# sangminwoo/SVOL

Hardware: AMD Instinct MI355X
Metric: frames/sec (fwd+matcher+bwd), T=32·P=196·d=256 (higher is better)
Workload: dtype bf16

## Files before the change

### include/svol_hip.h

```cpp
#ifndef SVOL_HIP_H
#define SVOL_HIP_H

#include <stdint.h>

#ifdef __cplusplus
extern "C" {
#endif

#define SVOL_F32 0
#define SVOL_BF16 1
#define SVOL_F16 2

#define SVOL_OK 0
#define SVOL_E_INVALID (-1)
#define SVOL_E_UNSUPPORTED (-2)
#define SVOL_E_LAUNCH (-3)

#define SVOL_ACT_NONE 0
#define SVOL_ACT_RELU 1
#define SVOL_ACT_GELU 2
#define SVOL_ACT_SIGMOID 3
#define SVOL_ACT_GELU_D 5
#define SVOL_ACT_RELU_RES 4

int svol_abi_version(void);
const char* svol_strerror(int code);

int svol_cast(const void* src, int dtype_src, void* dst, int dtype_dst, int64_t n, void* stream);
int svol_cast_transpose(const float* src, void* dst, void* dstT, int dtype, int64_t R, int64_t C, void* stream);
int svol_cast_transpose_multi(const void* descs, int32_t n_desc, int64_t total_tiles, int dtype, void* stream);
int svol_cast_split(const float* src, int64_t ld_src, void* dst_hilo, int64_t R, int64_t C, void* stream);

int svol_adamw_flat(float* p, const float* g, float* m, float* v, int64_t n, float lr, float beta1, float beta2, float eps,
                    float weight_decay, int64_t step, float grad_scale, void* stream);
int svol_adamw_flat_zero(float* p, float* g, float* m, float* v, int64_t n, float lr, float beta1, float beta2, float eps,
                         float weight_decay, int64_t step, float grad_scale, void* stream);
int svol_grad_finite(const float* g, int64_t n, float* scaler_state, void* stream);
int svol_adamw_flat_scaled(float* p, const float* g, float* m, float* v, int64_t n, float lr, float beta1, float beta2, float eps,
                           float weight_decay, float grad_mul, const float* scaler_state, void* stream);
int svol_loss_scaler_update(float* scaler_state, float growth_factor, float backoff_factor, int64_t growth_interval, float min_scale,
                            float max_scale, void* stream);
int svol_sgd_flat(float* p, const float* g, float* buf, int64_t n, float lr, float momentum, float weight_decay, float grad_scale,
                  void* stream);
int svol_sgd_flat_zero(float* p, float* g, float* buf, int64_t n, float lr, float momentum, float weight_decay, float grad_scale,
                       void* stream);
int svol_sgd_flat_scaled(float* p, const float* g, float* buf, int64_t n, float lr, float momentum, float weight_decay, float grad_mul,
                         const float* scaler_state, void* stream);
int svol_adam_flat(float* p, const float* g, float* m, float* v, int64_t n, float lr, float beta1, float beta2, float eps,
                   float weight_decay, int64_t step, float grad_scale, void* stream);
int svol_adam_flat_zero(float* p, float* g, float* m, float* v, int64_t n, float lr, float beta1, float beta2, float eps,
                        float weight_decay, int64_t step, float grad_scale, void* stream);
int svol_adam_flat_scaled(float* p, const float* g, float* m, float* v, int64_t n, float lr, float beta1, float beta2, float eps,
                          float weight_decay, float grad_mul, const float* scaler_state, void* stream);
int64_t svol_grad_sqnorm_ws_bytes(int64_t n);
int svol_grad_sqnorm(const float* g, int64_t n, float* ws, float* out, void* stream);
int svol_grad_clip_state(const float* sq, int32_t nb, float grad_mul, float max_norm, float loss_scale, int64_t steps_taken,
                         float* scaler_state, float* state_out, void* stream);
int svol_sgd_flat_grouped(float* p, float* g, float* buf, int64_t n, const int32_t* seg_end, const int32_t* seg_group, int32_t nseg,
                          const float* hyper, int32_t ngroups, const float* state, float grad_mul, int zero, void* stream);
int svol_adam_flat_grouped(float* p, float* g, float* m, float* v, int64_t n, const int32_t* seg_end, const int32_t* seg_group,
                           int32_t nseg, const float* hyper, int32_t ngroups, const float* state, const float* step_count,
                           float grad_mul, int zero, void* stream);
int svol_adamw_flat_grouped(float* p, float* g, float* m, float* v, int64_t n, const int32_t* seg_end, const int32_t* seg_group,
                            int32_t nseg, const float* hyper, int32_t ngroups, const float* state, const float* step_count,
                            float grad_mul, int zero, void* stream);
int svol_flat_step_advance(float* step_count, const float* state, void* stream);

int svol_gemm_nt(const void* A, int64_t lda, const void* A2, int64_t n_split, const void* B, int64_t ldb,
                 void* C, int64_t ldc, const float* bias, const float* colscale, int act, void* pre_act_out,
                 int64_t ldp, const void* residual, int64_t ldr, int out_f32, int64_t M, int64_t N, int64_t K,
                 int dtype, void* stream);
int svol_gemm_nt_split(const void* A, int64_t lda, const void* W_hilo, int64_t ldw, void* C, int64_t ldc, const float* bias,
                       int64_t M, int64_t N, int64_t K, void* stream);
int svol_gemm_nt_dgelu(const void* A, int64_t lda, const void* B, int64_t ldb, void* C, int64_t ldc,
                       const void* pre, int64_t ldp, float* colsum, int64_t M, int64_t N, int64_t K, int dtype,
                       void* stream);
int svol_gemm_nt_dact(const void* A, int64_t lda, const void* B, int64_t ldb, void* C, int64_t ldc,
                      const void* aux, int64_t ldaux, int act, float* colsum, int64_t M, int64_t N, int64_t K,
                      int dtype, void* stream);

int svol_gemm_tn(const void* A, int64_t lda, const void* B, int64_t ldb, float* C, int64_t ldc, float* colsum,
                 int64_t Mc, int64_t N, int64_t K, int dtype, void* stream);
#define SVOL_TN_GROUP_MAX 6
typedef struct svol_tn_problem {
    const void* A; int64_t lda;
    const void* B; int64_t ldb;
    float* C; int64_t ldc;
    float* colsum;
    int64_t Mc, N, K;
} svol_tn_problem;
int svol_gemm_tn_grouped(const svol_tn_problem* problems, int32_t n, int dtype, void* stream);
int svol_colsum(const void* X, int64_t ldx, float* out, int64_t M, int64_t N, int dtype, void* stream);
int svol_act_bwd(const void* dy, const void* aux, void* dpre, int act, int64_t n, int dtype, void* stream);

int svol_layernorm_fwd(const void* x, int x_f32, const float* gamma, const float* beta, float* y32, void* y,
                       void* ypos, const void* pos, int64_t pos_rows, float* mean, float* rstd, int64_t M, int64_t D,
                       float dropout_p, uint64_t seed, const int64_t* seed_offset_dev, int dtype, void* stream);
int svol_layernorm_bwd(const float* dy32, const void* dy, const void* dy2, const void* x, int x_f32,
                       const float* gamma, const float* mean, const float* rstd, float* dx32, void* dx,
                       float* dgamma, float* dbeta, float* dx_colsum, int64_t M, int64_t D, float dropout_p,
                       uint64_t seed, const int64_t* seed_offset_dev, int dtype, void* stream);

int svol_dropout(const void* x, void* y, int64_t n, int64_t row_len, float p, uint64_t seed, int dtype, void* stream);
int svol_dropout_add(const float* t32, const float* res32, float* out32, int64_t n, int64_t row_len, float p, uint64_t seed, void* stream);
int svol_dropout_sd(const void* x, void* y, int64_t n, int64_t row_len, float p, uint64_t seed, const int64_t* seed_step_dev, int dtype,
                    void* stream);
int svol_dropout_add_sd(const float* t32, const float* res32, float* out32, int64_t n, int64_t row_len, float p, uint64_t seed,
                        const int64_t* seed_step_dev, void* stream);

int svol_posenc_sine(const float* mask, void* pos, int64_t B, int64_t L, int64_t D, int dtype, void* stream);

int64_t svol_attn_ws_bytes(int64_t B, int64_t H, int64_t Lq, int64_t Lk, int64_t dh);
int svol_attn_fwd(const void* q, int64_t ldq, const void* k, int64_t ldk, const void* v, int64_t ldv, void* o,
                  int64_t ldo, float* lse2, const float* kbias, int64_t B, int64_t H, int64_t Lq, int64_t Lk,
                  int64_t dh, float scale, float q_premul, void* ws, int64_t ws_bytes, int dtype, void* stream);
int svol_attn_bwd(const void* q, int64_t ldq, const void* k, int64_t ldk, const void* v, int64_t ldv, const void* o,
                  int64_t ldo, const void* d_o, int64_t lddo, const float* lse2, float* delta, const float* kbias,
                  void* dq, int64_t lddq, void* dk, int64_t lddk, void* dv, int64_t lddv, int64_t B, int64_t H,
                  int64_t Lq, int64_t Lk, int64_t dh, float scale, float q_premul, void* ws, int64_t ws_bytes,
                  int dtype, void* stream);

#define SVOL_ATTN_DQ_PREZEROED 1
int64_t svol_attn_bwd_sp_image_bytes(int64_t B, int64_t H, int64_t Lq, int64_t Lk, int64_t dh, int64_t ws_bytes, int dtype);
int svol_attn_bwd_zero_ws(void* ws, int64_t ws_bytes, int64_t B, int64_t H, int64_t Lq, int64_t Lk, int64_t dh, int dtype, void* stream);
int svol_attn_bwd_ex(const void* q, int64_t ldq, const void* k, int64_t ldk, const void* v, int64_t ldv, const void* o,
                     int64_t ldo, const void* d_o, int64_t lddo, const float* lse2, float* delta, const float* kbias,
                     void* dq, int64_t lddq, void* dk, int64_t lddk, void* dv, int64_t lddv, int64_t B, int64_t H,
                     int64_t Lq, int64_t Lk, int64_t dh, float scale, float q_premul, void* ws, int64_t ws_bytes,
                     int dtype, int flags, void* ev_prep, void* stream);

int svol_attn_fwd_dropout(const void* q, int64_t ldq, const void* k, int64_t ldk, const void* v, int64_t ldv, void* o,
                          int64_t ldo, float* lse2, const float* kbias, int64_t B, int64_t H, int64_t Lq, int64_t Lk,
                          int64_t dh, float scale, float q_premul, void* ws, int64_t ws_bytes, float dropout_p, uint64_t seed,
                          int dtype, void* stream);
int svol_attn_bwd_dropout(const void* q, int64_t ldq, const void* k, int64_t ldk, const void* v, int64_t ldv, const void* o,
                          int64_t ldo, const void* d_o, int64_t lddo, const float* lse2, float* delta, const float* kbias,
                          void* dq, int64_t lddq, void* dk, int64_t lddk, void* dv, int64_t lddv, int64_t B, int64_t H,
                          int64_t Lq, int64_t Lk, int64_t dh, float scale, float q_premul, void* ws, int64_t ws_bytes,
                          float dropout_p, uint64_t seed, int dtype, void* stream);
int svol_attn_fwd_dropout_sd(const void* q, int64_t ldq, const void* k, int64_t ldk, const void* v, int64_t ldv, void* o,
                             int64_t ldo, float* lse2, const float* kbias, int64_t B, int64_t H, int64_t Lq, int64_t Lk,
                             int64_t dh, float scale, float q_premul, void* ws, int64_t ws_bytes, float dropout_p, uint64_t seed,
                             const int64_t* seed_step_dev, int dtype, void* stream);
int svol_attn_bwd_dropout_sd(const void* q, int64_t ldq, const void* k, int64_t ldk, const void* v, int64_t ldv, const void* o,
                             int64_t ldo, const void* d_o, int64_t lddo, const float* lse2, float* delta, const float* kbias,
                             void* dq, int64_t lddq, void* dk, int64_t lddk, void* dv, int64_t lddv, int64_t B, int64_t H,
                             int64_t Lq, int64_t Lk, int64_t dh, float scale, float q_premul, void* ws, int64_t ws_bytes,
                             float dropout_p, uint64_t seed, const int64_t* seed_step_dev, int dtype, void* stream);

int svol_gate_fwd(const float* x32, const void* pos, const float* u, const float* gamma, const float* beta,
                  float* y32, void* y, void* ypos, float* a, float* mean, float* rstd, float* ws, int64_t B,
                  int64_t L, int64_t D, int64_t H, int dtype, void* stream);
int svol_gate_bwd(const float* dy32, const void* dy, const void* dy2, const float* x32, const void* pos,
                  const float* u, const float* gamma, const float* a, const float* mean, const float* rstd,
                  const float* ws, float* ws2, float* dx32, float* du, float* dgamma, float* dbeta, int64_t B,
                  int64_t L, int64_t D, int64_t H, int dtype, void* stream);

int svol_layernorm_gate_scores_fwd(const float* x32, const float* gamma, const float* beta, float* y32, void* y, void* ypos,
                                   const void* pos, float* mean, float* rstd, const float* u_next, float* scores_next,
                                   int64_t B, int64_t L, int64_t D, int64_t H, int dtype, void* stream);
int svol_gate_fwd_scored(const float* x32, const void* pos, const float* u, const float* gamma, const float* beta,
                         float* y32, void* y, void* ypos, float* a, float* mean, float* rstd, float* ws, int64_t B,
                         int64_t L, int64_t D, int64_t H, int dtype, void* stream);

int svol_gate_vectors_fwd(const float* skch, const float* W_in, const float* b_in, float* q_out, float* u_out, int64_t B, int64_t D,
                          int64_t H, void* stream);
int svol_gate_vectors_bwd(const float* du, const float* skch, const float* W_in, const float* q, float* dq_ws, float* dskch,
                          float* dW_in, float* db_in, int64_t B, int64_t D, int64_t H, void* stream);
#define SVOL_GATE_VEC_MAX_LAYERS 8
int svol_gate_vectors_fwd_multi(const float* skch, const float* const* W_in, const float* const* b_in, float* const* q_out,
                                float* const* u_out, int64_t n_layers, int64_t B, int64_t D, int64_t H, void* stream);
int svol_gate_vectors_bwd_multi(const float* const* du, const float* skch, const float* const* W_in, const float* const* q,
                                float* const* dq_ws, float* const* dskch, float* const* dW_in, float* const* db_in, int64_t n_layers,
                                int64_t B, int64_t D, int64_t H, void* stream);

int svol_match_cost(const float* logits, const float* boxes, const float* tgt_boxes, const int32_t* pred_off,
                    const int32_t* pred_cnt, const int32_t* tgt_off, const int32_t* tgt_cnt,
                    const int64_t* cost_off, float* cost, int32_t n_problems, float w_bbox, float w_giou,
                    float w_class, int32_t* box_status, void* stream);
int svol_lsap_batched(const float* cost, const int64_t* cost_off, const int32_t* pred_off, const int32_t* pred_cnt,
                      const int32_t* tgt_off, const int32_t* tgt_cnt, int32_t* match, int32_t* status,
                      int32_t n_problems, int32_t max_dim, void* stream);
int svol_heads_fwd(const float* hs, const float* Wc, const float* bc, const float* W0, const float* b0, const float* W1, const float* b1,
                   const float* W2, const float* b2, float* logits, float* h1, float* h2, float* boxes, int64_t R, int64_t D, void* stream);
int svol_heads_bwd(const float* dlogits, const float* dboxes, const float* hs, const float* h1, const float* h2, const float* boxes,
                   const float* Wc, const float* W0, const float* W1, const float* W2, float* dhs, float* gp0, float* gp1, float* dWc,
                   float* dbc, float* dW2, float* db2, int64_t R, int64_t D, void* stream);
int svol_set_loss_bwd(const float* g_label, const float* g_bbox, const float* g_giou, const float* dl, float* dlogits, float* dboxes,
                      int64_t n_layers, int64_t rows_per_layer, void* stream);
int svol_weighted_total(const float* x, const float* w, int64_t n, float* out, void* stream);
int svol_weighted_total_bwd(const float* w, const float* dout, int64_t n, float* dx, void* stream);
int svol_lsap_solve(const double* cost, int64_t nr, int64_t nc, int64_t* rows, int64_t* cols);
int svol_set_loss(const float* logits, const float* boxes, const float* tgt_boxes, const int32_t* match,
                  float* losses, float* g_label, float* g_bbox, float* g_giou, int32_t n_layers,
                  int32_t rows_per_layer, float eos_coef, const int32_t* rebase_vid_off, int32_t rows_per_video,
                  const int32_t* status, const int32_t* box_status, int32_t problems_per_layer, void* stream);

int svol_postprocess(const float* logits, const float* boxes, float* out, int64_t B, int64_t N, int64_t chunk, void* stream);
int svol_eval_max_iou(const double* pred_box, const int32_t* pred_off, const double* gt_box, const int32_t* gt_off,
                      const int32_t* gt_rec, double* out, int64_t n_gt, int32_t k, void* stream);
int svol_eval_ap(const double* pred_box, const double* pred_score, const int32_t* pred_frame, const int32_t* grp_pred_off,
                 const double* gt_box, const int32_t* gt_frame, const int32_t* grp_gt_off, const double* thresholds,
                 int32_t n_thresholds, int32_t* ws_order, unsigned char* ws_u8, double* ws_f64, double* ap, int64_t n_pred,
                 int64_t n_gt, int64_t n_groups, void* stream);

int svol_ingest_resize(const uint8_t* src, int64_t n, int64_t H, int64_t W, int64_t s_n, int64_t s_h, int64_t s_w,
                       const int32_t* xtab, int64_t kx, const int32_t* ytab, int64_t ky, const float* lut, const uint8_t* flip,
                       void* out, int64_t o_n, int64_t o_c, int64_t o_h, int64_t o_w, int64_t OH, int64_t OW, int out_dtype,
                       void* stream);

int svol_patchify(const float* pixel_values, void* out, int64_t n, int64_t C, int64_t H, int64_t W, int64_t p, int dtype,
                  void* stream);
int svol_vit_embed(const float* patch_proj, const float* cls_token, const float* pos_embed, float* x32, void* x, int64_t n,
                   int64_t P, int64_t D, int dtype, void* stream);
int svol_im2col(const void* x, int64_t sn, int64_t sh, int64_t sw, int64_t sc, int src_dtype, void* cols, int64_t ldcols,
                int64_t N, int64_t H, int64_t W, int64_t C, int64_t kh, int64_t kw, int64_t stride, int64_t pad, int dtype,
                void* stream);
int svol_conv_nhwc(const void* x, const void* w, int64_t ldw, void* y, const float* bias, int act, const void* residual,
                   int64_t N, int64_t H, int64_t W, int64_t C, int64_t Cout, int64_t kh, int64_t kw, int64_t stride,
                   int64_t pad, int dtype, void* stream);
int svol_maxpool_nhwc(const void* x, void* y, int64_t N, int64_t H, int64_t W, int64_t C, int64_t k, int64_t stride,
                      int64_t pad, int dtype, void* stream);
int svol_avgpool_nhwc(const void* x, float* y, int64_t N, int64_t HW, int64_t C, int dtype, void* stream);
int svol_bn_colstats(const void* z, const float* shift, float shift_scale, float* sum, float* sumsq, int64_t M, int64_t C, int dtype,
                     void* stream);
int svol_bn_finalize(const float* sum, const float* sumsq_centered, const float* pivot, const float* gamma, const float* beta,
                     float* running_mean, float* running_var, float momentum, float eps, int64_t M, int64_t C, float* mean, float* rstd,
                     float* scale, float* shift, void* stream);
int svol_conv_weight_pack(const float* w, void* out, int64_t Cout, int64_t Cin, int64_t kh, int64_t kw, int64_t Kp, int flip, int dtype,
                          void* stream);
int svol_conv_weight_unpack_add(const float* dwp, float* grad, int64_t Cout, int64_t Cin, int64_t kh, int64_t kw, int64_t Kp, void* stream);
int svol_conv_wgrad_nhwc(const void* dz, const void* x, float* dwp, int64_t N, int64_t H, int64_t W, int64_t C, int64_t Cout, int64_t kh, int64_t kw,
                         int64_t stride, int64_t pad, int64_t Kp, int dtype, void* stream);
int svol_bn_apply(const void* z, const float* scale, const float* shift, const void* residual, int relu, void* y, int64_t M, int64_t C,
                  int dtype, void* stream);
int svol_bn_bwd_reduce(const void* dy, const void* y, const void* z, const float* mean, const float* rstd, float* sum_g, float* sum_gx,
                       int64_t M, int64_t C, int dtype, void* stream);
int svol_bn_bwd_apply(const void* dy, const void* y, const void* z, const float* mean, const float* rstd, const float* gamma,
                      const float* sum_g, const float* sum_gx, void* dz, void* dres, int64_t M, int64_t C, int dtype, void* stream);
int svol_col2im_nhwc(const void* dcols, int64_t ldcols, void* dx, int64_t N, int64_t H, int64_t W, int64_t C, int64_t kh, int64_t kw,
                     int64_t stride, int64_t pad, int dtype, void* stream);
int svol_maxpool_idx_nhwc(const void* x, void* y, uint8_t* idx, int64_t N, int64_t H, int64_t W, int64_t C, int64_t k, int64_t stride,
                          int64_t pad, int dtype, void* stream);
int svol_maxpool_bwd_nhwc(const void* dy, const uint8_t* idx, void* dx, int64_t N, int64_t H, int64_t W, int64_t C, int64_t k,
                          int64_t stride, int64_t pad, int dtype, void* stream);
int svol_attn_weights_mean(const void* q, int64_t ldq, const void* k, int64_t ldk, const float* lse2, const float* kbias,
                           float* att, int64_t B, int64_t H, int64_t Lq, int64_t Lk, int64_t dh, float scale,
                           float q_premul, int dtype, void* stream);
int svol_attn_small_fwd(const void* q, int64_t ldq, const void* k, int64_t ldk, const void* v, int64_t ldv, void* o, int64_t ldo,
                        int64_t n_seq, int64_t H, int64_t L, int64_t dh, float scale, int dtype, void* stream);
int svol_attn_small_fwd_lse(const void* q, int64_t ldq, const void* k, int64_t ldk, const void* v, int64_t ldv, void* o, int64_t ldo,
                            float* lse2, int64_t n_seq, int64_t H, int64_t L, int64_t dh, float scale, int dtype, void* stream);
int svol_attn_small_bwd(const void* q, int64_t ldq, const void* k, int64_t ldk, const void* v, int64_t ldv, const void* o, int64_t ldo,
                        const void* dout, int64_t lddo, const float* lse2, void* dq, int64_t lddq, void* dk, int64_t lddk, void* dv,
                        int64_t lddv, int64_t n_seq, int64_t H, int64_t L, int64_t dh, float scale, int dtype, void* stream);
int svol_attn_small_fwd_h16(const void* q, int64_t ldq, const void* k, int64_t ldk, const void* v, int64_t ldv, void* o, int64_t ldo,
                            int64_t n_seq, int64_t H, int64_t L, int64_t dh, float scale, int dtype, void* stream);
int svol_attn_small_fwd_lse_h16(const void* q, int64_t ldq, const void* k, int64_t ldk, const void* v, int64_t ldv, void* o, int64_t ldo,
                                float* lse2, int64_t n_seq, int64_t H, int64_t L, int64_t dh, float scale, int dtype, void* stream);
int svol_attn_small_bwd_h16(const void* q, int64_t ldq, const void* k, int64_t ldk, const void* v, int64_t ldv, const void* o, int64_t ldo,
                            const void* dout, int64_t lddo, const float* lse2, void* dq, int64_t lddq, void* dk, int64_t lddk, void* dv,
                            int64_t lddv, int64_t n_seq, int64_t H, int64_t L, int64_t dh, float scale, int dtype, void* stream);

int svol_attn_cls_fwd(const void* q, int64_t ldq, const void* k, int64_t ldk, const void* v, int64_t ldv, void* o, int64_t ldo, float* lse2,
                      int64_t n, int64_t H, int64_t L, int64_t dh, float scale, int dtype, void* stream);
int svol_attn_cls_bwd(const void* q, int64_t ldq, const void* k, int64_t ldk, const void* v, int64_t ldv, const void* o, int64_t ldo,
                      const void* dout, int64_t lddo, const float* lse2, void* dq, int64_t lddq, void* dk, int64_t lddk, void* dv,
                      int64_t lddv, int64_t n, int64_t H, int64_t L, int64_t dh, float scale, int dtype, void* stream);
int svol_attn_cls_fwd_h16(const void* q, int64_t ldq, const void* k, int64_t ldk, const void* v, int64_t ldv, void* o, int64_t ldo, float* lse2,
                          int64_t n, int64_t H, int64_t L, int64_t dh, float scale, int dtype, void* stream);
int svol_attn_cls_bwd_h16(const void* q, int64_t ldq, const void* k, int64_t ldk, const void* v, int64_t ldv, const void* o, int64_t ldo,
                          const void* dout, int64_t lddo, const float* lse2, void* dq, int64_t lddq, void* dk, int64_t lddk, void* dv,
                          int64_t lddv, int64_t n, int64_t H, int64_t L, int64_t dh, float scale, int dtype, void* stream);
int svol_softmax_xent(const float* logits, int64_t ld, const int64_t* targets, float* loss, float* dlogits, int64_t lddl, int32_t* correct,
                      int64_t n, int64_t C, void* stream);


#define SVOL_DIM_B 0
#define SVOL_DIM_L 1
#define SVOL_DIM_N 2
#define SVOL_DIM_D 3
#define SVOL_DIM_H 4
#define SVOL_DIM_F 5
#define SVOL_DIM_DTYPE 6
#define SVOL_DIM_QDTYPE 7
#define SVOL_DIM_ATTN_WS_BYTES 8
#define SVOL_DIM_COUNT 9

#define SVOL_BLK_VIDEO_HALF 0
#define SVOL_BLK_QUERY_SELF 1
#define SVOL_BLK_QUERY_CROSS 2
const char* svol_block_slot_names(int block);
int svol_block_trace_dump(char* buf, int64_t cap);
int svol_clock_probe(uint64_t* samples, int32_t* count, int32_t max_samples, const int32_t* stop, int64_t period_us,
                     int64_t max_ms, int32_t* wall_khz, void* stream);


#define SVOL_VH_SLOTS(X) \
    X(X32) X(POS) X(U) X(G1) X(BT1) X(G2) X(BT2) X(G3) X(BT3) X(B_IN) X(B_O) X(B_FC1) X(B_FC2) X(QSCALE) \
    X(W_IN) X(WV_HILO) X(W_O) X(W_FC1) X(W_FC2) X(W_IN_T) X(W_O_T) X(W_FC1_T) X(W_FC2_T) \
    X(Y1) X(Y1POS) X(A) X(MEAN1) X(RSTD1) X(GATE_WS) X(GATE_PRE) X(U_NEXT) X(GATE_WS_NEXT) \
    X(QKV) X(O) X(LSE) X(S2) X(Y2) X(MEAN2) X(RSTD2) X(PRE) X(HID) X(S3) \
    X(MEAN3) X(RSTD3) X(M32) X(M) X(MPOS) X(Y1_32) X(Y2_32) X(ATTN_WS) \
    X(DM32) X(DM) X(DMPOS) X(DS32_3) X(DS3) X(DPRE) X(DY2) X(DS32_2) X(G2D) X(DO) X(DQKV) X(DELTA) X(DXQP) X(DXQ) X(GATE_WS2) \
    X(DX32) X(DU) \
    X(DG1) X(DBT1) X(DG2) X(DBT2) X(DG3) X(DBT3) X(DW_IN) X(DB_IN) X(DW_O) X(DB_O) X(DW_FC1) X(DB_FC1) X(DW_FC2) X(DB_FC2) \
    X(EV_A0) X(EV_A1) X(EV_CLEAN_IN) X(EV_PREP) X(ATTN_WS_NEXT) X(ZERO_STREAM) X(EV_CLEAN_OUT)
#define SVOL_QS_SLOTS(X) \
    X(O32) X(O) X(OPOS) X(QPOS) X(B_IN) X(B_O) X(G4) X(BT4) X(QSCALE) X(W_IN) X(WV_HILO) X(W_O) X(W_IN_T) X(W_O_T) \
    X(QKV) X(OA) X(LSE) X(S4) X(MEAN4) X(RSTD4) X(Y32) X(Y) X(YPOS) X(ATTN_WS) \
    X(DY32) X(DY) X(DYPOS) X(G) X(DOA) X(DQKV) X(DELTA) X(DO32) X(DXQ) X(DXQP) X(DQPOS) \
    X(DW_IN) X(DB_IN) X(DW_O) X(DB_O) X(DG4) X(DBT4)
#define SVOL_QC_SLOTS(X) \
    X(O32) X(O) X(OPOS) X(MV) X(MPOS) X(KBIAS) X(QPOS) X(B_IN) X(B_O) X(G5) X(BT5) X(B_FC1) X(B_FC2) X(G6) X(BT6) X(QSCALE) \
    X(W_INQ) X(W_INQ_T) X(W_KV) X(W_KV_T) X(WV_HILO) X(W_O) X(W_O_T) X(W_FC1) X(W_FC1_T) X(W_FC2) X(W_FC2_T) \
    X(Q) X(QC) X(KV) X(OA) X(OAQ) X(LSE) X(S5) X(Y5_32) X(Y5) X(MEAN5) X(RSTD5) X(PRE) X(HID) X(S6) X(MEAN6) X(RSTD6) \
    X(Y32) X(Y) X(YPOS) X(ATTN_WS) \
    X(DY32) X(DY) X(DYPOS) X(DS32_6) X(DS6) X(DPRE) X(DY5) X(DS32_5) X(G5D) X(DOAQ) X(DOA) X(DQC) X(DQ) X(DKV) X(DELTA) \
    X(DO32) X(DXQP) X(DMPOS) X(DMV) X(DQPOS) \
    X(DW_IN) X(DB_IN) X(DW_O) X(DB_O) X(DG5) X(DBT5) X(DW_FC1) X(DB_FC1) X(DW_FC2) X(DB_FC2) X(DG6) X(DBT6)
#define SVOL_SLOT_ENUM_VH(n) SVOL_VH_##n,
#define SVOL_SLOT_ENUM_QS(n) SVOL_QS_##n,
#define SVOL_SLOT_ENUM_QC(n) SVOL_QC_##n,
enum { SVOL_VH_SLOTS(SVOL_SLOT_ENUM_VH) SVOL_VH_COUNT };
enum { SVOL_QS_SLOTS(SVOL_SLOT_ENUM_QS) SVOL_QS_COUNT };
enum { SVOL_QC_SLOTS(SVOL_SLOT_ENUM_QC) SVOL_QC_COUNT };

int svol_video_half_fwd(const int64_t* dims, void* const* slots, void* stream);
int svol_video_half_bwd(const int64_t* dims, void* const* slots, int phase, void* stream);
int svol_video_half_wgrad(const int64_t* dims, void* const* slots, void* stream);
int svol_video_half_wgrad_part(const int64_t* dims, void* const* slots, int part, void* stream);
int svol_query_self_fwd(const int64_t* dims, void* const* slots, void* stream);
int svol_query_self_bwd(const int64_t* dims, void* const* slots, void* stream);
int svol_query_self_wgrad(const int64_t* dims, void* const* slots, void* stream);
int svol_query_cross_fwd(const int64_t* dims, void* const* slots, void* stream);
int svol_query_cross_bwd(const int64_t* dims, void* const* slots, void* stream);
int svol_query_cross_wgrad(const int64_t* dims, void* const* slots, void* stream);

#ifdef __cplusplus
}
#endif
#endif
```

### svol_amd/_lib.py

```python
from __future__ import annotations

import ctypes
import os

_HERE = os.path.dirname(os.path.abspath(__file__))
LIB_PATH = os.path.join(_HERE, 'libsvol_hip.so')

_p = ctypes.c_void_p
_i64 = ctypes.c_int64
_i32 = ctypes.c_int32
_int = ctypes.c_int
_f32 = ctypes.c_float
_u64 = ctypes.c_uint64

SIGNATURES = {
    'svol_block_trace_dump': [ctypes.c_char_p, _i64],
    'svol_lsap_solve': [_p, _i64, _i64, _p, _p],
    'svol_heads_fwd': [_p] * 13 + [_i64, _i64, _p],
    'svol_heads_bwd': [_p] * 17 + [_i64, _i64, _p],
    'svol_set_loss_bwd': [_p] * 6 + [_i64, _i64, _p],
    'svol_weighted_total': [_p, _p, _i64, _p, _p],
    'svol_weighted_total_bwd': [_p, _p, _i64, _p, _p],
    'svol_cast': [_p, _int, _p, _int, _i64, _p],
    'svol_cast_transpose': [_p, _p, _p, _int, _i64, _i64, _p],
    'svol_cast_split': [_p, _i64, _p, _i64, _i64, _p],
    'svol_gemm_nt_split': [_p, _i64, _p, _i64, _p, _i64, _p, _i64, _i64, _i64, _p],
    'svol_gemm_nt': [_p, _i64, _p, _i64, _p, _i64, _p, _i64, _p, _p, _int, _p, _i64, _p, _i64, _int, _i64, _i64, _i64,
                     _int, _p],
    'svol_gemm_nt_dgelu': [_p, _i64, _p, _i64, _p, _i64, _p, _i64, _p, _i64, _i64, _i64, _int, _p],
    'svol_gemm_nt_dact': [_p, _i64, _p, _i64, _p, _i64, _p, _i64, _int, _p, _i64, _i64, _i64, _int, _p],
    'svol_gemm_tn': [_p, _i64, _p, _i64, _p, _i64, _p, _i64, _i64, _i64, _int, _p],
    'svol_gemm_tn_grouped': [_p, _i32, _int, _p],
    'svol_colsum': [_p, _i64, _p, _i64, _i64, _int, _p],
    'svol_act_bwd': [_p, _p, _p, _int, _i64, _int, _p],
    'svol_layernorm_fwd': [_p, _int, _p, _p, _p, _p, _p, _p, _i64, _p, _p, _i64, _i64, _f32, _u64, _p, _int, _p],
    'svol_layernorm_bwd': [_p, _p, _p, _p, _int, _p, _p, _p, _p, _p, _p, _p, _p, _i64, _i64, _f32, _u64, _p, _int, _p],
    'svol_cast_transpose_multi': [_p, _int, _i64, _int, _p],
    'svol_postprocess': [_p, _p, _p, _i64, _i64, _i64, _p],
    'svol_eval_max_iou': [_p, _p, _p, _p, _p, _p, _i64, _int, _p],
    'svol_eval_ap': [_p, _p, _p, _p, _p, _p, _p, _p, _int, _p, _p, _p, _p, _i64, _i64, _i64, _p],
    'svol_patchify': [_p, _p, _i64, _i64, _i64, _i64, _i64, _int, _p],
    'svol_vit_embed': [_p, _p, _p, _p, _p, _i64, _i64, _i64, _int, _p],
    'svol_ingest_resize': [_p, _i64, _i64, _i64, _i64, _i64, _i64, _p, _i64, _p, _i64, _p, _p, _p, _i64, _i64, _i64, _i64, _i64, _i64, _int, _p],
    'svol_adamw_flat': [_p, _p, _p, _p, _i64, _f32, _f32, _f32, _f32, _f32, _i64, _f32, _p],
    'svol_adamw_flat_zero': [_p, _p, _p, _p, _i64, _f32, _f32, _f32, _f32, _f32, _i64, _f32, _p],
    'svol_grad_finite': [_p, _i64, _p, _p],
    'svol_adamw_flat_scaled': [_p, _p, _p, _p, _i64, _f32, _f32, _f32, _f32, _f32, _f32, _p, _p],
    'svol_loss_scaler_update': [_p, _f32, _f32, _i64, _f32, _f32, _p],
    'svol_sgd_flat': [_p, _p, _p, _i64, _f32, _f32, _f32, _f32, _p],
    'svol_sgd_flat_zero': [_p, _p, _p, _i64, _f32, _f32, _f32, _f32, _p],
    'svol_sgd_flat_scaled': [_p, _p, _p, _i64, _f32, _f32, _f32, _f32, _p, _p],
    'svol_adam_flat': [_p, _p, _p, _p, _i64, _f32, _f32, _f32, _f32, _f32, _i64, _f32, _p],
    'svol_adam_flat_zero': [_p, _p, _p, _p, _i64, _f32, _f32, _f32, _f32, _f32, _i64, _f32, _p],
    'svol_adam_flat_scaled': [_p, _p, _p, _p, _i64, _f32, _f32, _f32, _f32, _f32, _f32, _p, _p],
    'svol_grad_sqnorm_ws_bytes': [_i64],
    'svol_grad_sqnorm': [_p, _i64, _p, _p, _p],
    'svol_grad_clip_state': [_p, _i32, _f32, _f32, _f32, _i64, _p, _p, _p],
    'svol_sgd_flat_grouped': [_p, _p, _p, _i64, _p, _p, _i32, _p, _i32, _p, _f32, _int, _p],
    'svol_adam_flat_grouped': [_p, _p, _p, _p, _i64, _p, _p, _i32, _p, _i32, _p, _p, _f32, _int, _p],
    'svol_adamw_flat_grouped': [_p, _p, _p, _p, _i64, _p, _p, _i32, _p, _i32, _p, _p, _f32, _int, _p],
    'svol_flat_step_advance': [_p, _p, _p],
    'svol_conv_nhwc': [_p, _p, _i64, _p, _p, _int, _p, _i64, _i64, _i64, _i64, _i64, _i64, _i64, _i64, _i64, _int, _p],
    'svol_im2col': [_p, _i64, _i64, _i64, _i64, _int, _p, _i64, _i64, _i64, _i64, _i64, _i64, _i64, _i64, _i64, _int, _p],
    'svol_maxpool_nhwc': [_p, _p, _i64, _i64, _i64, _i64, _i64, _i64, _i64, _int, _p],
    'svol_avgpool_nhwc': [_p, _p, _i64, _i64, _i64, _int, _p],
    'svol_bn_colstats': [_p, _p, _f32, _p, _p, _i64, _i64, _int, _p],
    'svol_bn_finalize': [_p, _p, _p, _p, _p, _p, _p, _f32, _f32, _i64, _i64, _p, _p, _p, _p, _p],
    'svol_conv_weight_pack': [_p, _p, _i64, _i64, _i64, _i64, _i64, _int, _int, _p],
    'svol_conv_weight_unpack_add': [_p, _p, _i64, _i64, _i64, _i64, _i64, _p],
    'svol_conv_wgrad_nhwc': [_p, _p, _p, _i64, _i64, _i64, _i64, _i64, _i64, _i64, _i64, _i64, _i64, _int, _p],
    'svol_bn_apply': [_p, _p, _p, _p, _int, _p, _i64, _i64, _int, _p],
    'svol_bn_bwd_reduce': [_p, _p, _p, _p, _p, _p, _p, _i64, _i64, _int, _p],
    'svol_bn_bwd_apply': [_p, _p, _p, _p, _p, _p, _p, _p, _p, _p, _i64, _i64, _int, _p],
    'svol_col2im_nhwc': [_p, _i64, _p, _i64, _i64, _i64, _i64, _i64, _i64, _i64, _i64, _int, _p],
    'svol_maxpool_idx_nhwc': [_p, _p, _p, _i64, _i64, _i64, _i64, _i64, _i64, _i64, _int, _p],
    'svol_maxpool_bwd_nhwc': [_p, _p, _p, _i64, _i64, _i64, _i64, _i64, _i64, _i64, _int, _p],
    'svol_attn_weights_mean': [_p, _i64, _p, _i64, _p, _p, _p, _i64, _i64, _i64, _i64, _i64, _f32, _f32, _int, _p],
    'svol_attn_small_fwd': [_p, _i64, _p, _i64, _p, _i64, _p, _i64, _i64, _i64, _i64, _i64, _f32, _int, _p],
    'svol_attn_small_fwd_lse': [_p, _i64, _p, _i64, _p, _i64, _p, _i64, _p, _i64, _i64, _i64, _i64, _f32, _int, _p],
    'svol_attn_small_bwd': [_p, _i64, _p, _i64, _p, _i64, _p, _i64, _p, _i64, _p, _p, _i64, _p, _i64, _p, _i64, _i64, _i64, _i64,
                            _i64, _f32, _int, _p],
    'svol_attn_cls_fwd': [_p, _i64, _p, _i64, _p, _i64, _p, _i64, _p, _i64, _i64, _i64, _i64, _f32, _int, _p],
    'svol_attn_cls_bwd': [_p, _i64, _p, _i64, _p, _i64, _p, _i64, _p, _i64, _p, _p, _i64, _p, _i64, _p, _i64, _i64, _i64, _i64,
                          _i64, _f32, _int, _p],
    'svol_attn_small_fwd_h16': [_p, _i64, _p, _i64, _p, _i64, _p, _i64, _i64, _i64, _i64, _i64, _f32, _int, _p],
    'svol_attn_small_fwd_lse_h16': [_p, _i64, _p, _i64, _p, _i64, _p, _i64, _p, _i64, _i64, _i64, _i64, _f32, _int, _p],
    'svol_attn_small_bwd_h16': [_p, _i64, _p, _i64, _p, _i64, _p, _i64, _p, _i64, _p, _p, _i64, _p, _i64, _p, _i64, _i64, _i64, _i64,
                                _i64, _f32, _int, _p],
    'svol_attn_cls_fwd_h16': [_p, _i64, _p, _i64, _p, _i64, _p, _i64, _p, _i64, _i64, _i64, _i64, _f32, _int, _p],
    'svol_attn_cls_bwd_h16': [_p, _i64, _p, _i64, _p, _i64, _p, _i64, _p, _i64, _p, _p, _i64, _p, _i64, _p, _i64, _i64, _i64, _i64,
                              _i64, _f32, _int, _p],
    'svol_softmax_xent': [_p, _i64, _p, _p, _p, _i64, _p, _i64, _i64, _p],
    'svol_posenc_sine': [_p, _p, _i64, _i64, _i64, _int, _p],
    'svol_attn_ws_bytes': [_i64, _i64, _i64, _i64, _i64],
    'svol_attn_fwd': [_p, _i64, _p, _i64, _p, _i64, _p, _i64, _p, _p, _i64, _i64, _i64, _i64, _i64, _f32, _f32, _p, _i64,
                      _int, _p],
    'svol_attn_bwd': [_p, _i64, _p, _i64, _p, _i64, _p, _i64, _p, _i64, _p, _p, _p, _p, _i64, _p, _i64, _p, _i64,
                      _i64, _i64, _i64, _i64, _i64, _f32, _f32, _p, _i64, _int, _p],
    'svol_attn_bwd_ex': [_p, _i64, _p, _i64, _p, _i64, _p, _i64, _p, _i64, _p, _p, _p, _p, _i64, _p, _i64, _p, _i64,
                         _i64, _i64, _i64, _i64, _i64, _f32, _f32, _p, _i64, _int, _int, _p, _p],
    'svol_attn_bwd_sp_image_bytes': [_i64, _i64, _i64, _i64, _i64, _i64, _int],
    'svol_attn_bwd_zero_ws': [_p, _i64, _i64, _i64, _i64, _i64, _i64, _int, _p],
    'svol_attn_fwd_dropout': [_p, _i64, _p, _i64, _p, _i64, _p, _i64, _p, _p, _i64, _i64, _i64, _i64, _i64, _f32, _f32, _p, _i64,
                              _f32, _u64, _int, _p],
    'svol_attn_bwd_dropout': [_p, _i64, _p, _i64, _p, _i64, _p, _i64, _p, _i64, _p, _p, _p, _p, _i64, _p, _i64, _p, _i64,
                              _i64, _i64, _i64, _i64, _i64, _f32, _f32, _p, _i64, _f32, _u64, _int, _p],
    'svol_dropout': [_p, _p, _i64, _i64, _f32, _u64, _int, _p],
    'svol_dropout_add': [_p, _p, _p, _i64, _i64, _f32, _u64, _p],
    'svol_attn_fwd_dropout_sd': [_p, _i64, _p, _i64, _p, _i64, _p, _i64, _p, _p, _i64, _i64, _i64, _i64, _i64, _f32, _f32, _p, _i64,
                                 _f32, _u64, _p, _int, _p],
    'svol_attn_bwd_dropout_sd': [_p, _i64, _p, _i64, _p, _i64, _p, _i64, _p, _i64, _p, _p, _p, _p, _i64, _p, _i64, _p, _i64,
                                 _i64, _i64, _i64, _i64, _i64, _f32, _f32, _p, _i64, _f32, _u64, _p, _int, _p],
    'svol_dropout_sd': [_p, _p, _i64, _i64, _f32, _u64, _p, _int, _p],
    'svol_dropout_add_sd': [_p, _p, _p, _i64, _i64, _f32, _u64, _p, _p],
    'svol_gate_fwd': [_p, _p, _p, _p, _p, _p, _p, _p, _p, _p, _p, _p, _i64, _i64, _i64, _i64, _int, _p],
    'svol_gate_bwd': [_p, _p, _p, _p, _p, _p, _p, _p, _p, _p, _p, _p, _p, _p, _p, _p, _i64, _i64, _i64, _i64, _int,
                      _p],
    'svol_clock_probe': [_p, _p, _int, _p, _i64, _i64, _p, _p],
    'svol_gate_fwd_scored': [_p, _p, _p, _p, _p, _p, _p, _p, _p, _p, _p, _p, _i64, _i64, _i64, _i64, _int, _p],
    'svol_layernorm_gate_scores_fwd': [_p, _p, _p, _p, _p, _p, _p, _p, _p, _p, _p, _i64, _i64, _i64, _i64, _int, _p],
    'svol_gate_vectors_fwd': [_p, _p, _p, _p, _p, _i64, _i64, _i64, _p],
    'svol_gate_vectors_bwd': [_p, _p, _p, _p, _p, _p, _p, _p, _i64, _i64, _i64, _p],
    'svol_gate_vectors_fwd_multi': [_p, _p, _p, _p, _p, _i64, _i64, _i64, _i64, _p],
    'svol_gate_vectors_bwd_multi': [_p, _p, _p, _p, _p, _p, _p, _p, _i64, _i64, _i64, _i64, _p],
    'svol_match_cost': [_p, _p, _p, _p, _p, _p, _p, _p, _p, _i32, _f32, _f32, _f32, _p, _p],
    'svol_lsap_batched': [_p, _p, _p, _p, _p, _p, _p, _p, _i32, _i32, _p],
    'svol_set_loss': [_p, _p, _p, _p, _p, _p, _p, _p, _i32, _i32, _f32, _p, _i32, _p, _p, _i32, _p],
    'svol_video_half_fwd': [_p, _p, _p],
    'svol_video_half_bwd': [_p, _p, _int, _p],
    'svol_video_half_wgrad': [_p, _p, _p],
    'svol_video_half_wgrad_part': [_p, _p, _int, _p],
    'svol_query_self_fwd': [_p, _p, _p],
    'svol_query_self_bwd': [_p, _p, _p],
    'svol_query_self_wgrad': [_p, _p, _p],
    'svol_query_cross_fwd': [_p, _p, _p],
    'svol_query_cross_bwd': [_p, _p, _p],
    'svol_query_cross_wgrad': [_p, _p, _p],
}



class TnProblem(ctypes.Structure):
    _fields_ = [('A', _p), ('lda', _i64), ('B', _p), ('ldb', _i64), ('C', _p), ('ldc', _i64), ('colsum', _p),
                ('Mc', _i64), ('N', _i64), ('K', _i64)]


_LIB = None


class SvolHipError(RuntimeError):
    pass


def lib():
    global _LIB
    if _LIB is None:
        if not os.path.exists(LIB_PATH):
            raise SvolHipError(
                f'{LIB_PATH} not found: the SVOL hot path has no CPU fallback. '
                'Build it with `python -m svol_amd.build` (hipcc, gfx950).')
        L = ctypes.CDLL(LIB_PATH)
        L.svol_abi_version.restype = _int
        L.svol_abi_version.argtypes = []
        L.svol_strerror.restype = ctypes.c_char_p
        L.svol_strerror.argtypes = [_int]
        for name, at in SIGNATURES.items():
            f = getattr(L, name)
            f.restype = _int
            f.argtypes = at
        L.svol_attn_ws_bytes.restype = _i64
        L.svol_attn_bwd_sp_image_bytes.restype = _i64
        L.svol_grad_sqnorm_ws_bytes.restype = _i64
        L.svol_block_slot_names.restype = ctypes.c_char_p
        L.svol_block_slot_names.argtypes = [_int]
        _LIB = L
    return _LIB


def check(rc: int, name: str):
    if rc != 0:
        msg = lib().svol_strerror(rc).decode()
        raise SvolHipError(f'{name} failed: {msg} (code {rc})')
```

### svol_amd/blocks.py

```python
from __future__ import annotations

import ctypes
import math
import os
import weakref

import torch

from . import _lib, layers, ops, params, wgrad

ENABLED = os.environ.get('SVOL_NO_BLOCKS') is None
GATE_SCORES_FUSE = os.environ.get('SVOL_GATE_SCORES_FUSE') is not None
VH, QS, QC = 0, 1, 2
_F32, _BF16 = 0, 1
_ESZ = {torch.float32: 4, torch.bfloat16: 2, torch.float16: 2}
_SLOTS = {}


def _slots(block):
    m = _SLOTS.get(block)
    if m is None:
        names = _lib.lib().svol_block_slot_names(block).decode().rstrip(',').split(',')
        m = _SLOTS[block] = {n: i for i, n in enumerate(names)}
    return m


class _Table:

    __slots__ = ('arr', 'idx', 'n')

    def __init__(self, block, template=None):
        self.idx = _slots(block)
        self.n = len(self.idx)
        self.arr = (ctypes.c_void_p * self.n)()
        if template is not None:
            ctypes.memmove(self.arr, template.arr, self.n * 8)

    def set(self, name, ptr):
        self.arr[self.idx[name]] = ptr

    def set_t(self, name, t):
        self.arr[self.idx[name]] = t.data_ptr() if t is not None else None


def _align(n, a=256):
    return (n + a - 1) // a * a


class _Layout:

    def __init__(self, items):
        self.off = {}
        n = 0
        for name, nbytes in items:
            self.off[name] = (n, nbytes)
            n += _align(nbytes)
        self.total = max(n, 256)

    def fill(self, tbl, base):
        for name, (o, _) in self.off.items():
            tbl.arr[tbl.idx[name]] = base + o

    def view(self, arena, name, dtype, shape):
        o, nb = self.off[name]
        return arena[o:o + nb].view(dtype).view(shape)


_LAYOUTS = {}


def _layout(key, make):
    lay = _LAYOUTS.get(key)
    if lay is None:
        lay = _LAYOUTS[key] = _Layout(make())
    return lay


_SCRATCH = {}


def _scratch(dev, nbytes):
    key = (dev, ops._stream())
    t = _SCRATCH.get(key)
    if t is None or t.numel() < nbytes:
        t = _SCRATCH[key] = torch.empty((_align(nbytes, 1 << 20),), dtype=torch.uint8, device=dev)
    return t


def _dims(B, L, N, D, H, F, dt, qdt, ws_bytes):
    return (ctypes.c_int64 * 9)(B, L, N, D, H, F, ops._DT[dt], ops._DT[qdt], ws_bytes)


def _c(t):
    return t if t is None or t.is_contiguous() else t.contiguous()


_VH_PARAMS = [
    ('DG1', lambda l: l.norm1.weight), ('DBT1', lambda l: l.norm1.bias),
    ('DW_IN', lambda l: l.content_self_attn.in_proj_weight), ('DB_IN', lambda l: l.content_self_attn.in_proj_bias),
    ('DW_O', lambda l: l.content_self_attn.out_proj.weight), ('DB_O', lambda l: l.content_self_attn.out_proj.bias),
    ('DG2', lambda l: l.norm2.weight), ('DBT2', lambda l: l.norm2.bias),
    ('DW_FC1', lambda l: l.mlp1.fc1.weight), ('DB_FC1', lambda l: l.mlp1.fc1.bias),
    ('DW_FC2', lambda l: l.mlp1.fc2.weight), ('DB_FC2', lambda l: l.mlp1.fc2.bias),
    ('DG3', lambda l: l.norm3.weight), ('DBT3', lambda l: l.norm3.bias)]
_QS_PARAMS = [
    ('DW_IN', lambda l: l.token_self_attn.in_proj_weight), ('DB_IN', lambda l: l.token_self_attn.in_proj_bias),
    ('DW_O', lambda l: l.token_self_attn.out_proj.weight), ('DB_O', lambda l: l.token_self_attn.out_proj.bias),
    ('DG4', lambda l: l.norm4.weight), ('DBT4', lambda l: l.norm4.bias)]
_QC_PARAMS = [
    ('DW_IN', lambda l: l.content_token_cross_attn.in_proj_weight), ('DB_IN', lambda l: l.content_token_cross_attn.in_proj_bias),
    ('DW_O', lambda l: l.content_token_cross_attn.out_proj.weight), ('DB_O', lambda l: l.content_token_cross_attn.out_proj.bias),
    ('DG5', lambda l: l.norm5.weight), ('DBT5', lambda l: l.norm5.bias),
    ('DW_FC1', lambda l: l.mlp2.fc1.weight), ('DB_FC1', lambda l: l.mlp2.fc1.bias),
    ('DW_FC2', lambda l: l.mlp2.fc2.weight), ('DB_FC2', lambda l: l.mlp2.fc2.bias),
    ('DG6', lambda l: l.norm6.weight), ('DBT6', lambda l: l.norm6.bias)]
_PARAMS = {VH: _VH_PARAMS, QS: _QS_PARAMS, QC: _QC_PARAMS}


class BlockPlan:

    def __init__(self, block, layer, dt, qdt):
        self.block, self.dt, self.qdt = block, dt, qdt
        self.layer = weakref.ref(layer)
        self.params = [g(layer) for _, g in _PARAMS[block]]
        self.grad_slots = [n for n, _ in _PARAMS[block]]
        self.tpl = _Table(block)
        self.keep = []
        D = layer.d_model
        self.split_v = params.SPLIT_V and D % 32 == 0
        t = self.tpl
        W = params.weights
        dev = self.params[0].device

        self.casts = []
        self.epoch = W.epoch

        def both(name, w, dtype):
            got = wc, wt = W.get(w, dtype)
            t.set_t(name, wc)
            t.set_t(name + '_T', wt)
            self.keep += [wc, wt]
            self.casts.append((W.get, (w, dtype), got))

        wdt = dt if block == VH else qdt
        adt = qdt if block == QS else dt
        for slot, p in zip(self.grad_slots, self.params):
            if p.dim() == 1:
                t.set_t(slot[1:], p)
            elif block == QC and slot == 'DW_IN':
                both('W_INQ', p, qdt)
                both('W_KV', p, dt)
            else:
                both(slot[1:], p, wdt)
        if adt == torch.bfloat16 and self.split_v:
            w_in = self.params[self.grad_slots.index('DW_IN')]
            hl = W.get_split(w_in, 2 * D, D)
            t.set_t('WV_HILO', hl)
            self.keep.append(hl)
            self.casts.append((W.get_split, (w_in, 2 * D, D), hl))
        if adt != torch.float32:
            q = layers._qscale(D, layers.LOG2E / math.sqrt(D // layer.nhead), dev)
            t.set_t('QSCALE', q)
            self.keep.append(q)
        self.sinks = [params.claim(p, p.requires_grad) for p in self.params]
        self.nosink = [(i, p.numel()) for i, (p, s) in enumerate(zip(self.params, self.sinks)) if s is None]
        for name, s in zip(self.grad_slots, self.sinks):
            if s is not None:
                t.set_t(name, s.view)
        self.graph_params = self.params if (self.nosink or any(s.owner is None for s in self.sinks)) else []
        cnt = {}
        for s in self.sinks:
            if s is not None and s.owner is not None:
                cnt[(id(s.owner), s.bucket)] = (s.owner, s.bucket, cnt.get((id(s.owner), s.bucket), (None, None, 0))[2] + 1)
        self.notify = list(cnt.values())
        self.key = self._key()

    def _key(self):
        k = []
        for p in self.params:
            g = p.grad
            s = getattr(p, '_svol_sink', None)
            k.append((p.data_ptr(), g.data_ptr() if (g is not None and s is not None) else 0, p.requires_grad))
        return (params.SPLIT_V, tuple(k))

    def valid(self):
        return self.layer() is not None and self._key() == self.key

    def fresh_copies(self):
        for again, args, got in self.casts:
            if again(*args) is not got:
                return False
        return True

    def grad_buffers(self, tbl, dev):
        if not self.nosink:
            return None
        offs, n = [], 0
        for _, numel in self.nosink:
            offs.append(n)
            n += (numel + 3) // 4 * 4
        flat = torch.zeros((n,), dtype=torch.float32, device=dev)
        out = {}
        base = flat.data_ptr()
        for (i, numel), o in zip(self.nosink, offs):
            tbl.set(self.grad_slots[i], base + o * 4)
            out[i] = flat[o:o + numel].view_as(self.params[i])
        return out

    def inputs(self, *tensors):
        if self.graph_params or not any(t_.requires_grad for t_ in tensors):
            return self.params
        return ()

    def done(self, in_graph):
        if not in_graph:
            for owner, bi, n in self.notify:
                owner.params_done(bi, n)

    def grads_out(self, bufs, needs, in_graph):
        res = []
        if not in_graph:
            return res
        for i, p in enumerate(self.params):
            if bufs is not None and i in bufs and needs[i]:
                res.append(bufs[i])
            else:
                res.append(None)
        return res


_PLANS = weakref.WeakKeyDictionary()


def plan(layer, block, dt, qdt):
    per = _PLANS.get(layer)
    if per is None:
        per = _PLANS[layer] = {}
    k = (block, dt, qdt)
    pl = per.get(k)
    if pl is None or not pl.valid() or not pl.fresh_copies():
        pl = per[k] = BlockPlan(block, layer, dt, qdt)
    return pl


def _call(name, ctx, *extra, stream=None):
    rc = getattr(_lib.lib(), name)(ctx.dims, ctx.tbl.arr, *extra, ops._stream() if stream is None else stream)
    _lib.check(rc, name)


def _open(ctx, pl, block, key, dims, n_par, dev, fwd_items, scr_items, **inputs):
    ctx.set_materialize_grads(False)
    lay = _layout(('f', block) + key, fwd_items)
    slay = _layout(('s', block) + key, scr_items)
    arena = torch.empty((lay.total,), dtype=torch.uint8, device=dev)
    tbl = _Table(block, pl.tpl)
    lay.fill(tbl, arena.data_ptr())
    slay.fill(tbl, _scratch(dev, slay.total).data_ptr())
    for name, t in inputs.items():
        tbl.set(name, t.data_ptr())
    ctx.pl, ctx.tbl, ctx.dims, ctx.arena, ctx.key, ctx.n_par = pl, tbl, dims, arena, (block,) + key, n_par
    return lay


def _no_grads(ctx, n_in):
    ctx.pl.done(ctx.n_par > 0)
    return (None,) * (n_in + ctx.n_par)


def _open_bwd(ctx, dev, bwd_items, **grads):
    tbl = ctx.tbl
    lay = _layout(('b',) + ctx.key, bwd_items)
    tmp = torch.empty((lay.total,), dtype=torch.uint8, device=dev)
    lay.fill(tbl, tmp.data_ptr())
    gs = []
    for name, g in grads.items():
        g = _c(g)
        tbl.set_t(name, g)
        if g is not None:
            gs.append(g)
    slay = _layout(('s',) + ctx.key, None)
    slay.fill(tbl, _scratch(dev, slay.total).data_ptr())
    return lay, tmp, ctx.pl.grad_buffers(tbl, dev), gs


def _close_bwd(ctx, name, bufs, keep, n_in):
    if bufs is not None or not wgrad.issue(lambda ws: _call(name, ctx, stream=ws.cuda_stream), keep, ops._current_stream_obj()):
        _call(name, ctx)
    in_graph = ctx.n_par > 0
    ctx.pl.done(in_graph)
    return tuple(ctx.pl.grads_out(bufs, ctx.needs_input_grad[n_in:], in_graph))


def _maybe_events(name, meta):
    tm = ops.timer
    if not tm.enabled or name not in tm.names:
        return None
    e0, e1 = torch.cuda.Event(enable_timing=True), torch.cuda.Event(enable_timing=True)
    e0.record()
    e1.record()
    tm.records.setdefault((name, meta), []).append((e0, e1))
    return e0, e1


DQ_PREZERO = os.environ.get('SVOL_DQ_PREZERO') is not None and os.environ.get('SVOL_NO_DQ_PREZERO') is None
_DQ_PREZERO = {}


class _DqPrezero:
    __slots__ = ('bufs', 'side', 'ev_prep', 'clean_ev', 'clean', 'nxt')

    def __init__(self, dev, wsb):
        self.bufs = [torch.empty((_align(wsb, 1 << 20),), dtype=torch.uint8, device=dev) for _ in range(2)]
        self.side = torch.cuda.Stream(device=dev)
        self.ev_prep = torch.cuda.Event()
        self.clean_ev = [torch.cuda.Event(), torch.cuda.Event()]
        for e_ in [self.ev_prep] + self.clean_ev:
            e_.record()
        self.clean = [False, False]
        self.nxt = 0

    def bind(self, tbl):
        i = self.nxt
        tbl.set('ATTN_WS', self.bufs[i].data_ptr())
        tbl.set('EV_CLEAN_IN', self.clean_ev[i].cuda_event if self.clean[i] else None)
        tbl.set('EV_PREP', self.ev_prep.cuda_event)
        tbl.set('ATTN_WS_NEXT', self.bufs[1 - i].data_ptr())
        tbl.set('ZERO_STREAM', self.side.cuda_stream)
        tbl.set('EV_CLEAN_OUT', self.clean_ev[1 - i].cuda_event)
        self.clean[i] = False

    def advance(self, tbl):
        i = self.nxt
        self.clean[1 - i] = True
        self.nxt = 1 - i
        for n_ in ('EV_CLEAN_IN', 'EV_PREP', 'ATTN_WS_NEXT', 'ZERO_STREAM', 'EV_CLEAN_OUT'):
            tbl.set(n_, None)


def _dq_prezero(dev, B, H, L, dh, dt, wsb):
    if not DQ_PREZERO or dt == torch.float32 or torch.cuda.is_current_stream_capturing():
        return None
    key = (dev, ops._stream(), B, H, L, dh, dt, wsb)
    st = _DQ_PREZERO.get(key)
    if st is None:
        img = _lib.lib().svol_attn_bwd_sp_image_bytes(B, H, L, L, dh, wsb, ops._DT[dt])
        st = _DQ_PREZERO[key] = _DqPrezero(dev, wsb) if img > 0 else False
    return st or None


def _vh_fwd_layout(B, L, D, H, F, e):
    M = B * L
    return [('Y1', M * D * e), ('Y1POS', M * D * e), ('A', M * 4), ('MEAN1', M * 4), ('RSTD1', M * 4), ('GATE_WS', B * H * (L + 2) * 4),
            ('QKV', M * 3 * D * e), ('O', M * D * e), ('LSE', B * H * L * 4), ('S2', M * D * 4), ('Y2', M * D * e), ('MEAN2', M * 4),
            ('RSTD2', M * 4), ('PRE', M * F * e), ('HID', M * F * e), ('S3', M * D * 4), ('MEAN3', M * 4), ('RSTD3', M * 4),
            ('M32', M * D * 4), ('M', M * D * e), ('MPOS', M * D * e)]


def _vh_bwd_layout(B, L, D, H, F, e):
    M = B * L
    return [('DS32_3', M * D * 4), ('DS3', M * D * e), ('DPRE', M * F * e), ('DY2', M * D * e), ('DS32_2', M * D * 4), ('G2D', M * D * e),
            ('DO', M * D * e), ('DQKV', M * 3 * D * e), ('DELTA', 3 * B * H * L * 4), ('DXQ', M * D * e),
            ('GATE_WS2', (B * L + B * H) * 4), ('DX32', M * D * 4)]


def _attn_events(tbl, ev):
    tbl.set('EV_A0', ev[0].cuda_event if ev else None)
    tbl.set('EV_A1', ev[1].cuda_event if ev else None)


class VideoHalfFn(torch.autograd.Function):

    @staticmethod
    def forward(ctx, pl, x32, pos, u, u_next, sc_in, *params):
        B, L, D = x32.shape
        layer = pl.layer()
        H, F = layer.nhead, layer.mlp1.fc1.weight.shape[0]
        dt = pl.dt
        e = _ESZ[dt]
        dev = x32.device
        M = B * L
        x2, pos2, u = _c(x32.reshape(M, D)), _c(pos.reshape(M, D)), _c(u)
        assert x2.dtype == torch.float32 and pos2.dtype == dt and u.dtype == torch.float32
        wsb = ops.attn_ws_bytes(dt, B, H, L, L, D // H)
        lay = _open(ctx, pl, VH, (B, L, D, H, F, dt), _dims(B, L, 0, D, H, F, dt, dt, wsb), len(params), dev,
                    lambda: _vh_fwd_layout(B, L, D, H, F, e),
                    lambda: [('Y1_32', M * D * 4), ('Y2_32', M * D * 4), ('ATTN_WS', max(wsb, 16))], X32=x2, POS=pos2, U=u)
        tbl = ctx.tbl
        if sc_in is not None:
            assert sc_in.dtype == torch.float32 and sc_in.numel() == B * H * (L + 2) and sc_in.is_contiguous()
            tbl.set('GATE_WS', sc_in.data_ptr())
            tbl.set('GATE_PRE', sc_in.data_ptr())
        if u_next is not None:
            u_next = u_next.contiguous()
            assert u_next.dtype == torch.float32 and u_next.shape == u.shape and L % 4 == 0
            sc_next = torch.empty((B * H * (L + 2),), dtype=torch.float32, device=dev)
            tbl.set('U_NEXT', u_next.data_ptr())
            tbl.set('GATE_WS_NEXT', sc_next.data_ptr())
        else:
            sc_next = torch.empty((0,), dtype=torch.float32, device=dev)
        ctx.big = wgrad.attn_forward(B * H * L * L)
        _attn_events(tbl, _maybe_events('attn_fwd', (B, H, L, L, D // H)))
        _call('svol_video_half_fwd', ctx)
        _attn_events(tbl, None)
        tbl.set('U_NEXT', None)
        tbl.set('GATE_WS_NEXT', None)
        ctx.shape = (B, L, D, H, F)
        ctx.sc_in = sc_in
        ctx.save_for_backward(x2, pos2, u)
        ctx.mark_non_differentiable(sc_next)
        return (lay.view(ctx.arena, 'M32', torch.float32, (B, L, D)), lay.view(ctx.arena, 'M', dt, (B, L, D)),
                lay.view(ctx.arena, 'MPOS', dt, (B, L, D)), sc_next)

    @staticmethod
    def backward(ctx, dm32, dm, dmpos, _dsc=None):
        if dm32 is None and dm is None and dmpos is None:
            return _no_grads(ctx, 6)
        tbl = ctx.tbl
        B, L, D, H, F = ctx.shape
        dt = ctx.pl.dt
        dev = ctx.saved_tensors[0].device
        du = torch.zeros((B, H, D), dtype=torch.float32, device=dev)
        tbl.set('DU', du.data_ptr())
        lay, tmp, bufs, gs = _open_bwd(ctx, dev, lambda: _vh_bwd_layout(B, L, D, H, F, _ESZ[dt]), DM32=dm32, DM=dm, DMPOS=dmpos)
        _call('svol_video_half_bwd', ctx, 1)
        wgrad.attn_backward(B * H * L * L)
        _attn_events(tbl, _maybe_events('attn_bwd', (B, H, L, L, D // H)))
        pz = _dq_prezero(dev, B, H, L, D // H, dt, ctx.dims[8]) if ctx.big else None
        if pz is not None:
            pz.bind(tbl)
        _call('svol_video_half_bwd', ctx, 2)
        if pz is not None:
            pz.advance(tbl)
        _attn_events(tbl, None)
        pg = _close_bwd(ctx, 'svol_video_half_wgrad', bufs, [ctx.arena, tmp] + gs, 6)
        dx32 = lay.view(tmp, 'DX32', torch.float32, (B, L, D))
        return (None, dx32, None, du if ctx.needs_input_grad[3] else None, None, None) + pg


def gate_scores_fusable(L, D, H):
    return GATE_SCORES_FUSE and L % 4 == 0 and D % 4 == 0 and D <= 256 and H <= 8


def video_half(layer, x32, pos, u, dt, u_next=None, sc_in=None):
    pl = plan(layer, VH, dt, dt)
    if u_next is not None and not gate_scores_fusable(x32.shape[1], x32.shape[2], layer.nhead):
        u_next = None
    m32, m, mpos, sc = VideoHalfFn.apply(pl, x32, pos, u, u_next, sc_in, *pl.inputs(x32, u))
    return m32, m, mpos, (sc if u_next is not None else None)


def _qpos_target(ctx, qpos, need, N, D):
    g = s = None
    if need and qpos.requires_grad:
        s = params.claim(qpos, True) if (qpos.is_leaf and qpos.dtype == torch.float32) else None
        if s is None:
            g = torch.zeros((N, D), dtype=torch.float32, device=qpos.device)
    ctx.tbl.set_t('DQPOS', s.view if s is not None else g)
    return g


def _qpos_grad(g, qdt):
    return ops.cast(g, qdt) if (g is not None and qdt != torch.float32) else g


class QuerySelfFn(torch.autograd.Function):

    @staticmethod
    def forward(ctx, pl, o32, o, opos, qpos, *params):
        B, N, D = o.shape
        H, qdt = pl.layer().nhead, pl.qdt
        e, R = _ESZ[qdt], B * N
        o32_, o_, opos_, qpos_ = _c(o32), _c(o), _c(opos), _c(qpos)
        assert o32_.dtype == torch.float32 and o_.dtype == qdt and opos_.dtype == qdt and qpos_.dtype == qdt
        wsb = ops.attn_ws_bytes(qdt, B, H, N, N, D // H)
        lay = _open(ctx, pl, QS, (B, N, D, H, qdt), _dims(B, 0, N, D, H, 0, qdt, qdt, wsb), len(params), o.device,
                    lambda: [('QKV', R * 3 * D * e), ('OA', R * D * e), ('LSE', B * H * N * 4), ('S4', R * D * 4), ('MEAN4', R * 4),
                             ('RSTD4', R * 4), ('Y32', R * D * 4), ('Y', R * D * e), ('YPOS', R * D * e)],
                    lambda: [('ATTN_WS', max(wsb, 16))], O32=o32_, O=o_, OPOS=opos_, QPOS=qpos_)
        _call('svol_query_self_fwd', ctx)
        ctx.shape = (B, N, D, H)
        ctx.save_for_backward(o32_, o_, opos_, qpos)
        return (lay.view(ctx.arena, 'Y32', torch.float32, (B, N, D)), lay.view(ctx.arena, 'Y', qdt, (B, N, D)),
                lay.view(ctx.arena, 'YPOS', qdt, (B, N, D)))

    @staticmethod
    def backward(ctx, dy32, dy, dypos):
        if dy32 is None and dy is None and dypos is None:
            return _no_grads(ctx, 5)
        B, N, D, H = ctx.shape
        o32_, o_, opos_, qpos = ctx.saved_tensors
        qdt = ctx.pl.qdt
        e, R = _ESZ[qdt], B * N
        gq = _qpos_target(ctx, qpos, ctx.needs_input_grad[4], N, D)
        lay, tmp, bufs, gs = _open_bwd(ctx, o_.device, lambda: [('G', R * D * e), ('DOA', R * D * e), ('DQKV', R * 3 * D * e),
                                                               ('DELTA', 3 * B * H * N * 4), ('DO32', R * D * 4), ('DXQ', R * D * e),
                                                               ('DXQP', R * D * e)], DY32=dy32, DY=dy, DYPOS=dypos)
        _call('svol_query_self_bwd', ctx)
        pg = _close_bwd(ctx, 'svol_query_self_wgrad', bufs, [ctx.arena, tmp, o_, opos_], 5)
        v = lambda n_, dt_: lay.view(tmp, n_, dt_, (B, N, D))
        return (None, v('DO32', torch.float32), v('DXQ', qdt), v('DXQP', qdt), _qpos_grad(gq, qdt)) + pg


def query_self(layer, out, qpos, dt, qdt):
    pl = plan(layer, QS, dt, qdt)
    o32, o, opos = out
    return QuerySelfFn.apply(pl, o32, o, opos, qpos, *pl.inputs(o32, o, opos))


def _qc_fwd_layout(B, N, L, D, H, F, e, qe):
    R, M = B * N, B * L
    return [('Q', R * D * qe), ('QC', R * D * e), ('KV', M * 2 * D * e), ('OA', R * D * e), ('OAQ', R * D * qe), ('LSE', B * H * N * 4),
            ('S5', R * D * 4), ('Y5_32', R * D * 4), ('Y5', R * D * qe), ('MEAN5', R * 4), ('RSTD5', R * 4), ('PRE', R * F * qe),
            ('HID', R * F * qe), ('S6', R * D * 4), ('MEAN6', R * 4), ('RSTD6', R * 4), ('Y32', R * D * 4), ('Y', R * D * qe),
            ('YPOS', R * D * qe)]


def _qc_bwd_layout(B, N, L, D, H, F, e, qe, merged):
    R, M = B * N, B * L
    return [('DS32_6', R * D * 4), ('DS6', R * D * qe), ('DPRE', R * F * qe), ('DY5', R * D * qe), ('G5D', R * D * qe), ('DOAQ', R * D * qe),
            ('DOA', R * D * e), ('DQC', R * D * e), ('DQ', R * D * qe), ('DKV', M * 2 * D * e), ('DELTA', 3 * B * H * N * 4),
            ('DO32', R * D * 4), ('DXQP', R * D * qe)] + ([] if merged else [('DMPOS', M * D * e)]) + [('DMV', M * D * e)]


class QueryCrossFn(torch.autograd.Function):

    @staticmethod
    def forward(ctx, pl, o32, o, opos, mv, mpos, kbias, qpos, merged, *params):
        B, N, D = o.shape
        L = mv.shape[1]
        layer = pl.layer()
        H, F = layer.nhead, layer.mlp2.fc1.weight.shape[0]
        dt, qdt = pl.dt, pl.qdt
        e, qe = _ESZ[dt], _ESZ[qdt]
        o32_, o_, opos_, mv_, mpos_, kb_, qpos_ = _c(o32), _c(o), _c(opos), _c(mv), _c(mpos), _c(kbias), _c(qpos)
        assert o32_.dtype == torch.float32 and o_.dtype == qdt and opos_.dtype == qdt and qpos_.dtype == qdt
        assert mv_.dtype == dt and mpos_.dtype == dt and kb_.dtype == torch.float32
        wsb = ops.attn_ws_bytes(dt, B, H, N, L, D // H)
        lay = _open(ctx, pl, QC, (B, N, L, D, H, F, dt, qdt, merged), _dims(B, L, N, D, H, F, dt, qdt, wsb), len(params), o.device,
                    lambda: _qc_fwd_layout(B, N, L, D, H, F, e, qe), lambda: [('ATTN_WS', max(wsb, 16))],
                    O32=o32_, O=o_, OPOS=opos_, MV=mv_, MPOS=mpos_, KBIAS=kb_, QPOS=qpos_)
        _call('svol_query_cross_fwd', ctx)
        ctx.shape = (B, N, L, D, H, F)
        ctx.merged = merged
        ctx.save_for_backward(o32_, o_, opos_, mv_, mpos_, kb_, qpos)
        return (lay.view(ctx.arena, 'Y32', torch.float32, (B, N, D)), lay.view(ctx.arena, 'Y', qdt, (B, N, D)),
                lay.view(ctx.arena, 'YPOS', qdt, (B, N, D)))

    @staticmethod
    def backward(ctx, dy32, dy, dypos):
        if dy32 is None and dy is None and dypos is None:
            return _no_grads(ctx, 9)
        B, N, L, D, H, F = ctx.shape
        o32_, o_, opos_, mv_, mpos_, kb_, qpos = ctx.saved_tensors
        dt, qdt = ctx.pl.dt, ctx.pl.qdt
        gq = _qpos_target(ctx, qpos, ctx.needs_input_grad[7], N, D)
        lay, tmp, bufs, gs = _open_bwd(ctx, o_.device, lambda: _qc_bwd_layout(B, N, L, D, H, F, _ESZ[dt], _ESZ[qdt], ctx.merged),
                                       DY32=dy32, DY=dy, DYPOS=dypos)
        _call('svol_query_cross_bwd', ctx)
        pg = _close_bwd(ctx, 'svol_query_cross_wgrad', bufs, [ctx.arena, tmp, opos_, mv_, mpos_], 9)
        vq = lambda n_, dt_: lay.view(tmp, n_, dt_, (B, N, D))
        vm = lambda n_: lay.view(tmp, n_, dt, (B, L, D))
        return (None, vq('DO32', torch.float32), None, vq('DXQP', qdt), vm('DMV'), None if ctx.merged else vm('DMPOS'), None,
                _qpos_grad(gq, qdt), None) + pg


def query_cross(layer, out, mv, mpos, kbias, qpos, dt, qdt):
    pl = plan(layer, QC, dt, qdt)
    o32, o, opos = out
    fn = mv.grad_fn
    merged = fn is not None and fn is mpos.grad_fn and isinstance(fn, VideoHalfFn._backward_cls)
    return QueryCrossFn.apply(pl, o32, o, opos, mv, mpos, kbias, qpos, merged, *pl.inputs(o32, opos, mv, mpos))


def trace_dump() -> str:
    buf = ctypes.create_string_buffer(1 << 20)
    _lib.check(_lib.lib().svol_block_trace_dump(buf, len(buf)), 'svol_block_trace_dump')
    return buf.value.decode()
```

### svol_amd/csrc/blocks.hip

```cpp
#include <math.h>
#include <stdio.h>
#include <stdlib.h>
#include <string.h>

#include <map>
#include <mutex>
#include <string>
#include <vector>

#include "common.h"

namespace {

const bool kTrace = getenv("SVOL_BLOCK_TRACE") != nullptr;
struct TraceRec { const char* prog; const char* site; hipEvent_t e0, e1; };
std::mutex g_trace_mu;
std::vector<TraceRec> g_trace_log;
struct Trace {
    const char* prog;
    hipStream_t s;
    hipEvent_t last = nullptr;
    Trace* prev;
    static thread_local Trace* cur;
    Trace(const char* prog_, void* s_) : prog(prog_), s(static_cast<hipStream_t>(s_)), prev(cur) {
        cur = this;
        if (kTrace && hipEventCreate(&last) == hipSuccess) (void)hipEventRecord(last, s);
    }
    ~Trace() { cur = prev; }
    void mark(const char* site) {
        if (!kTrace || !last) return;
        hipEvent_t e;
        if (hipEventCreate(&e) != hipSuccess) return;
        (void)hipEventRecord(e, s);
        std::lock_guard<std::mutex> lk(g_trace_mu);
        g_trace_log.push_back({prog, site, last, e});
        last = e;
    }
};
thread_local Trace* Trace::cur = nullptr;

struct Dims {
    int64_t B, L, N, D, H, F, ws_bytes;
    int dt, qdt;
    explicit Dims(const int64_t* d)
        : B(d[SVOL_DIM_B]), L(d[SVOL_DIM_L]), N(d[SVOL_DIM_N]), D(d[SVOL_DIM_D]), H(d[SVOL_DIM_H]), F(d[SVOL_DIM_F]),
          ws_bytes(d[SVOL_DIM_ATTN_WS_BYTES]), dt((int)d[SVOL_DIM_DTYPE]), qdt((int)d[SVOL_DIM_QDTYPE]) {}
    bool ok() const {
        return B > 0 && D > 0 && H > 0 && D % H == 0 && (dt == SVOL_F32 || svol_is16(dt)) && (qdt == SVOL_F32 || svol_is16(qdt));
    }
};

inline int esz(int dtype) { return svol_is16(dtype) ? 2 : 4; }
inline void* at(void* p, int64_t elems, int dtype) { return p ? static_cast<char*>(p) + elems * esz(dtype) : nullptr; }
inline const void* at(const void* p, int64_t elems, int dtype) { return p ? static_cast<const char*>(p) + elems * esz(dtype) : nullptr; }
inline float* f32(void* p) { return static_cast<float*>(p); }

inline float attn_scale(int64_t dh) { return (float)(1.0 / sqrt((double)dh)); }
inline float attn_premul(int64_t dh, int dtype) { return svol_is16(dtype) ? (float)(1.4426950408889634 / sqrt((double)dh)) : 0.f; }

inline int nt(const void* A, int64_t lda, const void* W, int64_t ldw, void* C, int64_t ldc, const void* bias, const void* colscale,
              int64_t M, int64_t N, int64_t K, int dtype, void* s) {
    return svol_gemm_nt(A, lda, nullptr, 0, W, ldw, C, ldc, static_cast<const float*>(bias), static_cast<const float*>(colscale),
                        SVOL_ACT_NONE, nullptr, 0, nullptr, 0, 0, M, N, K, dtype, s);
}
inline int nt_res(const void* A, int64_t lda, const void* W, int64_t ldw, void* C32, const void* bias, const void* res32, int64_t M,
                  int64_t N, int64_t K, int dtype, void* s) {
    return svol_gemm_nt(A, lda, nullptr, 0, W, ldw, C32, N, static_cast<const float*>(bias), nullptr, SVOL_ACT_NONE, nullptr, 0, res32, N,
                        1, M, N, K, dtype, s);
}

#define RUN(expr)                                 \
    do {                                          \
        const int rc_ = (expr);                   \
        if (rc_) return rc_;                      \
        if (kTrace && Trace::cur) Trace::cur->mark(#expr); \
    } while (0)

#define SLOT_NAME(n) #n ","
const char* const kVhNames = SVOL_VH_SLOTS(SLOT_NAME);
const char* const kQsNames = SVOL_QS_SLOTS(SLOT_NAME);
const char* const kQcNames = SVOL_QC_SLOTS(SLOT_NAME);

inline void record(void* ev, void* stream) {
    if (ev) (void)hipEventRecord(static_cast<hipEvent_t>(ev), static_cast<hipStream_t>(stream));
}

}


extern "C" {

int svol_block_trace_dump(char* buf, int64_t cap) {
    if (!buf || cap <= 0) return SVOL_E_INVALID;
    buf[0] = 0;
    if (!kTrace) return SVOL_OK;
    if (hipDeviceSynchronize() != hipSuccess) return SVOL_E_LAUNCH;
    std::lock_guard<std::mutex> lk(g_trace_mu);
    static const bool timeline = getenv("SVOL_BLOCK_TRACE") && atoi(getenv("SVOL_BLOCK_TRACE")) == 2;
    if (timeline && !g_trace_log.empty()) {
        std::string out;
        char line[256];
        const hipEvent_t ref = g_trace_log.front().e0;
        for (const TraceRec& r : g_trace_log) {
            float t0 = 0.f, t1 = 0.f;
            if (hipEventElapsedTime(&t0, ref, r.e0) != hipSuccess || hipEventElapsedTime(&t1, ref, r.e1) != hipSuccess) continue;
            std::string site(r.site);
            const size_t c = site.find(',');
            if (c != std::string::npos) site.resize(c);
            snprintf(line, sizeof line, "%9.3f %9.3f  %-20s %s\n", t0, t1, r.prog, site.c_str());
            out += line;
        }
        std::map<hipEvent_t, int> seen_;
        for (const TraceRec& r : g_trace_log) { seen_[r.e0] = 1; seen_[r.e1] = 1; }
        for (auto& kv : seen_) (void)hipEventDestroy(kv.first);
        g_trace_log.clear();
        strncpy(buf, out.c_str(), (size_t)cap - 1);
        buf[cap - 1] = 0;
        return SVOL_OK;
    }
    std::map<std::string, std::pair<double, int>> acc;
    std::vector<std::string> order;
    std::map<hipEvent_t, int> seen;
    for (const TraceRec& r : g_trace_log) {
        float ms = 0.f;
        if (hipEventElapsedTime(&ms, r.e0, r.e1) != hipSuccess) continue;
        std::string site(r.site);
        const size_t c = site.find(',');
        if (c != std::string::npos) site.resize(c);
        const std::string key = std::string(r.prog) + " | " + site;
        if (!acc.count(key)) order.push_back(key);
        acc[key].first += ms;
        acc[key].second += 1;
    }
    for (const TraceRec& r : g_trace_log) { seen[r.e0] = 1; seen[r.e1] = 1; }
    for (auto& kv : seen) (void)hipEventDestroy(kv.first);
    g_trace_log.clear();
    std::string out;
    char line[256];
    for (const std::string& k : order) {
        snprintf(line, sizeof line, "%-110s calls %6d  avg_us %9.1f  total_ms %9.3f\n", k.c_str(), acc[k].second,
                 acc[k].first / acc[k].second * 1e3, acc[k].first);
        out += line;
    }
    strncpy(buf, out.c_str(), (size_t)cap - 1);
    buf[cap - 1] = 0;
    return SVOL_OK;
}

const char* svol_block_slot_names(int block) {
    switch (block) {
        case SVOL_BLK_VIDEO_HALF: return kVhNames;
        case SVOL_BLK_QUERY_SELF: return kQsNames;
        case SVOL_BLK_QUERY_CROSS: return kQcNames;
        default: return "";
    }
}

int svol_video_half_fwd(const int64_t* dims, void* const* p, void* s) {
    if (!dims || !p) return SVOL_E_INVALID;
    Trace tr_("video_half_fwd", s);
    const Dims d(dims);
    if (!d.ok() || d.L <= 0 || d.F <= 0) return SVOL_E_INVALID;
    const int64_t M = d.B * d.L, D = d.D, F = d.F, dh = D / d.H;
    const int dt = d.dt, xf = dt != SVOL_F32;
#define P(n) p[SVOL_VH_##n]
    if (P(GATE_PRE))
        RUN(svol_gate_fwd_scored(f32(P(X32)), P(POS), f32(P(U)), f32(P(G1)), f32(P(BT1)), f32(P(Y1_32)), P(Y1), P(Y1POS), f32(P(A)),
                                 f32(P(MEAN1)), f32(P(RSTD1)), f32(P(GATE_WS)), d.B, d.L, D, d.H, dt, s));
    else
        RUN(svol_gate_fwd(f32(P(X32)), P(POS), f32(P(U)), f32(P(G1)), f32(P(BT1)), f32(P(Y1_32)), P(Y1), P(Y1POS), f32(P(A)), f32(P(MEAN1)),
                          f32(P(RSTD1)), f32(P(GATE_WS)), d.B, d.L, D, d.H, dt, s));
    RUN(nt(P(Y1POS), D, P(W_IN), D, P(QKV), 3 * D, P(B_IN), P(QSCALE), M, 2 * D, D, dt, s));
    if (P(WV_HILO))
        RUN(svol_gemm_nt_split(P(Y1), D, P(WV_HILO), 2 * D, at(P(QKV), 2 * D, dt), 3 * D, f32(P(B_IN)) + 2 * D, M, D, D, s));
    else
        RUN(nt(P(Y1), D, at(P(W_IN), 2 * D * D, dt), D, at(P(QKV), 2 * D, dt), 3 * D, f32(P(B_IN)) + 2 * D, nullptr, M, D, D, dt, s));
    record(P(EV_A0), s);
    RUN(svol_attn_fwd(P(QKV), 3 * D, at(P(QKV), D, dt), 3 * D, at(P(QKV), 2 * D, dt), 3 * D, P(O), D, f32(P(LSE)), nullptr, d.B, d.H, d.L,
                      d.L, dh, attn_scale(dh), attn_premul(dh, dt), P(ATTN_WS), d.ws_bytes, dt, s));
    record(P(EV_A1), s);
    RUN(nt_res(P(O), D, P(W_O), D, P(S2), P(B_O), P(Y1_32), M, D, D, dt, s));
    RUN(svol_layernorm_fwd(P(S2), xf, f32(P(G2)), f32(P(BT2)), f32(P(Y2_32)), P(Y2), nullptr, nullptr, 0, f32(P(MEAN2)), f32(P(RSTD2)), M,
                           D, 0.f, 0, nullptr, dt, s));
    RUN(svol_gemm_nt(P(Y2), D, nullptr, 0, P(W_FC1), D, P(HID), F, f32(P(B_FC1)), nullptr, SVOL_ACT_GELU_D, P(PRE), F, nullptr, 0, 0, M, F, D, dt, s));
    RUN(nt_res(P(HID), F, P(W_FC2), F, P(S3), P(B_FC2), P(Y2_32), M, D, F, dt, s));
    if (P(U_NEXT) && P(GATE_WS_NEXT))
        RUN(svol_layernorm_gate_scores_fwd(f32(P(S3)), f32(P(G3)), f32(P(BT3)), f32(P(M32)), P(M), P(MPOS), P(POS), f32(P(MEAN3)),
                                           f32(P(RSTD3)), f32(P(U_NEXT)), f32(P(GATE_WS_NEXT)), d.B, d.L, D, d.H, dt, s));
    else
        RUN(svol_layernorm_fwd(P(S3), xf, f32(P(G3)), f32(P(BT3)), f32(P(M32)), P(M), P(MPOS), P(POS), M, f32(P(MEAN3)), f32(P(RSTD3)), M, D,
                               0.f, 0, nullptr, dt, s));
    return SVOL_OK;
}

int svol_video_half_bwd(const int64_t* dims, void* const* p, int phase, void* s) {
    if (!dims || !p || phase < 0 || phase > 2) return SVOL_E_INVALID;
    Trace tr_(phase == 2 ? "video_half_bwd.2" : "video_half_bwd.1", s);
    const Dims d(dims);
    if (!d.ok() || d.L <= 0 || d.F <= 0) return SVOL_E_INVALID;
    const int64_t M = d.B * d.L, D = d.D, F = d.F, dh = D / d.H;
    const int dt = d.dt, xf = dt != SVOL_F32;
    if (phase != 2) {
        RUN(svol_layernorm_bwd(f32(P(DM32)), P(DM), P(DMPOS), P(S3), xf, f32(P(G3)), f32(P(MEAN3)), f32(P(RSTD3)), f32(P(DS32_3)), P(DS3),
                               f32(P(DG3)), f32(P(DBT3)), f32(P(DB_FC2)), M, D, 0.f, 0, nullptr, dt, s));
        RUN(svol_gemm_nt_dact(P(DS3), D, P(W_FC2_T), D, P(DPRE), F, P(PRE), F, SVOL_ACT_GELU_D, f32(P(DB_FC1)), M, F, D, dt, s));
        RUN(nt(P(DPRE), F, P(W_FC1_T), F, P(DY2), D, nullptr, nullptr, M, D, F, dt, s));
        RUN(svol_layernorm_bwd(f32(P(DS32_3)), P(DY2), nullptr, P(S2), xf, f32(P(G2)), f32(P(MEAN2)), f32(P(RSTD2)), f32(P(DS32_2)), P(G2D),
                               f32(P(DG2)), f32(P(DBT2)), f32(P(DB_O)), M, D, 0.f, 0, nullptr, dt, s));
        RUN(nt(P(G2D), D, P(W_O_T), D, P(DO), D, nullptr, nullptr, M, D, D, dt, s));
    }
    if (phase != 1) {
        int aflags = 0;
        if (P(EV_CLEAN_IN)) {
            if (hipStreamWaitEvent(static_cast<hipStream_t>(s), static_cast<hipEvent_t>(P(EV_CLEAN_IN)), 0) != hipSuccess) return SVOL_E_LAUNCH;
            aflags = SVOL_ATTN_DQ_PREZEROED;
        }
        record(P(EV_A0), s);
        RUN(svol_attn_bwd_ex(P(QKV), 3 * D, at(P(QKV), D, dt), 3 * D, at(P(QKV), 2 * D, dt), 3 * D, P(O), D, P(DO), D, f32(P(LSE)),
                             f32(P(DELTA)), nullptr, P(DQKV), 3 * D, at(P(DQKV), D, dt), 3 * D, at(P(DQKV), 2 * D, dt), 3 * D, d.B, d.H, d.L,
                             d.L, dh, attn_scale(dh), attn_premul(dh, dt), P(ATTN_WS), d.ws_bytes, dt, aflags, P(EV_PREP), s));
        record(P(EV_A1), s);
        if (P(ATTN_WS_NEXT) && P(ZERO_STREAM) && P(EV_PREP) && P(EV_CLEAN_OUT)) {
            hipStream_t zs = static_cast<hipStream_t>(P(ZERO_STREAM));
            if (hipStreamWaitEvent(zs, static_cast<hipEvent_t>(P(EV_PREP)), 0) != hipSuccess) return SVOL_E_LAUNCH;
            const int zrc = svol_attn_bwd_zero_ws(P(ATTN_WS_NEXT), d.ws_bytes, d.B, d.H, d.L, d.L, dh, dt, zs);
            if (zrc) return zrc;
            record(P(EV_CLEAN_OUT), zs);
        }
        RUN(nt(P(DQKV), 3 * D, P(W_IN_T), 3 * D, P(DXQ), D, nullptr, nullptr, M, D, 3 * D, dt, s));
        RUN(svol_gate_bwd(f32(P(DS32_2)), P(DXQ), nullptr, f32(P(X32)), P(POS), f32(P(U)), f32(P(G1)), f32(P(A)), f32(P(MEAN1)),
                          f32(P(RSTD1)), f32(P(GATE_WS)), f32(P(GATE_WS2)), f32(P(DX32)), f32(P(DU)), f32(P(DG1)), f32(P(DBT1)), d.B, d.L,
                          D, d.H, dt, s));
    }
    return SVOL_OK;
}

int svol_video_half_wgrad_part(const int64_t* dims, void* const* p, int part, void* s) {
    if (!dims || !p || part < 0 || part > 2) return SVOL_E_INVALID;
    Trace tr_(part == 1 ? "video_half_wgrad.1" : part == 2 ? "video_half_wgrad.2" : "video_half_wgrad", s);
    const Dims d(dims);
    if (!d.ok()) return SVOL_E_INVALID;
    const int64_t M = d.B * d.L, D = d.D, F = d.F;
    const int dt = d.dt;
    const svol_tn_problem pr[5] = {
        {P(DS3), D, P(HID), F, f32(P(DW_FC2)), F, nullptr, M, D, F},
        {P(DPRE), F, P(Y2), D, f32(P(DW_FC1)), D, nullptr, M, F, D},
        {P(G2D), D, P(O), D, f32(P(DW_O)), D, nullptr, M, D, D},
        {P(DQKV), 3 * D, P(Y1POS), D, f32(P(DW_IN)), D, f32(P(DB_IN)), M, 2 * D, D},
        {at(P(DQKV), 2 * D, dt), 3 * D, P(Y1), D, f32(P(DW_IN)) + 2 * D * D, D, f32(P(DB_IN)) + 2 * D, M, D, D}};
    if (part == 1) RUN(svol_gemm_tn_grouped(pr, 3, dt, s));
    else if (part == 2) RUN(svol_gemm_tn_grouped(pr + 3, 2, dt, s));
    else RUN(svol_gemm_tn_grouped(pr, 5, dt, s));
    return SVOL_OK;
}

int svol_video_half_wgrad(const int64_t* dims, void* const* p, void* s) { return svol_video_half_wgrad_part(dims, p, 0, s); }
#undef P

int svol_query_self_fwd(const int64_t* dims, void* const* p, void* s) {
    if (!dims || !p) return SVOL_E_INVALID;
    Trace tr_("query_self_fwd", s);
    const Dims d(dims);
    if (!d.ok() || d.N <= 0) return SVOL_E_INVALID;
    const int64_t R = d.B * d.N, D = d.D, dh = D / d.H;
    const int qdt = d.qdt, xf = qdt != SVOL_F32;
#define P(n) p[SVOL_QS_##n]
    RUN(nt(P(OPOS), D, P(W_IN), D, P(QKV), 3 * D, P(B_IN), P(QSCALE), R, 2 * D, D, qdt, s));
    if (P(WV_HILO))
        RUN(svol_gemm_nt_split(P(O), D, P(WV_HILO), 2 * D, at(P(QKV), 2 * D, qdt), 3 * D, f32(P(B_IN)) + 2 * D, R, D, D, s));
    else
        RUN(nt(P(O), D, at(P(W_IN), 2 * D * D, qdt), D, at(P(QKV), 2 * D, qdt), 3 * D, f32(P(B_IN)) + 2 * D, nullptr, R, D, D, qdt, s));
    RUN(svol_attn_fwd(P(QKV), 3 * D, at(P(QKV), D, qdt), 3 * D, at(P(QKV), 2 * D, qdt), 3 * D, P(OA), D, f32(P(LSE)), nullptr, d.B, d.H,
                      d.N, d.N, dh, attn_scale(dh), attn_premul(dh, qdt), P(ATTN_WS), d.ws_bytes, qdt, s));
    RUN(nt_res(P(OA), D, P(W_O), D, P(S4), P(B_O), P(O32), R, D, D, qdt, s));
    RUN(svol_layernorm_fwd(P(S4), xf, f32(P(G4)), f32(P(BT4)), f32(P(Y32)), P(Y), P(YPOS), P(QPOS), d.N, f32(P(MEAN4)), f32(P(RSTD4)), R, D,
                           0.f, 0, nullptr, qdt, s));
    return SVOL_OK;
}

int svol_query_self_bwd(const int64_t* dims, void* const* p, void* s) {
    if (!dims || !p) return SVOL_E_INVALID;
    Trace tr_("query_self_bwd", s);
    const Dims d(dims);
    if (!d.ok() || d.N <= 0) return SVOL_E_INVALID;
    const int64_t R = d.B * d.N, D = d.D, dh = D / d.H;
    const int qdt = d.qdt, xf = qdt != SVOL_F32;
    RUN(svol_layernorm_bwd(f32(P(DY32)), P(DY), P(DYPOS), P(S4), xf, f32(P(G4)), f32(P(MEAN4)), f32(P(RSTD4)), f32(P(DO32)), P(G),
                           f32(P(DG4)), f32(P(DBT4)), f32(P(DB_O)), R, D, 0.f, 0, nullptr, qdt, s));
    if (P(DQPOS) && P(DYPOS))
        RUN(svol_colsum(P(DYPOS), d.N * D, f32(P(DQPOS)), d.B, d.N * D, qdt, s));
    RUN(nt(P(G), D, P(W_O_T), D, P(DOA), D, nullptr, nullptr, R, D, D, qdt, s));
    RUN(svol_attn_bwd(P(QKV), 3 * D, at(P(QKV), D, qdt), 3 * D, at(P(QKV), 2 * D, qdt), 3 * D, P(OA), D, P(DOA), D, f32(P(LSE)),
                      f32(P(DELTA)), nullptr, P(DQKV), 3 * D, at(P(DQKV), D, qdt), 3 * D, at(P(DQKV), 2 * D, qdt), 3 * D, d.B, d.H, d.N,
                      d.N, dh, attn_scale(dh), attn_premul(dh, qdt), P(ATTN_WS), d.ws_bytes, qdt, s));
    RUN(nt(P(DQKV), 3 * D, P(W_IN_T), 3 * D, P(DXQP), D, nullptr, nullptr, R, D, 2 * D, qdt, s));
    RUN(nt(at(P(DQKV), 2 * D, qdt), 3 * D, at(P(W_IN_T), 2 * D, qdt), 3 * D, P(DXQ), D, nullptr, nullptr, R, D, D, qdt, s));
    return SVOL_OK;
}

int svol_query_self_wgrad(const int64_t* dims, void* const* p, void* s) {
    if (!dims || !p) return SVOL_E_INVALID;
    Trace tr_("query_self_wgrad", s);
    const Dims d(dims);
    if (!d.ok()) return SVOL_E_INVALID;
    const int64_t R = d.B * d.N, D = d.D;
    const int qdt = d.qdt;
    const svol_tn_problem pr[3] = {
        {P(G), D, P(OA), D, f32(P(DW_O)), D, nullptr, R, D, D},
        {P(DQKV), 3 * D, P(OPOS), D, f32(P(DW_IN)), D, f32(P(DB_IN)), R, 2 * D, D},
        {at(P(DQKV), 2 * D, qdt), 3 * D, P(O), D, f32(P(DW_IN)) + 2 * D * D, D, f32(P(DB_IN)) + 2 * D, R, D, D}};
    RUN(svol_gemm_tn_grouped(pr, 3, qdt, s));
    return SVOL_OK;
#undef P
}

int svol_query_cross_fwd(const int64_t* dims, void* const* p, void* s) {
    if (!dims || !p) return SVOL_E_INVALID;
    Trace tr_("query_cross_fwd", s);
    const Dims d(dims);
    if (!d.ok() || d.N <= 0 || d.L <= 0 || d.F <= 0) return SVOL_E_INVALID;
    const int64_t R = d.B * d.N, M = d.B * d.L, D = d.D, F = d.F, dh = D / d.H;
    const int dt = d.dt, qdt = d.qdt, xf = qdt != SVOL_F32;
    const bool mixed = qdt != dt;
#define P(n) p[SVOL_QC_##n]
    if (mixed) {
        RUN(nt(P(OPOS), D, P(W_INQ), D, P(Q), D, P(B_IN), P(QSCALE), R, D, D, qdt, s));
        RUN(svol_cast(P(Q), qdt, P(QC), dt, R * D, s));
    } else {
        RUN(nt(P(OPOS), D, P(W_KV), D, P(QC), D, P(B_IN), P(QSCALE), R, D, D, dt, s));
    }
    RUN(nt(P(MPOS), D, at(P(W_KV), D * D, dt), D, P(KV), 2 * D, f32(P(B_IN)) + D, nullptr, M, D, D, dt, s));
    if (P(WV_HILO))
        RUN(svol_gemm_nt_split(P(MV), D, P(WV_HILO), 2 * D, at(P(KV), D, dt), 2 * D, f32(P(B_IN)) + 2 * D, M, D, D, s));
    else
        RUN(nt(P(MV), D, at(P(W_KV), 2 * D * D, dt), D, at(P(KV), D, dt), 2 * D, f32(P(B_IN)) + 2 * D, nullptr, M, D, D, dt, s));
    RUN(svol_attn_fwd(P(QC), D, P(KV), 2 * D, at(P(KV), D, dt), 2 * D, P(OA), D, f32(P(LSE)), f32(P(KBIAS)), d.B, d.H, d.N, d.L, dh,
                      attn_scale(dh), attn_premul(dh, dt), P(ATTN_WS), d.ws_bytes, dt, s));
    const void* oq = P(OA);
    if (mixed) {
        RUN(svol_cast(P(OA), dt, P(OAQ), qdt, R * D, s));
        oq = P(OAQ);
    }
    RUN(nt_res(oq, D, P(W_O), D, P(S5), P(B_O), P(O32), R, D, D, qdt, s));
    RUN(svol_layernorm_fwd(P(S5), xf, f32(P(G5)), f32(P(BT5)), f32(P(Y5_32)), P(Y5), nullptr, nullptr, 0, f32(P(MEAN5)), f32(P(RSTD5)), R,
                           D, 0.f, 0, nullptr, qdt, s));
    RUN(svol_gemm_nt(P(Y5), D, nullptr, 0, P(W_FC1), D, P(HID), F, f32(P(B_FC1)), nullptr, SVOL_ACT_GELU, P(PRE), F, nullptr, 0, 0, R, F, D,
                     qdt, s));
    RUN(nt_res(P(HID), F, P(W_FC2), F, P(S6), P(B_FC2), P(Y5_32), R, D, F, qdt, s));
    RUN(svol_layernorm_fwd(P(S6), xf, f32(P(G6)), f32(P(BT6)), f32(P(Y32)), P(Y), P(YPOS), P(QPOS), d.N, f32(P(MEAN6)), f32(P(RSTD6)), R, D,
                           0.f, 0, nullptr, qdt, s));
    return SVOL_OK;
}

int svol_query_cross_bwd(const int64_t* dims, void* const* p, void* s) {
    if (!dims || !p) return SVOL_E_INVALID;
    Trace tr_("query_cross_bwd", s);
    const Dims d(dims);
    if (!d.ok() || d.N <= 0 || d.L <= 0 || d.F <= 0) return SVOL_E_INVALID;
    const int64_t R = d.B * d.N, M = d.B * d.L, D = d.D, F = d.F, dh = D / d.H;
    const int dt = d.dt, qdt = d.qdt, xf = qdt != SVOL_F32;
    const bool mixed = qdt != dt;
    RUN(svol_layernorm_bwd(f32(P(DY32)), P(DY), P(DYPOS), P(S6), xf, f32(P(G6)), f32(P(MEAN6)), f32(P(RSTD6)), f32(P(DS32_6)), P(DS6),
                           f32(P(DG6)), f32(P(DBT6)), f32(P(DB_FC2)), R, D, 0.f, 0, nullptr, qdt, s));
    if (P(DQPOS) && P(DYPOS)) RUN(svol_colsum(P(DYPOS), d.N * D, f32(P(DQPOS)), d.B, d.N * D, qdt, s));
    RUN(svol_gemm_nt_dact(P(DS6), D, P(W_FC2_T), D, P(DPRE), F, P(PRE), F, SVOL_ACT_GELU, f32(P(DB_FC1)), R, F, D, qdt, s));
    RUN(nt(P(DPRE), F, P(W_FC1_T), F, P(DY5), D, nullptr, nullptr, R, D, F, qdt, s));
    RUN(svol_layernorm_bwd(f32(P(DS32_6)), P(DY5), nullptr, P(S5), xf, f32(P(G5)), f32(P(MEAN5)), f32(P(RSTD5)), f32(P(DO32)), P(G5D),
                           f32(P(DG5)), f32(P(DBT5)), f32(P(DB_O)), R, D, 0.f, 0, nullptr, qdt, s));
    RUN(nt(P(G5D), D, P(W_O_T), D, P(DOAQ), D, nullptr, nullptr, R, D, D, qdt, s));
    const void* d_o = P(DOAQ);
    if (mixed) {
        RUN(svol_cast(P(DOAQ), qdt, P(DOA), dt, R * D, s));
        d_o = P(DOA);
    }
    RUN(svol_attn_bwd(P(QC), D, P(KV), 2 * D, at(P(KV), D, dt), 2 * D, P(OA), D, d_o, D, f32(P(LSE)), f32(P(DELTA)), f32(P(KBIAS)), P(DQC), D,
                      P(DKV), 2 * D, at(P(DKV), D, dt), 2 * D, d.B, d.H, d.N, d.L, dh, attn_scale(dh), attn_premul(dh, dt), P(ATTN_WS),
                      d.ws_bytes, dt, s));
    if (P(DMPOS)) {
        RUN(nt(P(DKV), 2 * D, at(P(W_KV_T), D, dt), 3 * D, P(DMPOS), D, nullptr, nullptr, M, D, D, dt, s));
        RUN(nt(at(P(DKV), D, dt), 2 * D, at(P(W_KV_T), 2 * D, dt), 3 * D, P(DMV), D, nullptr, nullptr, M, D, D, dt, s));
    } else {
        RUN(nt(P(DKV), 2 * D, at(P(W_KV_T), D, dt), 3 * D, P(DMV), D, nullptr, nullptr, M, D, 2 * D, dt, s));
    }
    const void* dq = P(DQC);
    if (mixed) {
        RUN(svol_cast(P(DQC), dt, P(DQ), qdt, R * D, s));
        dq = P(DQ);
    }
    RUN(nt(dq, D, mixed ? P(W_INQ_T) : P(W_KV_T), 3 * D, P(DXQP), D, nullptr, nullptr, R, D, D, qdt, s));
    return SVOL_OK;
}

int svol_query_cross_wgrad(const int64_t* dims, void* const* p, void* s) {
    if (!dims || !p) return SVOL_E_INVALID;
    Trace tr_("query_cross_wgrad", s);
    const Dims d(dims);
    if (!d.ok()) return SVOL_E_INVALID;
    const int64_t R = d.B * d.N, M = d.B * d.L, D = d.D, F = d.F;
    const int dt = d.dt, qdt = d.qdt;
    const bool mixed = qdt != dt;
    const svol_tn_problem pv[2] = {
        {P(DKV), 2 * D, P(MPOS), D, f32(P(DW_IN)) + D * D, D, f32(P(DB_IN)) + D, M, D, D},
        {at(P(DKV), D, dt), 2 * D, P(MV), D, f32(P(DW_IN)) + 2 * D * D, D, f32(P(DB_IN)) + 2 * D, M, D, D}};
    RUN(svol_gemm_tn_grouped(pv, 2, dt, s));
    const svol_tn_problem pq[4] = {
        {P(DS6), D, P(HID), F, f32(P(DW_FC2)), F, nullptr, R, D, F},
        {P(DPRE), F, P(Y5), D, f32(P(DW_FC1)), D, nullptr, R, F, D},
        {P(G5D), D, mixed ? P(OAQ) : P(OA), D, f32(P(DW_O)), D, nullptr, R, D, D},
        {mixed ? P(DQ) : P(DQC), D, P(OPOS), D, f32(P(DW_IN)), D, f32(P(DB_IN)), R, D, D}};
    RUN(svol_gemm_tn_grouped(pq, 4, qdt, s));
    return SVOL_OK;
#undef P
}

}
```

### svol_amd/csrc/gate.hip

```cpp
#include <cstdlib>

#include "common.h"

namespace {

constexpr int GP = 4;
constexpr int GH = 8;

__device__ __forceinline__ void store_head_sums(const float (&part)[GH], float* __restrict__ scores, int b, int l, int L, int H, int lane) {
    const bool b0 = lane & 1, b1 = lane & 2;
    float h4[4], h2[2];
#pragma unroll
    for (int i = 0; i < 4; ++i) {
        const float send = b0 ? part[i] : part[4 + i], keep = b0 ? part[4 + i] : part[i];
        h4[i] = keep + dpp_f32<0xB1>(send);
    }
#pragma unroll
    for (int i = 0; i < 2; ++i) {
        const float send = b1 ? h4[i] : h4[2 + i], keep = b1 ? h4[2 + i] : h4[i];
        h2[i] = keep + dpp_f32<0x4E>(send);
    }
#pragma unroll
    for (int i = 0; i < 2; ++i) {
        float v = h2[i];
// ... 442 lines not shown
        }
#pragma unroll
        for (int hh = 0; hh < GH; ++hh)
            if (hh < H) sr[hh] = scores[((int64_t)b * H + hh) * L + l];
        dr1 = da[row];
    };
    if (l0 < lend) fetch(l0, xv, pv, dv, sc, dar);
    for (int l = l0; l < lend; ++l) {
        const int64_t row = (int64_t)b * L + l;
        if (l + 1 < lend) fetch(l + 1, nxv, npv, ndv, nsc, ndar);
        float ds[GH];
        const float dal = dar / (float)H;
#pragma unroll
        for (int hh = 0; hh < GH; ++hh) {
            if (hh < H) {
                const float pp = __expf(sc[hh] - mxr[hh]) * isr[hh];
                ds[hh] = pp * (dal - ccr[hh]);
            } else ds[hh] = 0.f;
        }
#pragma unroll
        for (int j = 0; j < NP; ++j) {
            const int c = (lane + 64 * j) * 4;
            if (c < D) {
#pragma unroll
                for (int e = 0; e < 4; ++e) {
                    const float t = xv[j].get(e) + pv[j].get(e);
                    float add = 0.f;
#pragma unroll
                    for (int hh = 0; hh < GH; ++hh) {
                        add += ds[hh] * ur[hh][j][e];
                        dur[hh][j][e] += ds[hh] * t;
                    }
                    dv[j].set(e, dv[j].get(e) + add);
                }
                dv[j].store(dx + row * D + c);
            }
        }
#pragma unroll
        for (int j = 0; j < NP; ++j) { xv[j] = nxv[j]; pv[j] = npv[j]; dv[j] = ndv[j]; }
#pragma unroll
        for (int hh = 0; hh < GH; ++hh) sc[hh] = nsc[hh];
        dar = ndar;
    }
    __shared__ float red[GH * NP * 256];
    for (int w = 0; w < 4; ++w) {
        if (wave == w) {
#pragma unroll
            for (int hh = 0; hh < GH; ++hh)
#pragma unroll
                for (int j = 0; j < NP; ++j) {
                    const int c = (lane + 64 * j) * 4;
#pragma unroll
                    for (int e = 0; e < 4; ++e) {
                        float* r = red + hh * NP * 256 + c + e;
                        if (w == 0) *r = dur[hh][j][e];
                        else *r += dur[hh][j][e];
                    }
                }
        }
        __syncthreads();
    }
    for (int i = threadIdx.x; i < GH * NP * 256; i += 256) {
        const int hh = i / (NP * 256), c = i % (NP * 256);
        if (hh < H && c < D) {
            if (det_du) det_du[(((int64_t)b * gridDim.x + blockIdx.x) * H + hh) * D + c] = red[i];
            else atomicAdd(du + ((int64_t)b * H + hh) * D + c, red[i]);
        }
    }
}

__device__ __forceinline__ void gate_vec_fwd_body(const float* __restrict__ skch, const float* __restrict__ W,
                                                  const float* __restrict__ bias, float* __restrict__ q_out,
                                                  float* __restrict__ u_out, int D, int H) {
    __shared__ float s_q[GP * 256];
    const int hh = blockIdx.x, b = blockIdx.y, tid = threadIdx.x, lane = tid & 63, wave = tid >> 6, dh = D / H;
    float sv[GP][4];
#pragma unroll
    for (int j = 0; j < GP; ++j) {
        const int c = (lane + 64 * j) * 4;
#pragma unroll
        for (int e = 0; e < 4; ++e) sv[j][e] = c < D ? skch[(int64_t)b * D + c + e] : 0.f;
    }
    for (int e = wave; e < dh; e += 4) {
        const int row = hh * dh + e;
        const float* w = W + (int64_t)row * D;
        float acc = 0.f;
#pragma unroll
        for (int j = 0; j < GP; ++j) {
            const int c = (lane + 64 * j) * 4;
            if (c < D) {
                const f32x4 wv = *reinterpret_cast<const f32x4*>(w + c);
                acc += wv[0] * sv[j][0] + wv[1] * sv[j][1] + wv[2] * sv[j][2] + wv[3] * sv[j][3];
            }
        }
        acc = wave_sum(acc) + bias[row];
        if (lane == 0) { s_q[e] = acc; q_out[(int64_t)b * D + row] = acc; }
    }
    __syncthreads();
    const float sc = rsqrtf((float)dh);
    const float* Wk = W + (int64_t)D * D + (int64_t)hh * dh * D;
    for (int c = tid; c < D; c += 256) {
        float acc = 0.f;
        for (int e = 0; e < dh; ++e) acc += s_q[e] * Wk[(int64_t)e * D + c];
        u_out[((int64_t)b * H + hh) * D + c] = acc * sc;
    }
}
__global__ __launch_bounds__(256) void gate_vec_fwd_kernel(const float* skch, const float* W, const float* bias, float* q_out,
                                                           float* u_out, int D, int H) {
    gate_vec_fwd_body(skch, W, bias, q_out, u_out, D, H);
}
__device__ __forceinline__ void gate_vec_bwd_a_body(const float* __restrict__ du, const float* __restrict__ W,
                                                    float* __restrict__ dq_out, int D, int H) {
    const int hh = blockIdx.x, b = blockIdx.y, tid = threadIdx.x, lane = tid & 63, wave = tid >> 6, dh = D / H;
    const float sc = rsqrtf((float)dh);
    float gv[GP][4];
#pragma unroll
    for (int j = 0; j < GP; ++j) {
        const int c = (lane + 64 * j) * 4;
#pragma unroll
        for (int e = 0; e < 4; ++e) gv[j][e] = c < D ? du[((int64_t)b * H + hh) * D + c + e] : 0.f;
    }
    const float* Wk = W + (int64_t)D * D;
    for (int e = wave; e < dh; e += 4) {
        const int row = hh * dh + e;
        const float* w = Wk + (int64_t)row * D;
        float acc = 0.f;
#pragma unroll
        for (int j = 0; j < GP; ++j) {
            const int c = (lane + 64 * j) * 4;
            if (c < D) {
                const f32x4 wv = *reinterpret_cast<const f32x4*>(w + c);
                acc += wv[0] * gv[j][0] + wv[1] * gv[j][1] + wv[2] * gv[j][2] + wv[3] * gv[j][3];
            }
        }
        acc = wave_sum(acc) * sc;
        if (lane == 0) dq_out[(int64_t)b * D + row] = acc;
    }
}
__global__ __launch_bounds__(256) void gate_vec_bwd_a_kernel(const float* du, const float* W, float* dq_out, int D, int H) {
    gate_vec_bwd_a_body(du, W, dq_out, D, H);
}
__device__ __forceinline__ void gate_vec_bwd_b_body(const float* __restrict__ du, const float* __restrict__ skch,
                                                    const float* __restrict__ q, const float* __restrict__ dq,
                                                    const float* __restrict__ W, float* __restrict__ dW,
                                                    float* __restrict__ db, float* __restrict__ dskch, int B, int D, int H) {
    const int tid = threadIdx.x, dh = D / H;
    if ((int)blockIdx.x >= D) {
        const int b = blockIdx.x - D;
        if (!dskch) return;
        __shared__ float s_dq[GP * 256];
        __shared__ float4 s_red[4][GP * 64];
        for (int e = tid; e < D; e += 256) s_dq[e] = dq[(int64_t)b * D + e];
        __syncthreads();
        const int w = tid >> 6, l = tid & 63;
        for (int c = 4 * l, k = l; c < D; c += 256, k += 64) {
            float4 acc = make_float4(0.f, 0.f, 0.f, 0.f);
#pragma unroll 8
            for (int e = w; e < D; e += 4) {
                const float4 wv = *reinterpret_cast<const float4*>(W + (int64_t)e * D + c);
                const float g = s_dq[e];
                acc.x += g * wv.x; acc.y += g * wv.y; acc.z += g * wv.z; acc.w += g * wv.w;
            }
            s_red[w][k] = acc;
        }
        __syncthreads();
        for (int c = tid; c < D; c += 256) {
            const float* r = reinterpret_cast<const float*>(&s_red[0][0]);
            const int stride = GP * 64 * 4;
            dskch[(int64_t)b * D + c] = (r[c] + r[stride + c]) + (r[2 * stride + c] + r[3 * stride + c]);
        }
        return;
    }
    const int e = blockIdx.x, hh = e / dh;
    const float sc = rsqrtf((float)dh);
    for (int c = tid; c < D; c += 256) {
        float aq = 0.f, ak = 0.f;
        for (int b = 0; b < B; ++b) {
            aq += dq[(int64_t)b * D + e] * skch[(int64_t)b * D + c];
            ak += q[(int64_t)b * D + e] * du[((int64_t)b * H + hh) * D + c];
        }
        dW[(int64_t)e * D + c] += aq;
        dW[(int64_t)(D + e) * D + c] += ak * sc;
    }
    if (tid == 0) {
        float bsum = 0.f;
        for (int b = 0; b < B; ++b) bsum += dq[(int64_t)b * D + e];
        db[e] += bsum;
    }
}
__global__ __launch_bounds__(256) void gate_vec_bwd_b_kernel(const float* du, const float* skch, const float* q, const float* dq,
                                                             const float* W, float* dW, float* db, float* dskch, int B, int D, int H) {
    gate_vec_bwd_b_body(du, skch, q, dq, W, dW, db, dskch, B, D, H);
}

struct GateVecMulti {
    const float* du[SVOL_GATE_VEC_MAX_LAYERS];
    const float* W[SVOL_GATE_VEC_MAX_LAYERS];
    const float* bias[SVOL_GATE_VEC_MAX_LAYERS];
    float* q[SVOL_GATE_VEC_MAX_LAYERS];
    float* u[SVOL_GATE_VEC_MAX_LAYERS];
    float* dq[SVOL_GATE_VEC_MAX_LAYERS];
    float* dW[SVOL_GATE_VEC_MAX_LAYERS];
    float* db[SVOL_GATE_VEC_MAX_LAYERS];
    float* dskch[SVOL_GATE_VEC_MAX_LAYERS];
};
__global__ __launch_bounds__(256) void gate_vec_fwd_multi_kernel(const float* skch, GateVecMulti g, int D, int H) {
    const int l = blockIdx.z;
    gate_vec_fwd_body(skch, g.W[l], g.bias[l], g.q[l], g.u[l], D, H);
}
__global__ __launch_bounds__(256) void gate_vec_bwd_a_multi_kernel(GateVecMulti g, int D, int H) {
    const int l = blockIdx.z;
    gate_vec_bwd_a_body(g.du[l], g.W[l], g.dq[l], D, H);
}
__global__ __launch_bounds__(256) void gate_vec_bwd_b_multi_kernel(const float* skch, GateVecMulti g, int B, int D, int H) {
    const int l = blockIdx.z;
    gate_vec_bwd_b_body(g.du[l], skch, g.q[l], g.dq[l], g.W[l], g.dW[l], g.db[l], g.dskch[l], B, D, H);
}

int rows_per_wave(int64_t rows, int64_t target_waves) {
    int64_t r = (rows + target_waves - 1) / target_waves;
    return (int)(r < 1 ? 1 : r);
}
int64_t gate_waves(int which) {
    static const char* names[3] = {"SVOL_GATE_WAVES_SC", "SVOL_GATE_WAVES_LN", "SVOL_GATE_WAVES_AP"};
    static int64_t w[3] = {0, 0, 0};
    if (!w[which]) w[which] = getenv(names[which]) ? atoll(getenv(names[which])) : 4096;
    return w[which] < 64 ? 64 : w[which];
}

}

extern "C" {

static int gate_fwd_impl(const float* x32, const void* pos, const float* u, const float* gamma, const float* beta, float* y32,
                         void* y, void* ypos, float* a, float* mean, float* rstd, float* ws, int64_t B, int64_t L, int64_t D, int64_t H,
                         int dtype, void* stream, bool scored) {
    if (!x32 || !pos || !u || !gamma || !beta || (!y && !y32) || !a || !mean || !rstd || !ws) return SVOL_E_INVALID;
    if (!aligned16(gamma) || !aligned16(beta)) return SVOL_E_INVALID;
    if (B <= 0 || L <= 0 || D <= 0 || H <= 0) return SVOL_E_INVALID;
    if (D % 4 || D > GP * 256 || H > GH || B > 65535 || L > (1 << 24)) return SVOL_E_UNSUPPORTED;
    if (!svol_is16(dtype) && dtype != SVOL_F32) return SVOL_E_INVALID;
    hipStream_t s = reinterpret_cast<hipStream_t>(stream);
    const int np_ = D <= 256 ? 1 : (D <= 512 ? 2 : 4);
    float* scores = ws;
    float* mx = ws + B * H * L;
    float* sm = mx + B * H;
    const int rpw = rows_per_wave(L, gate_waves(0) / B + 1);
    dim3 g1((unsigned)((L + 4 * rpw - 1) / (4 * rpw)), (unsigned)B);
    const int64_t M = B * L;
    const unsigned g3 = (unsigned)((M + 3) / 4);
#define SVOL_GATE_FWD(TT)                                                                                                   \
    do {                                                                                                                    \
        if (scored) { }                                                                                                      \
        else if (np_ == 1) hipLaunchKernelGGL((gate_scores_kernel<TT, 1>), g1, dim3(256), 0, s, x32, (const TT*)pos, u, scores, (int)L, (int)D, (int)H, rpw); \
        else if (np_ == 2) hipLaunchKernelGGL((gate_scores_kernel<TT, 2>), g1, dim3(256), 0, s, x32, (const TT*)pos, u, scores, (int)L, (int)D, (int)H, rpw); \
        else hipLaunchKernelGGL((gate_scores_kernel<TT, 4>), g1, dim3(256), 0, s, x32, (const TT*)pos, u, scores, (int)L, (int)D, (int)H, rpw); \
        hipLaunchKernelGGL(gate_stats_kernel, dim3((unsigned)(B * H)), dim3(256), 0, s, scores, mx, sm, (int)L);            \
        if (np_ == 1) hipLaunchKernelGGL((gate_apply_kernel<TT, 1>), dim3(g3), dim3(256), 0, s, x32, (const TT*)pos, scores, mx, sm, gamma, beta, y32, (TT*)y, (TT*)ypos, a, mean, rstd, (int)L, (int)D, (int)H, M); \
        else if (np_ == 2) hipLaunchKernelGGL((gate_apply_kernel<TT, 2>), dim3(g3), dim3(256), 0, s, x32, (const TT*)pos, scores, mx, sm, gamma, beta, y32, (TT*)y, (TT*)ypos, a, mean, rstd, (int)L, (int)D, (int)H, M); \
        else hipLaunchKernelGGL((gate_apply_kernel<TT, 4>), dim3(g3), dim3(256), 0, s, x32, (const TT*)pos, scores, mx, sm, gamma, beta, y32, (TT*)y, (TT*)ypos, a, mean, rstd, (int)L, (int)D, (int)H, M); \
    } while (0)
    if (dtype == SVOL_BF16) SVOL_GATE_FWD(bf16_t);
    else if (dtype == SVOL_F16) SVOL_GATE_FWD(f16_t);
    else SVOL_GATE_FWD(float);
#undef SVOL_GATE_FWD
    SVOL_CHECK_LAUNCH();
    return SVOL_OK;
}

int svol_gate_fwd(const float* x32, const void* pos, const float* u, const float* gamma, const float* beta, float* y32,
                  void* y, void* ypos, float* a, float* mean, float* rstd, float* ws, int64_t B, int64_t L, int64_t D, int64_t H,
                  int dtype, void* stream) {
    return gate_fwd_impl(x32, pos, u, gamma, beta, y32, y, ypos, a, mean, rstd, ws, B, L, D, H, dtype, stream, false);
}

int svol_gate_fwd_scored(const float* x32, const void* pos, const float* u, const float* gamma, const float* beta, float* y32,
                         void* y, void* ypos, float* a, float* mean, float* rstd, float* ws, int64_t B, int64_t L, int64_t D,
                         int64_t H, int dtype, void* stream) {
    return gate_fwd_impl(x32, pos, u, gamma, beta, y32, y, ypos, a, mean, rstd, ws, B, L, D, H, dtype, stream, true);
}

int svol_layernorm_gate_scores_fwd(const float* x32, const float* gamma, const float* beta, float* y32, void* y, void* ypos,
                                   const void* pos, float* mean, float* rstd, const float* u_next, float* scores_next, int64_t B,
                                   int64_t L, int64_t D, int64_t H, int dtype, void* stream) {
    if (!x32 || !gamma || !beta || (!y && !y32 && !ypos) || !pos || !mean || !rstd || !u_next || !scores_next) return SVOL_E_INVALID;
    if (!aligned16(gamma) || !aligned16(beta) || !aligned16(u_next)) return SVOL_E_INVALID;
    if (B <= 0 || L <= 0 || D <= 0 || H <= 0) return SVOL_E_INVALID;
    if (D % 4 || D > 256 || H > GH || L % 4 || L > (1 << 24) || B > 65535) return SVOL_E_UNSUPPORTED;
    if (!svol_is16(dtype) && dtype != SVOL_F32) return SVOL_E_INVALID;
    hipStream_t s = reinterpret_cast<hipStream_t>(stream);
    const dim3 grid((unsigned)(L / 4), (unsigned)B);
    const size_t lds = (size_t)GH * D * sizeof(float);
#define SVOL_LNS(TT)                                                                                                          \
    hipLaunchKernelGGL((ln_scores_kernel<TT, 1>), grid, dim3(256), lds, s, x32, gamma, beta, y32, (TT*)y, (TT*)ypos,               \
                       (const TT*)pos, mean, rstd, u_next, scores_next, (int)L, (int)D, (int)H)
    if (dtype == SVOL_BF16) SVOL_LNS(bf16_t);
    else if (dtype == SVOL_F16) SVOL_LNS(f16_t);
    else SVOL_LNS(float);
#undef SVOL_LNS
    SVOL_CHECK_LAUNCH();
    return SVOL_OK;
}

int svol_gate_bwd(const float* dy32, const void* dy, const void* dy2, const float* x32, const void* pos, const float* u,
                  const float* gamma, const float* a, const float* mean, const float* rstd, const float* ws, float* ws2,
                  float* dx32, float* du, float* dgamma, float* dbeta, int64_t B, int64_t L, int64_t D, int64_t H, int dtype,
                  void* stream) {
    if ((!dy32 && !dy && !dy2) || !x32 || !pos || !u || !gamma || !a || !mean || !rstd || !ws || !ws2 || !dx32 || !du ||
        !dgamma || !dbeta)
        return SVOL_E_INVALID;
    if (B <= 0 || L <= 0 || D <= 0 || H <= 0) return SVOL_E_INVALID;
    if (D % 4 || D > GP * 256 || H > GH || B > 65535 || L > (1 << 24)) return SVOL_E_UNSUPPORTED;
    if (!svol_is16(dtype) && dtype != SVOL_F32) return SVOL_E_INVALID;
    hipStream_t s = reinterpret_cast<hipStream_t>(stream);
    const int np_ = D <= 256 ? 1 : (D <= 512 ? 2 : 4);
    const float* scores = ws;
    const float* mx = ws + B * H * L;
    const float* sm = mx + B * H;
    float* da = ws2;
    float* cc = ws2 + B * L;
    const int64_t M = B * L;
    const int rpw1 = rows_per_wave(M, gate_waves(1));
    const unsigned g1 = (unsigned)(((M + rpw1 - 1) / rpw1 + 3) / 4);
    const int rpw3 = rows_per_wave(L, gate_waves(2) / B + 1);
    dim3 g3((unsigned)((L + 4 * rpw3 - 1) / (4 * rpw3)), (unsigned)B);
    if (hipMemsetAsync(cc, 0, sizeof(float) * (size_t)(B * H), s) != hipSuccess) return SVOL_E_LAUNCH;
    const bool det_mode = svol_deterministic();
    const size_t n_cc = (size_t)g1 * 4 * (size_t)(B * H), n_gb = (size_t)g1 * 2 * (size_t)D, n_du = (size_t)B * g3.x * (size_t)(H * D);
    DetScratch det(det_mode ? n_cc + n_gb + n_du : 0, s, true);
    if (det_mode && !det.p) return SVOL_E_LAUNCH;
    float* det_cc = det_mode ? det.p : nullptr;
    float* det_gb = det_mode ? det.p + n_cc : nullptr;
    float* det_du = det_mode ? det.p + n_cc + n_gb : nullptr;
#define SVOL_GATE_BWD(TT)                                                                                                   \
    do {                                                                                                                    \
        if (np_ == 1) hipLaunchKernelGGL((gate_bwd_ln_kernel<TT, 1>), dim3(g1), dim3(256), 0, s, dy32, (const TT*)dy, (const TT*)dy2, x32, a, gamma, mean, rstd, dx32, da, dgamma, dbeta, scores, mx, sm, cc, (int)L, (int)H, M, (int)D, rpw1, det_cc, det_gb); \
        else if (np_ == 2) hipLaunchKernelGGL((gate_bwd_ln_kernel<TT, 2>), dim3(g1), dim3(256), 0, s, dy32, (const TT*)dy, (const TT*)dy2, x32, a, gamma, mean, rstd, dx32, da, dgamma, dbeta, scores, mx, sm, cc, (int)L, (int)H, M, (int)D, rpw1, det_cc, det_gb); \
        else hipLaunchKernelGGL((gate_bwd_ln_kernel<TT, 4>), dim3(g1), dim3(256), 0, s, dy32, (const TT*)dy, (const TT*)dy2, x32, a, gamma, mean, rstd, dx32, da, dgamma, dbeta, scores, mx, sm, cc, (int)L, (int)H, M, (int)D, rpw1, det_cc, det_gb); \
        if (det_mode) {                                                                                                     \
            det_fold(det_cc, (int)(g1 * 4), B * H, cc, B * H, s);                                                           \
            det_fold(det_gb, (int)g1, 2 * D, dgamma, D, s);                                                                 \
            det_fold(det_gb + D, (int)g1, 2 * D, dbeta, D, s);                                                              \
        }                                                                                                                   \
        if (np_ == 1) hipLaunchKernelGGL((gate_bwd_apply_kernel<TT, 1>), g3, dim3(256), 0, s, x32, (const TT*)pos, u, scores, mx, sm, da, cc, dx32, du, (int)L, (int)D, (int)H, rpw3, det_du); \
        else if (np_ == 2) hipLaunchKernelGGL((gate_bwd_apply_kernel<TT, 2>), g3, dim3(256), 0, s, x32, (const TT*)pos, u, scores, mx, sm, da, cc, dx32, du, (int)L, (int)D, (int)H, rpw3, det_du); \
        else hipLaunchKernelGGL((gate_bwd_apply_kernel<TT, 4>), g3, dim3(256), 0, s, x32, (const TT*)pos, u, scores, mx, sm, da, cc, dx32, du, (int)L, (int)D, (int)H, rpw3, det_du); \
    } while (0)
    if (dtype == SVOL_BF16) SVOL_GATE_BWD(bf16_t);
    else if (dtype == SVOL_F16) SVOL_GATE_BWD(f16_t);
    else SVOL_GATE_BWD(float);
#undef SVOL_GATE_BWD
    if (det_mode) det_fold(det_du, (int)g3.x, H * D, du, H * D, s, (int)B, (int64_t)g3.x * H * D, H * D);
    SVOL_CHECK_LAUNCH();
    return SVOL_OK;
}

int svol_gate_vectors_fwd(const float* skch, const float* W_in, const float* b_in, float* q_out, float* u_out, int64_t B, int64_t D,
                          int64_t H, void* stream) {
    if (!skch || !W_in || !b_in || !q_out || !u_out || B <= 0 || D <= 0 || H <= 0) return SVOL_E_INVALID;
    if (D % 4 || D > GP * 256 || H > GH || D % H || B > 65535) return SVOL_E_UNSUPPORTED;
    if (!aligned16(W_in)) return SVOL_E_INVALID;
    hipLaunchKernelGGL(gate_vec_fwd_kernel, dim3((unsigned)H, (unsigned)B), dim3(256), 0, reinterpret_cast<hipStream_t>(stream), skch,
                       W_in, b_in, q_out, u_out, (int)D, (int)H);
    SVOL_CHECK_LAUNCH();
    return SVOL_OK;
}

int svol_gate_vectors_bwd(const float* du, const float* skch, const float* W_in, const float* q, float* dq_ws, float* dskch,
                          float* dW_in, float* db_in, int64_t B, int64_t D, int64_t H, void* stream) {
    if (!du || !skch || !W_in || !q || !dq_ws || !dW_in || !db_in || B <= 0 || D <= 0 || H <= 0) return SVOL_E_INVALID;
    if (D % 4 || D > GP * 256 || H > GH || D % H || B > 65535) return SVOL_E_UNSUPPORTED;
    if (!aligned16(W_in)) return SVOL_E_INVALID;
    hipStream_t s = reinterpret_cast<hipStream_t>(stream);
    hipLaunchKernelGGL(gate_vec_bwd_a_kernel, dim3((unsigned)H, (unsigned)B), dim3(256), 0, s, du, W_in, dq_ws, (int)D, (int)H);
    hipLaunchKernelGGL(gate_vec_bwd_b_kernel, dim3((unsigned)(D + B)), dim3(256), 0, s, du, skch, q, dq_ws, W_in, dW_in, db_in, dskch,
                       (int)B, (int)D, (int)H);
    SVOL_CHECK_LAUNCH();
    return SVOL_OK;
}

int svol_gate_vectors_fwd_multi(const float* skch, const float* const* W_in, const float* const* b_in, float* const* q_out,
                                float* const* u_out, int64_t n_layers, int64_t B, int64_t D, int64_t H, void* stream) {
    if (!skch || !W_in || !b_in || !q_out || !u_out || B <= 0 || D <= 0 || H <= 0 || n_layers <= 0) return SVOL_E_INVALID;
    if (D % 4 || D > GP * 256 || H > GH || D % H || B > 65535 || n_layers > SVOL_GATE_VEC_MAX_LAYERS) return SVOL_E_UNSUPPORTED;
    GateVecMulti g{};
    for (int l = 0; l < n_layers; ++l) {
        if (!W_in[l] || !b_in[l] || !q_out[l] || !u_out[l] || !aligned16(W_in[l])) return SVOL_E_INVALID;
        g.W[l] = W_in[l]; g.bias[l] = b_in[l]; g.q[l] = q_out[l]; g.u[l] = u_out[l];
    }
    hipLaunchKernelGGL(gate_vec_fwd_multi_kernel, dim3((unsigned)H, (unsigned)B, (unsigned)n_layers), dim3(256), 0,
                       reinterpret_cast<hipStream_t>(stream), skch, g, (int)D, (int)H);
    SVOL_CHECK_LAUNCH();
    return SVOL_OK;
}

int svol_gate_vectors_bwd_multi(const float* const* du, const float* skch, const float* const* W_in, const float* const* q,
                                float* const* dq_ws, float* const* dskch, float* const* dW_in, float* const* db_in, int64_t n_layers,
                                int64_t B, int64_t D, int64_t H, void* stream) {
    if (!du || !skch || !W_in || !q || !dq_ws || !dW_in || !db_in || B <= 0 || D <= 0 || H <= 0 || n_layers <= 0) return SVOL_E_INVALID;
    if (D % 4 || D > GP * 256 || H > GH || D % H || B > 65535 || n_layers > SVOL_GATE_VEC_MAX_LAYERS) return SVOL_E_UNSUPPORTED;
    GateVecMulti g{};
    for (int l = 0; l < n_layers; ++l) {
        if (!du[l] || !W_in[l] || !q[l] || !dq_ws[l] || !dW_in[l] || !db_in[l] || !aligned16(W_in[l])) return SVOL_E_INVALID;
        g.du[l] = du[l]; g.W[l] = W_in[l]; g.q[l] = const_cast<float*>(q[l]); g.dq[l] = dq_ws[l]; g.dW[l] = dW_in[l]; g.db[l] = db_in[l];
        g.dskch[l] = dskch ? dskch[l] : nullptr;
    }
    hipStream_t s = reinterpret_cast<hipStream_t>(stream);
    hipLaunchKernelGGL(gate_vec_bwd_a_multi_kernel, dim3((unsigned)H, (unsigned)B, (unsigned)n_layers), dim3(256), 0, s, g, (int)D, (int)H);
    hipLaunchKernelGGL(gate_vec_bwd_b_multi_kernel, dim3((unsigned)(D + B), 1, (unsigned)n_layers), dim3(256), 0, s, skch, g, (int)B,
                       (int)D, (int)H);
    SVOL_CHECK_LAUNCH();
    return SVOL_OK;
}

}
```

### svol_amd/csrc/norm.hip

```cpp
#include "common.h"

namespace {

constexpr int LN_MAX_PASSES = 4;

template <typename T, typename TX, int NP>
__global__ __launch_bounds__(256) void ln_fwd_kernel(const TX* __restrict__ x, const float* __restrict__ gamma,
                                                     const float* __restrict__ beta, float* __restrict__ y32,
                                                     T* __restrict__ y, T* __restrict__ ypos, const T* __restrict__ pos,
                                                     int64_t pos_rows, float* __restrict__ mean, float* __restrict__ rstd,
                                                     int64_t M, int D, float p, float inv_keep, uint64_t seed0,
                                                     const int64_t* __restrict__ soff) {
    const uint64_t seed = seed0 + (soff ? ((uint64_t)soff[0] << 8) : 0ull);
    const int lane = threadIdx.x & 63;
    const int64_t row = (int64_t)blockIdx.x * 4 + (threadIdx.x >> 6);
    if (row >= M) return;
    const TX* xr = x + row * D;
    float v[NP][4];
    float s = 0.f;
    const T* pr = pos ? pos + (row % pos_rows) * D : nullptr;
    Vec4<TX> t[NP];
    Vec4<T> pv[NP];
    Vec4<float> gv[NP], bv[NP];
#pragma unroll
    for (int j = 0; j < NP; ++j) {
        const int c = (lane + 64 * j) * 4;
        if (c < D) {
            t[j].load(xr + c);
            if (pr) pv[j].load(pr + c);
            gv[j].load(gamma + c);
            bv[j].load(beta + c);
        }
    }
#pragma unroll
    for (int j = 0; j < NP; ++j) {
        const int c = (lane + 64 * j) * 4;
#pragma unroll
        for (int e = 0; e < 4; ++e) {
            v[j][e] = c < D ? t[j].get(e) : 0.f;
            s += v[j][e];
        }
    }
    const float mu = wave_sum(s) / (float)D;
    float q = 0.f;
#pragma unroll
    for (int j = 0; j < NP; ++j) {
        const int c = (lane + 64 * j) * 4;
        if (c < D) {
#pragma unroll
            for (int e = 0; e < 4; ++e) { const float d = v[j][e] - mu; q += d * d; }
        }
    }
    const float rs = rsqrtf(wave_sum(q) / (float)D + 1e-5f);
    if (lane == 0) { mean[row] = mu; rstd[row] = rs; }
#pragma unroll
    for (int j = 0; j < NP; ++j) {
        const int c = (lane + 64 * j) * 4;
        if (c < D) {
            Vec4<T> o, op;
            Vec4<float> o32;
#pragma unroll
            for (int e = 0; e < 4; ++e) {
                float r = (v[j][e] - mu) * rs * gv[j].get(e) + bv[j].get(e);
                if (p > 0.f) r *= dropout_scale(seed, (uint64_t)row, (uint32_t)(c + e), p, inv_keep);
                o.set(e, r);
                o32.set(e, r);
                if (pr) op.set(e, r + pv[j].get(e));
            }
            if (y32) o32.store(y32 + row * D + c);
            if (y) o.store(y + row * D + c);
            if (ypos) op.store(ypos + row * D + c);
        }
    }
}

template <typename T, typename TX, int NP>
__global__ __launch_bounds__(256) void ln_bwd_kernel(const float* __restrict__ dy32, const T* __restrict__ dy,
                                                     const T* __restrict__ dy2, const TX* __restrict__ x,
                                                     const float* __restrict__ gamma, const float* __restrict__ mean,
                                                     const float* __restrict__ rstd, float* __restrict__ dx32,
                                                     T* __restrict__ dx, float* __restrict__ dgamma,
                                                     float* __restrict__ dbeta, float* __restrict__ dxsum, int64_t M, int D,
                                                     float p, float inv_keep, uint64_t seed0, const int64_t* __restrict__ soff, int rows_per_wave,
                                                     float* __restrict__ det_part) {
    const uint64_t seed = seed0 + (soff ? ((uint64_t)soff[0] << 8) : 0ull);
    const int lane = threadIdx.x & 63;
    const int64_t wave_id = (int64_t)blockIdx.x * 4 + (threadIdx.x >> 6);
    const int64_t r0 = wave_id * rows_per_wave;
    float dg[NP][4], db[NP][4], dxs[NP][4], gm[NP][4];
#pragma unroll
    for (int j = 0; j < NP; ++j) {
        const int c = (lane + 64 * j) * 4;
#pragma unroll
        for (int e = 0; e < 4; ++e) { dg[j][e] = 0.f; db[j][e] = 0.f; dxs[j][e] = 0.f; gm[j][e] = c < D ? gamma[c + e] : 0.f; }
    }
    struct Row { Vec4<float> a32[NP]; Vec4<T> a[NP], b[NP]; Vec4<TX> xv[NP]; float mu, rs; };
    auto fetch = [&](int64_t row, Row& r) {
#pragma unroll
        for (int j = 0; j < NP; ++j) {
            const int c = (lane + 64 * j) * 4;
            if (c < D) {
                if (dy32) r.a32[j].load(dy32 + row * D + c);
                if (dy) r.a[j].load(dy + row * D + c);
                if (dy2) r.b[j].load(dy2 + row * D + c);
                r.xv[j].load(x + row * D + c);
            }
        }
        r.mu = mean[row];
        r.rs = rstd[row];
    };
    const int64_t rend = (r0 + rows_per_wave < M) ? r0 + rows_per_wave : M;
    Row cur, nxt;
    if (r0 < rend) fetch(r0, cur);
    for (int64_t row = r0; row < rend; ++row) {
        if (row + 1 < rend) fetch(row + 1, nxt);
        const float mu = cur.mu, rs = cur.rs;
        float g[NP][4], xh[NP][4];
        float s1 = 0.f, s2 = 0.f;
#pragma unroll
        for (int j = 0; j < NP; ++j) {
            const int c = (lane + 64 * j) * 4;
            if (c < D) {
#pragma unroll
                for (int e = 0; e < 4; ++e) {
                    float d = (dy32 ? cur.a32[j].get(e) : 0.f) + (dy ? cur.a[j].get(e) : 0.f) + (dy2 ? cur.b[j].get(e) : 0.f);
                    if (p > 0.f) d *= dropout_scale(seed, (uint64_t)row, (uint32_t)(c + e), p, inv_keep);
                    const float h = (cur.xv[j].get(e) - mu) * rs;
                    xh[j][e] = h;
                    dg[j][e] += d * h;
                    db[j][e] += d;
                    const float gg = d * gm[j][e];
                    g[j][e] = gg;
                    s1 += gg;
                    s2 += gg * h;
                }
            }
        }
        s1 = wave_sum(s1) / (float)D;
        s2 = wave_sum(s2) / (float)D;
#pragma unroll
        for (int j = 0; j < NP; ++j) {
            const int c = (lane + 64 * j) * 4;
            if (c < D) {
                Vec4<T> o;
                Vec4<float> o32;
#pragma unroll
                for (int e = 0; e < 4; ++e) {
                    const float r = rs * (g[j][e] - s1 - xh[j][e] * s2);
                    dxs[j][e] += r;
                    o.set(e, r);
                    o32.set(e, r);
                }
                if (dx32) o32.store(dx32 + row * D + c);
                if (dx) o.store(dx + row * D + c);
            }
        }
        cur = nxt;
    }
    __shared__ float red[3][NP * 256];
    const int wave = threadIdx.x >> 6;
    for (int w = 0; w < 4; ++w) {
        if (wave == w) {
#pragma unroll
            for (int j = 0; j < NP; ++j) {
                const int c = (lane + 64 * j) * 4;
                if (c < D) {
#pragma unroll
                    for (int e = 0; e < 4; ++e) {
                        if (w == 0) { red[0][c + e] = dg[j][e]; red[1][c + e] = db[j][e]; red[2][c + e] = dxs[j][e]; }
                        else { red[0][c + e] += dg[j][e]; red[1][c + e] += db[j][e]; red[2][c + e] += dxs[j][e]; }
                    }
                }
            }
        }
        __syncthreads();
    }
    if (det_part) {
        float* row = det_part + (int64_t)blockIdx.x * 3 * D;
        for (int c = threadIdx.x; c < D; c += 256) { row[c] = red[0][c]; row[D + c] = red[1][c]; row[2 * D + c] = red[2][c]; }
        return;
    }
    for (int c = threadIdx.x; c < D; c += 256) {
        atomicAdd(dgamma + c, red[0][c]);
        atomicAdd(dbeta + c, red[1][c]);
        if (dxsum) atomicAdd(dxsum + c, red[2][c]);
    }
}

template <typename T>
__global__ __launch_bounds__(256) void posenc_kernel(const float* __restrict__ mask, T* __restrict__ pos, int L, int D) {
    __shared__ float red[2][4];
    __shared__ float xe[64];
    const int b = blockIdx.y, tid = threadIdx.x, lane = tid & 63, wave = tid >> 6;
    const float* mr = mask + (int64_t)b * L;
    const int l0 = blockIdx.x * 64;
    float before = 0.f, all = 0.f;
    for (int l = tid; l < L; l += 256) {
        const float v = (mr[l] != 0.f) ? 1.f : 0.f;
        all += v;
        if (l < l0) before += v;
    }
    before = wave_sum(before);
    all = wave_sum(all);
    if (lane == 0) { red[0][wave] = before; red[1][wave] = all; }
    __syncthreads();
    if (tid == 0) {
        float run = red[0][0] + red[0][1] + red[0][2] + red[0][3];
        const float denom = (red[1][0] + red[1][1] + red[1][2] + red[1][3]) + 1e-6f;
        for (int i = 0; i < 64 && l0 + i < L; ++i) {
            run += (mr[l0 + i] != 0.f) ? 1.f : 0.f;
            xe[i] = run / denom * 6.283185307179586f;
        }
    }
    __syncthreads();
    const int ntok = min(64, L - l0);
    for (int i = tid; i < D; i += 256) {
        const float dim_t = powf(10000.f, (float)(2 * (i / 2)) / (float)D);
        const bool odd = i & 1;
        T* out = pos + ((int64_t)b * L + l0) * D + i;
        if constexpr (sizeof(T) == 4) {
            for (int t = 0; t < ntok; ++t) {
                const float a = xe[t] / dim_t;
                out[(int64_t)t * D] = from_f32<T>(odd ? cosf(a) : sinf(a));
            }
        } else {
            const float inv = 0.15915494309189535f / dim_t;
            for (int t = 0; t < ntok; ++t) {
                const float rev = xe[t] * inv;
                out[(int64_t)t * D] = from_f32<T>(odd ? __builtin_amdgcn_cosf(rev) : __builtin_amdgcn_sinf(rev));
            }
        }
    }
}


template <typename T>
__global__ __launch_bounds__(256) void dropout_kernel(const T* __restrict__ x, T* __restrict__ y, int64_t n, int64_t row_len, float p,
                                                      float inv_keep, uint64_t seed, const int64_t* __restrict__ step) {
    const uint32_t s0 = drop_seed32(drop_seed_at(seed, step));
    int64_t i = ((int64_t)blockIdx.x * blockDim.x + threadIdx.x) * 4;
    const int64_t stride = (int64_t)gridDim.x * blockDim.x * 4;
    for (; i < n; i += stride) {
        int64_t r = i / row_len;
        int64_t k = i - r * row_len;
        uint32_t rm = drop_row(s0, (uint64_t)r);
#pragma unroll
        for (int e = 0; e < 4; ++e) {
            if (i + e >= n) break;
            y[i + e] = from_f32<T>(to_f32(x[i + e]) * drop_scale_rk(rm, (uint32_t)k, p, inv_keep));
            if (++k == row_len) { k = 0; ++r; rm = drop_row(s0, (uint64_t)r); }
        }
    }
}
__global__ __launch_bounds__(256) void dropout_add_kernel(const float* t, const float* res, float* out, int64_t n, int64_t row_len, float p,
                                                          float inv_keep, uint64_t seed, const int64_t* __restrict__ step) {
    const uint32_t s0 = drop_seed32(drop_seed_at(seed, step));
    int64_t i = ((int64_t)blockIdx.x * blockDim.x + threadIdx.x) * 4;
    const int64_t stride = (int64_t)gridDim.x * blockDim.x * 4;
    for (; i < n; i += stride) {
        int64_t r = i / row_len;
        int64_t k = i - r * row_len;
        uint32_t rm = drop_row(s0, (uint64_t)r);
#pragma unroll
        for (int e = 0; e < 4; ++e) {
            if (i + e >= n) break;
            out[i + e] = res[i + e] + t[i + e] * drop_scale_rk(rm, (uint32_t)k, p, inv_keep);
            if (++k == row_len) { k = 0; ++r; rm = drop_row(s0, (uint64_t)r); }
        }
    }
}
}

extern "C" {

int svol_layernorm_fwd(const void* x, int x_f32, const float* gamma, const float* beta, float* y32, void* y,
                       void* ypos, const void* pos, int64_t pos_rows, float* mean, float* rstd, int64_t M, int64_t D,
                       float dropout_p, uint64_t seed, const int64_t* seed_offset_dev, int dtype, void* stream) {
    if (!x || !gamma || !beta || (!y && !y32) || !mean || !rstd || M < 0 || D <= 0) return SVOL_E_INVALID;
    if (!aligned16(gamma) || !aligned16(beta)) return SVOL_E_INVALID;
    if ((ypos != nullptr) != (pos != nullptr)) return SVOL_E_INVALID;
    if (pos && pos_rows <= 0) return SVOL_E_INVALID;
    if (D % 4 || D > LN_MAX_PASSES * 256) return SVOL_E_UNSUPPORTED;
    if (dropout_p < 0.f || dropout_p >= 1.f) return SVOL_E_INVALID;
    if (!svol_is16(dtype) && dtype != SVOL_F32) return SVOL_E_INVALID;
    if (M == 0) return SVOL_OK;
    const float inv_keep = 1.f / (1.f - dropout_p);
    const unsigned grid = (unsigned)((M + 3) / 4);
    hipStream_t s = reinterpret_cast<hipStream_t>(stream);
#define SVOL_LNF(TT, TXX, NPP)                                                                                              \
    hipLaunchKernelGGL((ln_fwd_kernel<TT, TXX, NPP>), dim3(grid), dim3(256), 0, s, (const TXX*)x, gamma, beta, y32, (TT*)y,      \
                       (TT*)ypos, (const TT*)pos, pos_rows, mean, rstd, M, (int)D, dropout_p, inv_keep, seed, seed_offset_dev)
#define SVOL_LNF_NP(TT, TXX)                     \
    do {                                         \
        if (D <= 256) SVOL_LNF(TT, TXX, 1);      \
        else if (D <= 512) SVOL_LNF(TT, TXX, 2); \
        else SVOL_LNF(TT, TXX, 4);               \
    } while (0)
    if (dtype == SVOL_BF16 && x_f32) SVOL_LNF_NP(bf16_t, float);
    else if (dtype == SVOL_BF16) SVOL_LNF_NP(bf16_t, bf16_t);
    else if (dtype == SVOL_F16 && x_f32) SVOL_LNF_NP(f16_t, float);
    else if (dtype == SVOL_F16) SVOL_LNF_NP(f16_t, f16_t);
    else SVOL_LNF_NP(float, float);
#undef SVOL_LNF_NP
#undef SVOL_LNF
    SVOL_CHECK_LAUNCH();
    return SVOL_OK;
}

int svol_layernorm_bwd(const float* dy32, const void* dy, const void* dy2, const void* x, int x_f32, const float* gamma,
                       const float* mean, const float* rstd, float* dx32, void* dx, float* dgamma, float* dbeta,
                       float* dx_colsum, int64_t M, int64_t D, float dropout_p, uint64_t seed, const int64_t* seed_offset_dev,
                       int dtype, void* stream) {
    if ((!dy32 && !dy && !dy2) || !x || !gamma || !mean || !rstd || (!dx && !dx32) || !dgamma || !dbeta || M < 0 || D <= 0)
        return SVOL_E_INVALID;
    if (D % 4 || D > LN_MAX_PASSES * 256) return SVOL_E_UNSUPPORTED;
    if (dropout_p < 0.f || dropout_p >= 1.f) return SVOL_E_INVALID;
    if (!svol_is16(dtype) && dtype != SVOL_F32) return SVOL_E_INVALID;
    if (M == 0) return SVOL_OK;
    const float inv_keep = 1.f / (1.f - dropout_p);
    int64_t rpw = (M + 2047) / 2048;
    if (rpw < 1) rpw = 1;
    const int64_t waves = (M + rpw - 1) / rpw;
    const unsigned grid = (unsigned)((waves + 3) / 4);
    hipStream_t s = reinterpret_cast<hipStream_t>(stream);
    const bool det_mode = svol_deterministic();
    DetScratch det(det_mode ? (size_t)grid * 3 * (size_t)D : 0, s);
    if (det_mode && !det.p) return SVOL_E_LAUNCH;
#define SVOL_LNB(TT, TXX, NPP)                                                                                                      \
    hipLaunchKernelGGL((ln_bwd_kernel<TT, TXX, NPP>), dim3(grid), dim3(256), 0, s, dy32, (const TT*)dy, (const TT*)dy2, (const TXX*)x, \
                       gamma, mean, rstd, dx32, (TT*)dx, dgamma, dbeta, dx_colsum, M, (int)D, dropout_p, inv_keep, seed,              \
                       seed_offset_dev, (int)rpw, det.p)
#define SVOL_LNB_NP(TT, TXX)                  \
    do {                                      \
        if (D <= 256) SVOL_LNB(TT, TXX, 1);   \
        else if (D <= 512) SVOL_LNB(TT, TXX, 2); \
        else SVOL_LNB(TT, TXX, 4);            \
    } while (0)
    if (dtype == SVOL_BF16 && x_f32) SVOL_LNB_NP(bf16_t, float);
    else if (dtype == SVOL_BF16) SVOL_LNB_NP(bf16_t, bf16_t);
    else if (dtype == SVOL_F16 && x_f32) SVOL_LNB_NP(f16_t, float);
    else if (dtype == SVOL_F16) SVOL_LNB_NP(f16_t, f16_t);
    else SVOL_LNB_NP(float, float);
#undef SVOL_LNB_NP
#undef SVOL_LNB
    if (det_mode) {
        det_fold(det.p, (int)grid, 3 * D, dgamma, D, s);
        det_fold(det.p + D, (int)grid, 3 * D, dbeta, D, s);
        det_fold(det.p + 2 * D, (int)grid, 3 * D, dx_colsum, D, s);
    }
    SVOL_CHECK_LAUNCH();
    return SVOL_OK;
}

int svol_dropout_sd(const void* x, void* y, int64_t n, int64_t row_len, float p, uint64_t seed, const int64_t* seed_step_dev, int dtype,
                    void* stream) {
    if (!x || !y || n < 0 || row_len <= 0 || row_len > 0xffffffffll || !(p >= 0.f && p < 1.f)) return SVOL_E_INVALID;
    if (n == 0) return SVOL_OK;
    const float inv = 1.f / (1.f - p);
    int64_t g = (n + 1023) / 1024;
    if (g > 8192) g = 8192;
    hipStream_t s = reinterpret_cast<hipStream_t>(stream);
    if (dtype == SVOL_F32) hipLaunchKernelGGL(dropout_kernel<float>, dim3((unsigned)g), dim3(256), 0, s, (const float*)x, (float*)y, n, row_len, p, inv, seed, seed_step_dev);
    else if (dtype == SVOL_BF16) hipLaunchKernelGGL(dropout_kernel<bf16_t>, dim3((unsigned)g), dim3(256), 0, s, (const bf16_t*)x, (bf16_t*)y, n, row_len, p, inv, seed, seed_step_dev);
    else if (dtype == SVOL_F16) hipLaunchKernelGGL(dropout_kernel<f16_t>, dim3((unsigned)g), dim3(256), 0, s, (const f16_t*)x, (f16_t*)y, n, row_len, p, inv, seed, seed_step_dev);
    else return SVOL_E_INVALID;
    SVOL_CHECK_LAUNCH();
    return SVOL_OK;
}

int svol_dropout(const void* x, void* y, int64_t n, int64_t row_len, float p, uint64_t seed, int dtype, void* stream) {
    return svol_dropout_sd(x, y, n, row_len, p, seed, nullptr, dtype, stream);
}

int svol_dropout_add_sd(const float* t32, const float* res32, float* out32, int64_t n, int64_t row_len, float p, uint64_t seed,
                        const int64_t* seed_step_dev, void* stream) {
    if (!t32 || !res32 || !out32 || n < 0 || row_len <= 0 || row_len > 0xffffffffll || !(p >= 0.f && p < 1.f)) return SVOL_E_INVALID;
    if (n == 0) return SVOL_OK;
    int64_t g = (n + 1023) / 1024;
    if (g > 8192) g = 8192;
    hipLaunchKernelGGL(dropout_add_kernel, dim3((unsigned)g), dim3(256), 0, reinterpret_cast<hipStream_t>(stream), t32, res32, out32, n,
                       row_len, p, 1.f / (1.f - p), seed, seed_step_dev);
    SVOL_CHECK_LAUNCH();
    return SVOL_OK;
}
int svol_dropout_add(const float* t32, const float* res32, float* out32, int64_t n, int64_t row_len, float p, uint64_t seed, void* stream) {
    return svol_dropout_add_sd(t32, res32, out32, n, row_len, p, seed, nullptr, stream);
}

int svol_posenc_sine(const float* mask, void* pos, int64_t B, int64_t L, int64_t D, int dtype, void* stream) {
    if (!mask || !pos || B <= 0 || L <= 0 || D <= 0) return SVOL_E_INVALID;
    if (L > (1 << 24) || D > 4096) return SVOL_E_UNSUPPORTED;
    hipStream_t s = reinterpret_cast<hipStream_t>(stream);
    if (B > 65535) return SVOL_E_UNSUPPORTED;
    dim3 grid((unsigned)((L + 63) / 64), (unsigned)B);
    if (dtype == SVOL_BF16)
        hipLaunchKernelGGL(posenc_kernel<bf16_t>, grid, dim3(256), 0, s, mask, (bf16_t*)pos, (int)L, (int)D);
    else if (dtype == SVOL_F16)
        hipLaunchKernelGGL(posenc_kernel<f16_t>, grid, dim3(256), 0, s, mask, (f16_t*)pos, (int)L, (int)D);
    else if (dtype == SVOL_F32)
        hipLaunchKernelGGL(posenc_kernel<float>, grid, dim3(256), 0, s, mask, (float*)pos, (int)L, (int)D);
    else return SVOL_E_INVALID;
    SVOL_CHECK_LAUNCH();
    return SVOL_OK;
}

}
```

### svol_amd/modeling/cross_modal_transformer.py

```python
from __future__ import annotations

import copy
import os

import torch
from torch import nn

from .. import _lib, blocks, layers, ops
from ..params import GradGroup, claim, weights

D_FF = 2048


class MLP(nn.Module):

    def __init__(self, in_features, hidden_features):
        super().__init__()
        self.fc1 = nn.Linear(in_features, hidden_features)
        self.fc2 = nn.Linear(hidden_features, in_features)


OVERLAP_QUERY_STREAM = os.environ.get('SVOL_NO_STREAM_OVERLAP') is None
QUERY_FP32 = os.environ.get('SVOL_QUERY_BF16') is None
_SIDE = {}


def _side_stream(dev):
    s = _SIDE.get(dev)
    if s is None:
        s = _SIDE[dev] = torch.cuda.Stream(device=dev)
        try:
            torch.autograd.graph.set_warn_on_accumulate_grad_stream_mismatch(False)
        except AttributeError:
            pass
    return s


def side_streams(dev):
    return [s for d, s in _SIDE.items() if d == dev]


class _GateVectorsFn(torch.autograd.Function):

    @staticmethod
    def forward(ctx, skch, W_in, b_in, h):
        B, d = skch.shape
        skch = skch.contiguous().float()
        q = torch.empty((B, d), dtype=torch.float32, device=skch.device)
        u = torch.empty((B, h, d), dtype=torch.float32, device=skch.device)
        Wd, bd = W_in.detach(), b_in.detach()
        rc = _lib.lib().svol_gate_vectors_fwd(ops._ptr(skch), ops._ptr(Wd), ops._ptr(bd), ops._ptr(q), ops._ptr(u), B, d, h, ops._stream())
        _lib.check(rc, 'svol_gate_vectors_fwd')
        ctx.save_for_backward(skch, W_in, q)
        ctx.h = h
        ctx.sinks = (claim(W_in, ctx.needs_input_grad[1]), claim(b_in, ctx.needs_input_grad[2]))
        return u

    @staticmethod
    def backward(ctx, du):
        skch, W_in, q = ctx.saved_tensors
        h = ctx.h
        B, d = skch.shape
        sW, sb = ctx.sinks
        du = du.contiguous().float()
        dev = du.device
        gW, gb = GradGroup(((sW, (3 * d, d)),), dev), GradGroup(((sb, (3 * d,)),), dev)
        dskch = torch.empty((B, d), dtype=torch.float32, device=dev) if ctx.needs_input_grad[0] else None
        ws = torch.empty((B, d), dtype=torch.float32, device=dev)
        rc = _lib.lib().svol_gate_vectors_bwd(ops._ptr(du), ops._ptr(skch), ops._ptr(W_in.detach()), ops._ptr(q), ops._ptr(ws),
                                              ops._ptr(dskch), ops._ptr(gW.out[0]), ops._ptr(gb.out[0]), B, d, h, ops._stream())
        _lib.check(rc, 'svol_gate_vectors_bwd')
        return (dskch,) + gW.finish() + gb.finish() + (None,)


def _ptr_array(tensors):
    import ctypes
    return (ctypes.c_void_p * len(tensors))(*[None if t is None else t.data_ptr() for t in tensors])


class _GateVectorsAllFn(torch.autograd.Function):

    @staticmethod
    def forward(ctx, skch, h, *params):
        B, d = skch.shape
        n = len(params) // 2
        skch = skch.contiguous().float()
        dev = skch.device
        Ws, bs = params[0::2], params[1::2]
        q = torch.empty((n, B, d), dtype=torch.float32, device=dev)
        us = [torch.empty((B, h, d), dtype=torch.float32, device=dev) for _ in range(n)]
        rc = _lib.lib().svol_gate_vectors_fwd_multi(ops._ptr(skch), _ptr_array([w.detach() for w in Ws]), _ptr_array([b.detach() for b in bs]),
                                                    _ptr_array(list(q.unbind(0))), _ptr_array(us), n, B, d, h, ops._stream())
        _lib.check(rc, 'svol_gate_vectors_fwd_multi')
        ctx.save_for_backward(skch, q, *Ws)
        ctx.h, ctx.n = h, n
        ctx.sinks = [(claim(Ws[l], ctx.needs_input_grad[2 + 2 * l]), claim(bs[l], ctx.needs_input_grad[3 + 2 * l])) for l in range(n)]
        return tuple(us)

    @staticmethod
    def backward(ctx, *dus):
        skch, q = ctx.saved_tensors[:2]
        Ws = ctx.saved_tensors[2:]
        h, n = ctx.h, ctx.n
        B, d = skch.shape
        dev = skch.device
        dus = [torch.zeros((B, h, d), dtype=torch.float32, device=dev) if g is None else g.contiguous().float() for g in dus]
        gWs = [GradGroup(((sW, (3 * d, d)),), dev) for sW, _ in ctx.sinks]
        gbs = [GradGroup(((sb, (3 * d,)),), dev) for _, sb in ctx.sinks]
        ws = torch.empty((n, B, d), dtype=torch.float32, device=dev)
        dsk = torch.empty((n, B, d), dtype=torch.float32, device=dev) if ctx.needs_input_grad[0] else None
        rc = _lib.lib().svol_gate_vectors_bwd_multi(_ptr_array(dus), ops._ptr(skch), _ptr_array([w.detach() for w in Ws]),
                                                    _ptr_array(list(q.unbind(0))), _ptr_array(list(ws.unbind(0))),
                                                    None if dsk is None else _ptr_array(list(dsk.unbind(0))), _ptr_array([g.out[0] for g in gWs]),
                                                    _ptr_array([g.out[0] for g in gbs]), n, B, d, h, ops._stream())
        _lib.check(rc, 'svol_gate_vectors_bwd_multi')
        grads = [None if dsk is None else dsk.sum(0), None]
        for gW, gb in zip(gWs, gbs):
            grads += gW.finish() + gb.finish()
        return tuple(grads)


GATE_VECTORS_MULTI_MAX = 8


def all_gate_vectors(layers, skch):
    import os
    if len(layers) > GATE_VECTORS_MULTI_MAX or len(layers) < 2 or os.environ.get('SVOL_GATE_VEC_PER_LAYER') is not None:
        return [layer.gate_vectors(skch) for layer in layers]
    params = []
    for layer in layers:
        a = layer.sketch_video_cross_attn
        params += [a.in_proj_weight, a.in_proj_bias]
    return list(_GateVectorsAllFn.apply(skch, layers[0].nhead, *params))


class CrossModalTransformerLayer(nn.Module):
    def __init__(self, d_model=512, nhead=8, dim_feedforward=D_FF):
        super().__init__()
        self.sketch_video_cross_attn = nn.MultiheadAttention(d_model, nhead)
        self.norm1 = nn.LayerNorm(d_model)
        self.content_self_attn = nn.MultiheadAttention(d_model, nhead)
        self.norm2 = nn.LayerNorm(d_model)
        self.mlp1 = MLP(d_model, dim_feedforward)
        self.norm3 = nn.LayerNorm(d_model)
        self.token_self_attn = nn.MultiheadAttention(d_model, nhead)
        self.norm4 = nn.LayerNorm(d_model)
        self.content_token_cross_attn = nn.MultiheadAttention(d_model, nhead)
        self.norm5 = nn.LayerNorm(d_model)
        self.mlp2 = MLP(d_model, dim_feedforward)
        self.norm6 = nn.LayerNorm(d_model)
        self.d_model, self.nhead = d_model, nhead

    def gate_vectors(self, skch):
        m = self.sketch_video_cross_attn
        return _GateVectorsFn.apply(skch, m.in_proj_weight, m.in_proj_bias, self.nhead)

    def forward(self, mem32, skch32, out, pos, qpos, kbias, u=None):
        m32, m, mpos = self.video_half(mem32, skch32, pos, u)
        return m32, self.query_half(out, m, mpos, qpos, kbias)

    def video_half(self, mem32, skch32, pos, u=None, u_next=None, sc_in=None):
        if blocks.ENABLED:
            uu = self.gate_vectors(skch32) if u is None else u
            m32, m, mpos, sc = blocks.video_half(self, mem32, pos, uu, pos.dtype, u_next, sc_in)
            return (m32, m, mpos) if u_next is None else (m32, m, mpos, sc)
        assert sc_in is None
        h = self.nhead
        n = lambda m: (m.weight, m.bias)
        mha = lambda m: (m.in_proj_weight, m.in_proj_bias, m.out_proj.weight, m.out_proj.bias)
        mlp = lambda m: (m.fc1.weight, m.fc1.bias, m.fc2.weight, m.fc2.bias)
        m32, m, mpos = layers.gate(mem32, pos, self.gate_vectors(skch32) if u is None else u, *n(self.norm1), h)
        m32, m = layers.self_attn_ln(m32, m, mpos, *mha(self.content_self_attn), *n(self.norm2), None, h)
        return layers.mlp_ln(m32, m, *mlp(self.mlp1), *n(self.norm3), pos)

    def query_half(self, out, m, mpos, qpos, kbias):
        return self.query_cross(self.query_self(out, qpos, m.dtype), m, mpos, qpos, kbias)

    def query_self(self, out, qpos, dt=None):
        if blocks.ENABLED:
            return blocks.query_self(self, out, qpos, dt if dt is not None else qpos.dtype, qpos.dtype)
        n = lambda m_: (m_.weight, m_.bias)
        mha = lambda m_: (m_.in_proj_weight, m_.in_proj_bias, m_.out_proj.weight, m_.out_proj.bias)
        o32, o, opos = out
        return layers.self_attn_ln(o32, o, opos, *mha(self.token_self_attn), *n(self.norm4), qpos, self.nhead)

    def query_cross(self, out, m, mpos, qpos, kbias):
        n = lambda m_: (m_.weight, m_.bias)
        mha = lambda m_: (m_.in_proj_weight, m_.in_proj_bias, m_.out_proj.weight, m_.out_proj.bias)
        mlp = lambda m_: (m_.fc1.weight, m_.fc1.bias, m_.fc2.weight, m_.fc2.bias)
        if blocks.ENABLED:
            return blocks.query_cross(self, out, m, mpos, kbias, qpos, m.dtype, qpos.dtype)
        o32, o, opos = out
        o32, o = layers.cross_attn_ln(o32, o, opos, mpos, m, *mha(self.content_token_cross_attn), *n(self.norm5), None, self.nhead,
                                   kbias)
        return layers.mlp_ln(o32, o, *mlp(self.mlp2), *n(self.norm6), qpos)


class CrossModalTransformer(nn.Module):
    def __init__(self, d_model=512, nhead=8, num_layers=6, dim_feedforward=D_FF):
        super().__init__()
        layer = CrossModalTransformerLayer(d_model, nhead, dim_feedforward)
        self.layers = nn.ModuleList([copy.deepcopy(layer) for _ in range(num_layers)])
        for p in self.parameters():
            if p.dim() > 1:
                nn.init.xavier_uniform_(p)
        self.d_model, self.nhead, self.num_layers = d_model, nhead, num_layers
        self._epoch_seen = -1

    def forward(self, src_vid32, src_skch32, kbias, vid_pos, query_embed, us=None):
        if weights.epoch == self._epoch_seen:
            weights.new_epoch()
        self._epoch_seen = weights.epoch
        B = src_vid32.shape[0]
        dt = torch.float32 if QUERY_FP32 else vid_pos.dtype
        qpos = layers.cast_ag(query_embed, dt)
        N, d = qpos.shape
        def initial_queries():
            return (torch.zeros((B, N, d), dtype=torch.float32, device=vid_pos.device),
                    torch.zeros((B, N, d), dtype=dt, device=vid_pos.device),
                    qpos.unsqueeze(0).expand(B, -1, -1).contiguous())
        mem32 = src_vid32
        outputs = []
        if us is None:
            us = all_gate_vectors(list(self.layers), src_skch32)
        if not OVERLAP_QUERY_STREAM:
            out = initial_queries()
            for layer, u in zip(self.layers, us):
                mem32, out = layer(mem32, src_skch32, out, vid_pos, qpos, kbias, u)
                outputs.append(out[0])
            return torch.stack(outputs)
        main = torch.cuda.current_stream()
        side = _side_stream(main.device)
        side.wait_stream(main)
        qpos.record_stream(side)
        kbias.record_stream(side)
        with torch.cuda.stream(side):
            out = initial_queries()
        sc = None
        for li, (layer, u) in enumerate(zip(self.layers, us)):
            with torch.cuda.stream(side):
                out_sa = layer.query_self(out, qpos, vid_pos.dtype)
            if blocks.ENABLED and blocks.GATE_SCORES_FUSE and li + 1 < len(us):
                m32, m, mpos, sc = layer.video_half(mem32, src_skch32, vid_pos, u, us[li + 1], sc)
            elif sc is not None:
                m32, m, mpos = layer.video_half(mem32, src_skch32, vid_pos, u, None, sc)
            else:
                m32, m, mpos = layer.video_half(mem32, src_skch32, vid_pos, u)
            side.wait_stream(main)
            m.record_stream(side)
            mpos.record_stream(side)
            with torch.cuda.stream(side):
                out = layer.query_cross(out_sa, m, mpos, qpos, kbias)
                outputs.append(out[0])
            mem32 = m32
        main.wait_stream(side)
        for t in outputs:
            t.record_stream(main)
        return torch.stack(outputs)


def build_cross_modal_transformer(args):
    return CrossModalTransformer(d_model=args.hidden_dim, nhead=args.nheads, num_layers=args.num_layers,
                                 dim_feedforward=D_FF)
```

Measured before the change: 15290.

## Defer gate backward apply pass into next layer's LayerNorm backward kernel

Splits the gate backward into a partial pass (LN grads, dgamma/dbeta) and an apply pass that adds the gate-score contribution to dx and du. The apply pass is deferred across layers and fused into the following (earlier) layer's first LayerNorm backward kernel through a link object. That kernel reads the deferred gate workspaces and accumulates du. The goal is to drop one full read/write pass over the activation gradient per layer boundary. In exchange it adds deferral bookkeeping, pointer/key matching with a flush fallback, and a non-deterministic-only path with atomics.

```diff
diff --git a/include/svol_hip.h b/include/svol_hip.h
--- a/include/svol_hip.h
+++ b/include/svol_hip.h
@@ -155,6 +155,16 @@
                   const float* u, const float* gamma, const float* a, const float* mean, const float* rstd,
                   const float* ws, float* ws2, float* dx32, float* du, float* dgamma, float* dbeta, int64_t B,
                   int64_t L, int64_t D, int64_t H, int dtype, void* stream);
+int svol_gate_bwd_partial(const float* dy32, const void* dy, const void* dy2, const float* x32, const float* gamma,
+                          const float* a, const float* mean, const float* rstd, const float* ws, float* ws2, float* dx32,
+                          float* dgamma, float* dbeta, int64_t B, int64_t L, int64_t D, int64_t H, int dtype, void* stream);
+int svol_gate_bwd_apply(const float* x32, const void* pos, const float* u, const float* ws, const float* ws2, float* dx32,
+                        float* du, int64_t B, int64_t L, int64_t D, int64_t H, int dtype, void* stream);
+int svol_layernorm_bwd_gate(const float* dy32, const void* dy, const void* dy2, const float* x32, const float* gamma,
+                            const float* beta, const float* mean, const float* rstd, float* dx32, void* dx, float* dgamma,
+                            float* dbeta, float* dx_colsum, const void* pos, const float* u, const float* gate_ws,
+                            const float* gate_ws2, float* du, int64_t B, int64_t L, int64_t D, int64_t H, int dtype,
+                            void* stream);
 
 int svol_layernorm_gate_scores_fwd(const float* x32, const float* gamma, const float* beta, float* y32, void* y, void* ypos,
                                    const void* pos, float* mean, float* rstd, const float* u_next, float* scores_next,
@@ -305,7 +315,8 @@
     X(DM32) X(DM) X(DMPOS) X(DS32_3) X(DS3) X(DPRE) X(DY2) X(DS32_2) X(G2D) X(DO) X(DQKV) X(DELTA) X(DXQP) X(DXQ) X(GATE_WS2) \
     X(DX32) X(DU) \
     X(DG1) X(DBT1) X(DG2) X(DBT2) X(DG3) X(DBT3) X(DW_IN) X(DB_IN) X(DW_O) X(DB_O) X(DW_FC1) X(DB_FC1) X(DW_FC2) X(DB_FC2) \
-    X(EV_A0) X(EV_A1) X(EV_CLEAN_IN) X(EV_PREP) X(ATTN_WS_NEXT) X(ZERO_STREAM) X(EV_CLEAN_OUT)
+    X(EV_A0) X(EV_A1) X(EV_CLEAN_IN) X(EV_PREP) X(ATTN_WS_NEXT) X(ZERO_STREAM) X(EV_CLEAN_OUT) \
+    X(GATE_BWD_DEFER) X(DEFER_WS) X(DEFER_WS2) X(DEFER_U) X(DEFER_DU) X(DEFER_POS)
 #define SVOL_QS_SLOTS(X) \
     X(O32) X(O) X(OPOS) X(QPOS) X(B_IN) X(B_O) X(G4) X(BT4) X(QSCALE) X(W_IN) X(WV_HILO) X(W_O) X(W_IN_T) X(W_O_T) \
     X(QKV) X(OA) X(LSE) X(S4) X(MEAN4) X(RSTD4) X(Y32) X(Y) X(YPOS) X(ATTN_WS) \
diff --git a/svol_amd/_lib.py b/svol_amd/_lib.py
--- a/svol_amd/_lib.py
+++ b/svol_amd/_lib.py
@@ -116,6 +116,9 @@
     'svol_gate_fwd': [_p, _p, _p, _p, _p, _p, _p, _p, _p, _p, _p, _p, _i64, _i64, _i64, _i64, _int, _p],
     'svol_gate_bwd': [_p, _p, _p, _p, _p, _p, _p, _p, _p, _p, _p, _p, _p, _p, _p, _p, _i64, _i64, _i64, _i64, _int,
                       _p],
+    'svol_gate_bwd_partial': [_p, _p, _p, _p, _p, _p, _p, _p, _p, _p, _p, _p, _p, _i64, _i64, _i64, _i64, _int, _p],
+    'svol_gate_bwd_apply': [_p, _p, _p, _p, _p, _p, _p, _i64, _i64, _i64, _i64, _int, _p],
+    'svol_layernorm_bwd_gate': [_p] * 18 + [_i64, _i64, _i64, _i64, _int, _p],
     'svol_clock_probe': [_p, _p, _int, _p, _i64, _i64, _p, _p],
     'svol_gate_fwd_scored': [_p, _p, _p, _p, _p, _p, _p, _p, _p, _p, _p, _p, _i64, _i64, _i64, _i64, _int, _p],
     'svol_layernorm_gate_scores_fwd': [_p, _p, _p, _p, _p, _p, _p, _p, _p, _p, _p, _i64, _i64, _i64, _i64, _int, _p],
diff --git a/svol_amd/blocks.py b/svol_amd/blocks.py
--- a/svol_amd/blocks.py
+++ b/svol_amd/blocks.py
@@ -11,6 +11,7 @@
 
 ENABLED = os.environ.get('SVOL_NO_BLOCKS') is None
 GATE_SCORES_FUSE = os.environ.get('SVOL_GATE_SCORES_FUSE') is not None
+GATE_BWD_DEFER = True
 VH, QS, QC = 0, 1, 2
 _F32, _BF16 = 0, 1
 _ESZ = {torch.float32: 4, torch.bfloat16: 2, torch.float16: 2}
@@ -348,6 +349,52 @@
     return st or None
 
 
+def gate_bwd_deferrable(D, H, deterministic=None, enabled=None, defer=None):
+    deterministic = (os.environ.get('SVOL_DETERMINISTIC') is not None) if deterministic is None else deterministic
+    enabled = ENABLED if enabled is None else enabled
+    defer = GATE_BWD_DEFER if defer is None else defer
+    return bool(defer and enabled and not deterministic and D % 4 == 0 and D <= 256 and H <= 8)
+
+
+def gate_defer_pairs(n_layers, D, H, us_from_all, **state):
+    if n_layers < 2 or not us_from_all or not gate_bwd_deferrable(D, H, **state):
+        return None
+    return [GateDeferLink() for _ in range(n_layers - 1)]
+
+
+class GateDeferLink:
+
+    __slots__ = ('pending',)
+
+    def __init__(self):
+        self.pending = None
+
+    def pend(self, dx32_ptr, key, slots, apply_fn, keep):
+        if self.pending is not None:
+            self.flush()
+        self.pending = (dx32_ptr, key, slots, apply_fn, keep)
+
+    def take(self, dm32_ptr, key):
+        p = self.pending
+        if p is None:
+            return None
+        if dm32_ptr is not None and dm32_ptr == p[0] and key == p[1]:
+            self.pending = None
+            return p[2], p[4]
+        self.flush()
+        return None
+
+    def flush(self):
+        p, self.pending = self.pending, None
+        if p is not None:
+            p[3]()
+
+
+def flush_gate_defer(links):
+    for ln in links or ():
+        ln.flush()
+
+
 def _vh_fwd_layout(B, L, D, H, F, e):
     M = B * L
     return [('Y1', M * D * e), ('Y1POS', M * D * e), ('A', M * 4), ('MEAN1', M * 4), ('RSTD1', M * 4), ('GATE_WS', B * H * (L + 2) * 4),
@@ -371,7 +418,7 @@
 class VideoHalfFn(torch.autograd.Function):
 
     @staticmethod
-    def forward(ctx, pl, x32, pos, u, u_next, sc_in, *params):
+    def forward(ctx, pl, x32, pos, u, u_next, sc_in, defer, *params):
         B, L, D = x32.shape
         layer = pl.layer()
         H, F = layer.nhead, layer.mlp1.fc1.weight.shape[0]
@@ -406,6 +453,7 @@
         tbl.set('GATE_WS_NEXT', None)
         ctx.shape = (B, L, D, H, F)
         ctx.sc_in = sc_in
+        ctx.defer_out, ctx.defer_in = defer if defer is not None else (None, None)
         ctx.save_for_backward(x2, pos2, u)
         ctx.mark_non_differentiable(sc_next)
         return (lay.view(ctx.arena, 'M32', torch.float32, (B, L, D)), lay.view(ctx.arena, 'M', dt, (B, L, D)),
@@ -414,38 +462,62 @@
     @staticmethod
     def backward(ctx, dm32, dm, dmpos, _dsc=None):
         if dm32 is None and dm is None and dmpos is None:
-            return _no_grads(ctx, 6)
+            if ctx.defer_in is not None:
+                ctx.defer_in.flush()
+            return _no_grads(ctx, 7)
         tbl = ctx.tbl
         B, L, D, H, F = ctx.shape
         dt = ctx.pl.dt
-        dev = ctx.saved_tensors[0].device
+        x2, pos2, u = ctx.saved_tensors
+        dev = x2.device
         du = torch.zeros((B, H, D), dtype=torch.float32, device=dev)
         tbl.set('DU', du.data_ptr())
         lay, tmp, bufs, gs = _open_bwd(ctx, dev, lambda: _vh_bwd_layout(B, L, D, H, F, _ESZ[dt]), DM32=dm32, DM=dm, DMPOS=dmpos)
+        dkey = (B, L, D, H, dt, ops._stream())
+        taken = ctx.defer_in.take(gs[0].data_ptr() if dm32 is not None else None, dkey) if ctx.defer_in is not None else None
+        for n_, ptr in (taken[0] if taken else {}).items():
+            tbl.set(n_, ptr)
         _call('svol_video_half_bwd', ctx, 1)
+        for n_ in (taken[0] if taken else ()):
+            tbl.set(n_, None)
+        taken = None
         wgrad.attn_backward(B * H * L * L)
         _attn_events(tbl, _maybe_events('attn_bwd', (B, H, L, L, D // H)))
         pz = _dq_prezero(dev, B, H, L, D // H, dt, ctx.dims[8]) if ctx.big else None
         if pz is not None:
             pz.bind(tbl)
+        link = ctx.defer_out
+        tbl.set('GATE_BWD_DEFER', du.data_ptr() if link is not None else None)
         _call('svol_video_half_bwd', ctx, 2)
+        tbl.set('GATE_BWD_DEFER', None)
         if pz is not None:
             pz.advance(tbl)
         _attn_events(tbl, None)
-        pg = _close_bwd(ctx, 'svol_video_half_wgrad', bufs, [ctx.arena, tmp] + gs, 6)
+        pg = _close_bwd(ctx, 'svol_video_half_wgrad', bufs, [ctx.arena, tmp] + gs, 7)
         dx32 = lay.view(tmp, 'DX32', torch.float32, (B, L, D))
-        return (None, dx32, None, du if ctx.needs_input_grad[3] else None, None, None) + pg
+        if link is not None:
+            ptr = {n_: tbl.arr[tbl.idx[n_]] for n_ in ('GATE_WS', 'GATE_WS2', 'DX32')}
+            dims = (B, L, D, H, ops._DT[dt])
+
+            def apply_fn(x_=x2.data_ptr(), p_=pos2.data_ptr(), u_=u.data_ptr(), du_=du.data_ptr()):
+                rc = _lib.lib().svol_gate_bwd_apply(x_, p_, u_, ptr['GATE_WS'], ptr['GATE_WS2'], ptr['DX32'], du_, *dims, ops._stream())
+                _lib.check(rc, 'svol_gate_bwd_apply')
+
+            link.pend(ptr['DX32'], dkey,
+                      {'DEFER_WS': ptr['GATE_WS'], 'DEFER_WS2': ptr['GATE_WS2'], 'DEFER_U': u.data_ptr(), 'DEFER_DU': du.data_ptr(),
+                       'DEFER_POS': pos2.data_ptr()}, apply_fn, [ctx.arena, ctx.sc_in, tmp, x2, pos2, u, du])
+        return (None, dx32, None, du if ctx.needs_input_grad[3] else None, None, None, None) + pg
 
 
 def gate_scores_fusable(L, D, H):
     return GATE_SCORES_FUSE and L % 4 == 0 and D % 4 == 0 and D <= 256 and H <= 8
 
 
-def video_half(layer, x32, pos, u, dt, u_next=None, sc_in=None):
+def video_half(layer, x32, pos, u, dt, u_next=None, sc_in=None, defer=None):
     pl = plan(layer, VH, dt, dt)
     if u_next is not None and not gate_scores_fusable(x32.shape[1], x32.shape[2], layer.nhead):
         u_next = None
-    m32, m, mpos, sc = VideoHalfFn.apply(pl, x32, pos, u, u_next, sc_in, *pl.inputs(x32, u))
+    m32, m, mpos, sc = VideoHalfFn.apply(pl, x32, pos, u, u_next, sc_in, defer, *pl.inputs(x32, u))
     return m32, m, mpos, (sc if u_next is not None else None)
 
 
diff --git a/svol_amd/csrc/blocks.hip b/svol_amd/csrc/blocks.hip
--- a/svol_amd/csrc/blocks.hip
+++ b/svol_amd/csrc/blocks.hip
@@ -201,8 +201,13 @@
     const int64_t M = d.B * d.L, D = d.D, F = d.F, dh = D / d.H;
     const int dt = d.dt, xf = dt != SVOL_F32;
     if (phase != 2) {
-        RUN(svol_layernorm_bwd(f32(P(DM32)), P(DM), P(DMPOS), P(S3), xf, f32(P(G3)), f32(P(MEAN3)), f32(P(RSTD3)), f32(P(DS32_3)), P(DS3),
-                               f32(P(DG3)), f32(P(DBT3)), f32(P(DB_FC2)), M, D, 0.f, 0, nullptr, dt, s));
+        if (P(DEFER_WS) || P(DEFER_WS2) || P(DEFER_U) || P(DEFER_DU) || P(DEFER_POS))
+            RUN(svol_layernorm_bwd_gate(f32(P(DM32)), P(DM), P(DMPOS), f32(P(S3)), f32(P(G3)), f32(P(BT3)), f32(P(MEAN3)), f32(P(RSTD3)),
+                                        f32(P(DS32_3)), P(DS3), f32(P(DG3)), f32(P(DBT3)), f32(P(DB_FC2)), P(DEFER_POS), f32(P(DEFER_U)),
+                                        f32(P(DEFER_WS)), f32(P(DEFER_WS2)), f32(P(DEFER_DU)), d.B, d.L, D, d.H, dt, s));
+        else
+            RUN(svol_layernorm_bwd(f32(P(DM32)), P(DM), P(DMPOS), P(S3), xf, f32(P(G3)), f32(P(MEAN3)), f32(P(RSTD3)), f32(P(DS32_3)), P(DS3),
+                                   f32(P(DG3)), f32(P(DBT3)), f32(P(DB_FC2)), M, D, 0.f, 0, nullptr, dt, s));
         RUN(svol_gemm_nt_dact(P(DS3), D, P(W_FC2_T), D, P(DPRE), F, P(PRE), F, SVOL_ACT_GELU_D, f32(P(DB_FC1)), M, F, D, dt, s));
         RUN(nt(P(DPRE), F, P(W_FC1_T), F, P(DY2), D, nullptr, nullptr, M, D, F, dt, s));
         RUN(svol_layernorm_bwd(f32(P(DS32_3)), P(DY2), nullptr, P(S2), xf, f32(P(G2)), f32(P(MEAN2)), f32(P(RSTD2)), f32(P(DS32_2)), P(G2D),
@@ -228,9 +233,13 @@
             record(P(EV_CLEAN_OUT), zs);
         }
         RUN(nt(P(DQKV), 3 * D, P(W_IN_T), 3 * D, P(DXQ), D, nullptr, nullptr, M, D, 3 * D, dt, s));
-        RUN(svol_gate_bwd(f32(P(DS32_2)), P(DXQ), nullptr, f32(P(X32)), P(POS), f32(P(U)), f32(P(G1)), f32(P(A)), f32(P(MEAN1)),
-                          f32(P(RSTD1)), f32(P(GATE_WS)), f32(P(GATE_WS2)), f32(P(DX32)), f32(P(DU)), f32(P(DG1)), f32(P(DBT1)), d.B, d.L,
-                          D, d.H, dt, s));
+        if (P(GATE_BWD_DEFER))
+            RUN(svol_gate_bwd_partial(f32(P(DS32_2)), P(DXQ), nullptr, f32(P(X32)), f32(P(G1)), f32(P(A)), f32(P(MEAN1)), f32(P(RSTD1)),
+                                      f32(P(GATE_WS)), f32(P(GATE_WS2)), f32(P(DX32)), f32(P(DG1)), f32(P(DBT1)), d.B, d.L, D, d.H, dt, s));
+        else
+            RUN(svol_gate_bwd(f32(P(DS32_2)), P(DXQ), nullptr, f32(P(X32)), P(POS), f32(P(U)), f32(P(G1)), f32(P(A)), f32(P(MEAN1)),
+                              f32(P(RSTD1)), f32(P(GATE_WS)), f32(P(GATE_WS2)), f32(P(DX32)), f32(P(DU)), f32(P(DG1)), f32(P(DBT1)), d.B, d.L,
+                              D, d.H, dt, s));
     }
     return SVOL_OK;
 }
diff --git a/svol_amd/csrc/gate.hip b/svol_amd/csrc/gate.hip
--- a/svol_amd/csrc/gate.hip
+++ b/svol_amd/csrc/gate.hip
@@ -768,13 +768,10 @@
     return SVOL_OK;
 }
 
-int svol_gate_bwd(const float* dy32, const void* dy, const void* dy2, const float* x32, const void* pos, const float* u,
-                  const float* gamma, const float* a, const float* mean, const float* rstd, const float* ws, float* ws2,
-                  float* dx32, float* du, float* dgamma, float* dbeta, int64_t B, int64_t L, int64_t D, int64_t H, int dtype,
-                  void* stream) {
-    if ((!dy32 && !dy && !dy2) || !x32 || !pos || !u || !gamma || !a || !mean || !rstd || !ws || !ws2 || !dx32 || !du ||
-        !dgamma || !dbeta)
-        return SVOL_E_INVALID;
+static int gate_bwd_impl(const float* dy32, const void* dy, const void* dy2, const float* x32, const void* pos, const float* u,
+                         const float* gamma, const float* a, const float* mean, const float* rstd, const float* ws, float* ws2,
+                         float* dx32, float* du, float* dgamma, float* dbeta, int64_t B, int64_t L, int64_t D, int64_t H, int dtype,
+                         void* stream, int passes) {
     if (B <= 0 || L <= 0 || D <= 0 || H <= 0) return SVOL_E_INVALID;
     if (D % 4 || D > GP * 256 || H > GH || B > 65535 || L > (1 << 24)) return SVOL_E_UNSUPPORTED;
     if (!svol_is16(dtype) && dtype != SVOL_F32) return SVOL_E_INVALID;
@@ -790,35 +787,75 @@
     const unsigned g1 = (unsigned)(((M + rpw1 - 1) / rpw1 + 3) / 4);
     const int rpw3 = rows_per_wave(L, gate_waves(2) / B + 1);
     dim3 g3((unsigned)((L + 4 * rpw3 - 1) / (4 * rpw3)), (unsigned)B);
-    if (hipMemsetAsync(cc, 0, sizeof(float) * (size_t)(B * H), s) != hipSuccess) return SVOL_E_LAUNCH;
     const bool det_mode = svol_deterministic();
-    const size_t n_cc = (size_t)g1 * 4 * (size_t)(B * H), n_gb = (size_t)g1 * 2 * (size_t)D, n_du = (size_t)B * g3.x * (size_t)(H * D);
-    DetScratch det(det_mode ? n_cc + n_gb + n_du : 0, s, true);
-    if (det_mode && !det.p) return SVOL_E_LAUNCH;
-    float* det_cc = det_mode ? det.p : nullptr;
-    float* det_gb = det_mode ? det.p + n_cc : nullptr;
-    float* det_du = det_mode ? det.p + n_cc + n_gb : nullptr;
-#define SVOL_GATE_BWD(TT)                                                                                                   \
+    if (passes & 1) {
+        if (hipMemsetAsync(cc, 0, sizeof(float) * (size_t)(B * H), s) != hipSuccess) return SVOL_E_LAUNCH;
+        const size_t n_cc = (size_t)g1 * 4 * (size_t)(B * H), n_gb = (size_t)g1 * 2 * (size_t)D;
+        DetScratch det(det_mode ? n_cc + n_gb : 0, s, true);
+        if (det_mode && !det.p) return SVOL_E_LAUNCH;
+        float* det_cc = det_mode ? det.p : nullptr;
+        float* det_gb = det_mode ? det.p + n_cc : nullptr;
+#define SVOL_GATE_BWD1(TT)                                                                                                  \
     do {                                                                                                                    \
         if (np_ == 1) hipLaunchKernelGGL((gate_bwd_ln_kernel<TT, 1>), dim3(g1), dim3(256), 0, s, dy32, (const TT*)dy, (const TT*)dy2, x32, a, gamma, mean, rstd, dx32, da, dgamma, dbeta, scores, mx, sm, cc, (int)L, (int)H, M, (int)D, rpw1, det_cc, det_gb); \
         else if (np_ == 2) hipLaunchKernelGGL((gate_bwd_ln_kernel<TT, 2>), dim3(g1), dim3(256), 0, s, dy32, (const TT*)dy, (const TT*)dy2, x32, a, gamma, mean, rstd, dx32, da, dgamma, dbeta, scores, mx, sm, cc, (int)L, (int)H, M, (int)D, rpw1, det_cc, det_gb); \
         else hipLaunchKernelGGL((gate_bwd_ln_kernel<TT, 4>), dim3(g1), dim3(256), 0, s, dy32, (const TT*)dy, (const TT*)dy2, x32, a, gamma, mean, rstd, dx32, da, dgamma, dbeta, scores, mx, sm, cc, (int)L, (int)H, M, (int)D, rpw1, det_cc, det_gb); \
-        if (det_mode) {                                                                                                     \
-            det_fold(det_cc, (int)(g1 * 4), B * H, cc, B * H, s);                                                           \
-            det_fold(det_gb, (int)g1, 2 * D, dgamma, D, s);                                                                 \
-            det_fold(det_gb + D, (int)g1, 2 * D, dbeta, D, s);                                                              \
-        }                                                                                                                   \
+    } while (0)
+        if (dtype == SVOL_BF16) SVOL_GATE_BWD1(bf16_t);
+        else if (dtype == SVOL_F16) SVOL_GATE_BWD1(f16_t);
+        else SVOL_GATE_BWD1(float);
+#undef SVOL_GATE_BWD1
+        if (det_mode) {
+            det_fold(det_cc, (int)(g1 * 4), B * H, cc, B * H, s);
+            det_fold(det_gb, (int)g1, 2 * D, dgamma, D, s);
+            det_fold(det_gb + D, (int)g1, 2 * D, dbeta, D, s);
+        }
+    }
+    if (passes & 2) {
+        const size_t n_du = (size_t)B * g3.x * (size_t)(H * D);
+        DetScratch det(det_mode ? n_du : 0, s, true);
+        if (det_mode && !det.p) return SVOL_E_LAUNCH;
+        float* det_du = det_mode ? det.p : nullptr;
+#define SVOL_GATE_BWD3(TT)                                                                                                  \
+    do {                                                                                                                    \
         if (np_ == 1) hipLaunchKernelGGL((gate_bwd_apply_kernel<TT, 1>), g3, dim3(256), 0, s, x32, (const TT*)pos, u, scores, mx, sm, da, cc, dx32, du, (int)L, (int)D, (int)H, rpw3, det_du); \
         else if (np_ == 2) hipLaunchKernelGGL((gate_bwd_apply_kernel<TT, 2>), g3, dim3(256), 0, s, x32, (const TT*)pos, u, scores, mx, sm, da, cc, dx32, du, (int)L, (int)D, (int)H, rpw3, det_du); \
         else hipLaunchKernelGGL((gate_bwd_apply_kernel<TT, 4>), g3, dim3(256), 0, s, x32, (const TT*)pos, u, scores, mx, sm, da, cc, dx32, du, (int)L, (int)D, (int)H, rpw3, det_du); \
     } while (0)
-    if (dtype == SVOL_BF16) SVOL_GATE_BWD(bf16_t);
-    else if (dtype == SVOL_F16) SVOL_GATE_BWD(f16_t);
-    else SVOL_GATE_BWD(float);
-#undef SVOL_GATE_BWD
-    if (det_mode) det_fold(det_du, (int)g3.x, H * D, du, H * D, s, (int)B, (int64_t)g3.x * H * D, H * D);
+        if (dtype == SVOL_BF16) SVOL_GATE_BWD3(bf16_t);
+        else if (dtype == SVOL_F16) SVOL_GATE_BWD3(f16_t);
+        else SVOL_GATE_BWD3(float);
+#undef SVOL_GATE_BWD3
+        if (det_mode) det_fold(det_du, (int)g3.x, H * D, du, H * D, s, (int)B, (int64_t)g3.x * H * D, H * D);
+    }
     SVOL_CHECK_LAUNCH();
     return SVOL_OK;
+}
+
+int svol_gate_bwd(const float* dy32, const void* dy, const void* dy2, const float* x32, const void* pos, const float* u,
+                  const float* gamma, const float* a, const float* mean, const float* rstd, const float* ws, float* ws2,
+                  float* dx32, float* du, float* dgamma, float* dbeta, int64_t B, int64_t L, int64_t D, int64_t H, int dtype,
+                  void* stream) {
+    if ((!dy32 && !dy && !dy2) || !x32 || !pos || !u || !gamma || !a || !mean || !rstd || !ws || !ws2 || !dx32 || !du ||
+        !dgamma || !dbeta)
+        return SVOL_E_INVALID;
+    return gate_bwd_impl(dy32, dy, dy2, x32, pos, u, gamma, a, mean, rstd, ws, ws2, dx32, du, dgamma, dbeta, B, L, D, H, dtype, stream, 3);
+}
+
+int svol_gate_bwd_partial(const float* dy32, const void* dy, const void* dy2, const float* x32, const float* gamma, const float* a,
+                          const float* mean, const float* rstd, const float* ws, float* ws2, float* dx32, float* dgamma,
+                          float* dbeta, int64_t B, int64_t L, int64_t D, int64_t H, int dtype, void* stream) {
+    if ((!dy32 && !dy && !dy2) || !x32 || !gamma || !a || !mean || !rstd || !ws || !ws2 || !dx32 || !dgamma || !dbeta)
+        return SVOL_E_INVALID;
+    return gate_bwd_impl(dy32, dy, dy2, x32, nullptr, nullptr, gamma, a, mean, rstd, ws, ws2, dx32, nullptr, dgamma, dbeta, B, L, D, H,
+                         dtype, stream, 1);
+}
+
+int svol_gate_bwd_apply(const float* x32, const void* pos, const float* u, const float* ws, const float* ws2, float* dx32, float* du,
+                        int64_t B, int64_t L, int64_t D, int64_t H, int dtype, void* stream) {
+    if (!x32 || !pos || !u || !ws || !ws2 || !dx32 || !du) return SVOL_E_INVALID;
+    return gate_bwd_impl(nullptr, nullptr, nullptr, x32, pos, u, nullptr, nullptr, nullptr, nullptr, ws, const_cast<float*>(ws2), dx32, du,
+                         nullptr, nullptr, B, L, D, H, dtype, stream, 2);
 }
 
 int svol_gate_vectors_fwd(const float* skch, const float* W_in, const float* b_in, float* q_out, float* u_out, int64_t B, int64_t D,
diff --git a/svol_amd/csrc/norm.hip b/svol_amd/csrc/norm.hip
--- a/svol_amd/csrc/norm.hip
+++ b/svol_amd/csrc/norm.hip
@@ -184,6 +184,157 @@
         atomicAdd(dgamma + c, red[0][c]);
         atomicAdd(dbeta + c, red[1][c]);
         if (dxsum) atomicAdd(dxsum + c, red[2][c]);
+    }
+}
+
+constexpr int LNG_H = 8;
+template <typename T>
+__global__ __launch_bounds__(256) void ln_bwd_gate_kernel(const float* __restrict__ dy32, const T* __restrict__ dy,
+                                                          const T* __restrict__ dy2, const float* __restrict__ x,
+                                                          const float* __restrict__ gamma, const float* __restrict__ beta,
+                                                          const float* __restrict__ mean, const float* __restrict__ rstd,
+                                                          float* __restrict__ dx32, T* __restrict__ dx, float* __restrict__ dgamma,
+                                                          float* __restrict__ dbeta, float* __restrict__ dxsum,
+                                                          const T* __restrict__ pos, const float* __restrict__ u,
+                                                          const float* __restrict__ scores, const float* __restrict__ mx,
+                                                          const float* __restrict__ sm, const float* __restrict__ da,
+                                                          const float* __restrict__ cc, float* __restrict__ du, int L, int D, int H,
+                                                          int rpw) {
+    __shared__ __attribute__((aligned(16))) float su[LNG_H * 256];
+    __shared__ float red[3][256];
+    const int tid = threadIdx.x, lane = tid & 63, wave = tid >> 6;
+    const int b = blockIdx.y;
+    const int l0 = (blockIdx.x * 4 + wave) * rpw;
+    const int lend = min(l0 + rpw, L);
+    const int c = lane * 4;
+    for (int i = tid * 4; i < LNG_H * 256; i += 1024) {
+        const int hh = i >> 8, cc_ = i & 255;
+        f32x4 w = f32x4{0.f, 0.f, 0.f, 0.f};
+        if (hh < H && cc_ < D) w = *reinterpret_cast<const f32x4*>(u + ((int64_t)b * H + hh) * D + cc_);
+        *reinterpret_cast<f32x4*>(su + i) = w;
+    }
+    float dg[4], db[4], dxs[4], gm[4], bt[4], dur[LNG_H][4];
+#pragma unroll
+    for (int e = 0; e < 4; ++e) {
+        dg[e] = 0.f; db[e] = 0.f; dxs[e] = 0.f;
+        gm[e] = c < D ? gamma[c + e] : 0.f;
+        bt[e] = c < D ? beta[c + e] : 0.f;
+#pragma unroll
+        for (int hh = 0; hh < LNG_H; ++hh) dur[hh][e] = 0.f;
+    }
+    float mxl = 0.f, isl = 0.f, ccl = 0.f;
+    if (lane < H) { mxl = mx[b * H + lane]; isl = 1.f / sm[b * H + lane]; ccl = cc[b * H + lane]; }
+    __syncthreads();
+    struct Row { Vec4<float> a32, xv; Vec4<T> a, b, pv; float mu, rs, dar, sc; };
+    auto fetch = [&](int l, Row& r) {
+        const int64_t row = (int64_t)b * L + l;
+        if (c < D) {
+            r.a32.load(dy32 + row * D + c);
+            if (dy) r.a.load(dy + row * D + c);
+            if (dy2) r.b.load(dy2 + row * D + c);
+            r.xv.load(x + row * D + c);
+            r.pv.load(pos + row * D + c);
+        }
+        r.mu = mean[row];
+        r.rs = rstd[row];
+        r.dar = da[row];
+        r.sc = lane < H ? scores[((int64_t)b * H + lane) * L + l] : 0.f;
+    };
+    Row cur, nxt;
+    if (l0 < lend) fetch(l0, cur);
+    for (int l = l0; l < lend; ++l) {
+        const int64_t row = (int64_t)b * L + l;
+        if (l + 1 < lend) fetch(l + 1, nxt);
+        const float mu = cur.mu, rs = cur.rs;
+        const float dal = cur.dar / (float)H;
+        float dsl = 0.f;
+        if (lane < H) {
+            const float pp = __expf(cur.sc - mxl) * isl;
+            dsl = pp * (dal - ccl);
+        }
+        float ds[LNG_H];
+#pragma unroll
+        for (int hh = 0; hh < LNG_H; ++hh)
+            ds[hh] = __builtin_bit_cast(float, __builtin_amdgcn_readlane(__builtin_bit_cast(int, dsl), hh));
+        float g[4], xh[4];
+        float s1 = 0.f, s2 = 0.f;
+        if (c < D) {
+            float t[4], add[4];
+#pragma unroll
+            for (int e = 0; e < 4; ++e) {
+                xh[e] = (cur.xv.get(e) - mu) * rs;
+                t[e] = xh[e] * gm[e] + bt[e] + cur.pv.get(e);
+                add[e] = 0.f;
+            }
+#pragma unroll
+            for (int hh = 0; hh < LNG_H; ++hh) {
+                const f32x4 ur = *reinterpret_cast<const f32x4*>(su + hh * 256 + c);
+#pragma unroll
+                for (int e = 0; e < 4; ++e) {
+                    add[e] += ds[hh] * ur[e];
+                    dur[hh][e] += ds[hh] * t[e];
+                }
+            }
+#pragma unroll
+            for (int e = 0; e < 4; ++e) {
+                const float h = xh[e];
+                const float d = (cur.a32.get(e) + add[e]) + (dy ? cur.a.get(e) : 0.f) + (dy2 ? cur.b.get(e) : 0.f);
+                dg[e] += d * h;
+                db[e] += d;
+                const float gg = d * gm[e];
+                g[e] = gg;
+                s1 += gg;
+                s2 += gg * h;
+            }
+        }
+        s1 = wave_sum(s1) / (float)D;
+        s2 = wave_sum(s2) / (float)D;
+        if (c < D) {
+            Vec4<T> o;
+            Vec4<float> o32;
+#pragma unroll
+            for (int e = 0; e < 4; ++e) {
+                const float r = rs * (g[e] - s1 - xh[e] * s2);
+                dxs[e] += r;
+                o.set(e, r);
+                o32.set(e, r);
+            }
+            if (dx32) o32.store(dx32 + row * D + c);
+            if (dx) o.store(dx + row * D + c);
+        }
+        cur = nxt;
+    }
+    for (int w = 0; w < 4; ++w) {
+        if (wave == w && c < D) {
+#pragma unroll
+            for (int e = 0; e < 4; ++e) {
+                if (w == 0) { red[0][c + e] = dg[e]; red[1][c + e] = db[e]; red[2][c + e] = dxs[e]; }
+                else { red[0][c + e] += dg[e]; red[1][c + e] += db[e]; red[2][c + e] += dxs[e]; }
+            }
+        }
+        __syncthreads();
+    }
+    for (int i = tid; i < D; i += 256) {
+        atomicAdd(dgamma + i, red[0][i]);
+        atomicAdd(dbeta + i, red[1][i]);
+        if (dxsum) atomicAdd(dxsum + i, red[2][i]);
+    }
+    for (int w = 0; w < 4; ++w) {
+        if (wave == w) {
+#pragma unroll
+            for (int hh = 0; hh < LNG_H; ++hh)
+#pragma unroll
+                for (int e = 0; e < 4; ++e) {
+                    float* r = su + hh * 256 + c + e;
+                    if (w == 0) *r = dur[hh][e];
+                    else *r += dur[hh][e];
+                }
+        }
+        __syncthreads();
+    }
+    for (int i = tid; i < LNG_H * 256; i += 256) {
+        const int hh = i >> 8, cc_ = i & 255;
+        if (hh < H && cc_ < D) atomicAdd(du + ((int64_t)b * H + hh) * D + cc_, su[i]);
     }
 }
 
@@ -352,6 +503,38 @@
     return SVOL_OK;
 }
 
+int svol_layernorm_bwd_gate(const float* dy32, const void* dy, const void* dy2, const float* x32, const float* gamma,
+                            const float* beta, const float* mean, const float* rstd, float* dx32, void* dx, float* dgamma,
+                            float* dbeta, float* dx_colsum, const void* pos, const float* u, const float* gate_ws,
+                            const float* gate_ws2, float* du, int64_t B, int64_t L, int64_t D, int64_t H, int dtype, void* stream) {
+    if (!dy32 || !x32 || !gamma || !beta || !mean || !rstd || (!dx && !dx32) || !dgamma || !dbeta || !pos || !u || !gate_ws ||
+        !gate_ws2 || !du)
+        return SVOL_E_INVALID;
+    if (B <= 0 || L <= 0 || D <= 0 || H <= 0) return SVOL_E_INVALID;
+    if (!aligned16(u)) return SVOL_E_INVALID;
+    if (D % 4 || D > 256 || H > LNG_H || B > 65535 || L > (1 << 24) || svol_deterministic()) return SVOL_E_UNSUPPORTED;
+    if (!svol_is16(dtype) && dtype != SVOL_F32) return SVOL_E_INVALID;
+    const int64_t per_b = 2048 / B > 0 ? 2048 / B : 1;
+    const int64_t rpw = (L + per_b - 1) / per_b;
+    const dim3 grid((unsigned)((L + 4 * rpw - 1) / (4 * rpw)), (unsigned)B);
+    const float* scores = gate_ws;
+    const float* mx = gate_ws + B * H * L;
+    const float* sm = mx + B * H;
+    const float* da = gate_ws2;
+    const float* cc = gate_ws2 + B * L;
+    hipStream_t s = reinterpret_cast<hipStream_t>(stream);
+#define SVOL_LNBG(TT)                                                                                                              \
+    hipLaunchKernelGGL((ln_bwd_gate_kernel<TT>), grid, dim3(256), 0, s, dy32, (const TT*)dy, (const TT*)dy2, x32, gamma, beta, mean, \
+                       rstd, dx32, (TT*)dx, dgamma, dbeta, dx_colsum, (const TT*)pos, u, scores, mx, sm, da, cc, du, (int)L, (int)D,  \
+                       (int)H, (int)rpw)
+    if (dtype == SVOL_BF16) SVOL_LNBG(bf16_t);
+    else if (dtype == SVOL_F16) SVOL_LNBG(f16_t);
+    else SVOL_LNBG(float);
+#undef SVOL_LNBG
+    SVOL_CHECK_LAUNCH();
+    return SVOL_OK;
+}
+
 int svol_dropout_sd(const void* x, void* y, int64_t n, int64_t row_len, float p, uint64_t seed, const int64_t* seed_step_dev, int dtype,
                     void* stream) {
     if (!x || !y || n < 0 || row_len <= 0 || row_len > 0xffffffffll || !(p >= 0.f && p < 1.f)) return SVOL_E_INVALID;
diff --git a/svol_amd/modeling/cross_modal_transformer.py b/svol_amd/modeling/cross_modal_transformer.py
--- a/svol_amd/modeling/cross_modal_transformer.py
+++ b/svol_amd/modeling/cross_modal_transformer.py
@@ -104,6 +104,9 @@
         h, n = ctx.h, ctx.n
         B, d = skch.shape
         dev = skch.device
+        for links in getattr(ctx, 'gate_defer_links', ()):
+            blocks.flush_gate_defer(links)
+        ctx.gate_defer_links = []
         dus = [torch.zeros((B, h, d), dtype=torch.float32, device=dev) if g is None else g.contiguous().float() for g in dus]
         gWs = [GradGroup(((sW, (3 * d, d)),), dev) for sW, _ in ctx.sinks]
         gbs = [GradGroup(((sb, (3 * d,)),), dev) for _, sb in ctx.sinks]
@@ -132,6 +135,14 @@
         a = layer.sketch_video_cross_attn
         params += [a.in_proj_weight, a.in_proj_bias]
     return list(_GateVectorsAllFn.apply(skch, layers[0].nhead, *params))
+
+
+def gate_vectors_node(us):
+    fns = {id(u.grad_fn): u.grad_fn for u in us}
+    if len(fns) != 1:
+        return None
+    fn = next(iter(fns.values()))
+    return fn if isinstance(fn, _GateVectorsAllFn._backward_cls) else None
 
 
 class CrossModalTransformerLayer(nn.Module):
@@ -159,10 +170,10 @@
         m32, m, mpos = self.video_half(mem32, skch32, pos, u)
         return m32, self.query_half(out, m, mpos, qpos, kbias)
 
-    def video_half(self, mem32, skch32, pos, u=None, u_next=None, sc_in=None):
+    def video_half(self, mem32, skch32, pos, u=None, u_next=None, sc_in=None, defer=None):
         if blocks.ENABLED:
             uu = self.gate_vectors(skch32) if u is None else u
-            m32, m, mpos, sc = blocks.video_half(self, mem32, pos, uu, pos.dtype, u_next, sc_in)
+            m32, m, mpos, sc = blocks.video_half(self, mem32, pos, uu, pos.dtype, u_next, sc_in, defer)
             return (m32, m, mpos) if u_next is None else (m32, m, mpos, sc)
         assert sc_in is None
         h = self.nhead
@@ -237,15 +248,22 @@
         with torch.cuda.stream(side):
             out = initial_queries()
         sc = None
+        node = gate_vectors_node(us) if (blocks.ENABLED and torch.is_grad_enabled()) else None
+        links = blocks.gate_defer_pairs(len(self.layers), d, self.nhead, node is not None)
+        if links is not None:
+            if not hasattr(node, 'gate_defer_links'):
+                node.gate_defer_links = []
+            node.gate_defer_links.append(links)
+        defer = lambda li: None if links is None else (links[li - 1] if li > 0 else None, links[li] if li < len(links) else None)
         for li, (layer, u) in enumerate(zip(self.layers, us)):
             with torch.cuda.stream(side):
                 out_sa = layer.query_self(out, qpos, vid_pos.dtype)
             if blocks.ENABLED and blocks.GATE_SCORES_FUSE and li + 1 < len(us):
-                m32, m, mpos, sc = layer.video_half(mem32, src_skch32, vid_pos, u, us[li + 1], sc)
+                m32, m, mpos, sc = layer.video_half(mem32, src_skch32, vid_pos, u, us[li + 1], sc, defer(li))
             elif sc is not None:
-                m32, m, mpos = layer.video_half(mem32, src_skch32, vid_pos, u, None, sc)
+                m32, m, mpos = layer.video_half(mem32, src_skch32, vid_pos, u, None, sc, defer(li))
             else:
-                m32, m, mpos = layer.video_half(mem32, src_skch32, vid_pos, u)
+                m32, m, mpos = layer.video_half(mem32, src_skch32, vid_pos, u, None, None, defer(li))
             side.wait_stream(main)
             m.record_stream(side)
             mpos.record_stream(side)
```

Result: no change. 15390 (median of 6 runs) (+0.6%).
